# ChunLI-666/PointCloudProcessor

Measured on AMD Instinct MI355X. Metric: Mpoints×frames/sec colorized, higher is better.
Workload: dtype f32/f64

## Files before the change

### include/pcp_hip.h

```cpp
#ifndef PCP_HIP_H
#define PCP_HIP_H

#include <stdint.h>

#ifdef __cplusplus
extern "C" {
#endif

#define PCP_ABI_VERSION 6

#define PCP_OK 0
#define PCP_ERR_INVALID (-1)
#define PCP_ERR_STATE (-2)
#define PCP_ERR_DEVICE (-3)
#define PCP_ERR_NOMEM (-4)
#define PCP_ERR_RANGE (-5)

typedef struct pcp_context pcp_context;

typedef struct pcp_pose {
  double x, y, z, qw, qx, qy, qz;
} pcp_pose;

typedef struct pcp_camera {
// ... 70 lines not shown
int pcp_upload_cloud_aos(pcp_context *ctx, const void *points, int64_t n, int64_t stride_bytes);
int pcp_upload_cloud_from_result(pcp_context *dst, pcp_context *src, int64_t *out_n);
int64_t pcp_cloud_size(const pcp_context *ctx);

int pcp_pose_to_matrices(const pcp_pose *pose, const double *T_opt, float w2c[12], float c2w[12]);
int pcp_set_frames(pcp_context *ctx, const pcp_pose *poses, int32_t n_frames, const double *T_opt,
                   int32_t T_opt_stride);
int32_t pcp_frame_count(const pcp_context *ctx);
int pcp_upload_image(pcp_context *ctx, int32_t frame, const uint8_t *bgr, int64_t row_stride_bytes);
int pcp_upload_image_async(pcp_context *ctx, int32_t frame, const uint8_t *bgr, int64_t row_stride_bytes);
int pcp_upload_images_block(pcp_context *ctx, int32_t first_frame, int32_t count, const uint8_t *bgr, int64_t row_stride_bytes,
                            int64_t frame_stride_bytes);
int pcp_set_image_adjust(pcp_context *ctx, int32_t enable, float saturation_scale, float brightness_scale);
int pcp_download_image(pcp_context *ctx, int32_t frame, uint8_t *out_bgr, uint8_t *out_mask);
#define PCP_JPEG_MAGIC 0x4A504350u
#define PCP_JPEG_VERSION 1
typedef struct pcp_jpeg_component {
  int32_t h, v;
  int32_t blocks_w, blocks_h;
  int32_t down_w, down_h;
} pcp_jpeg_component;
typedef struct pcp_jpeg_header {
  uint32_t magic, version;
  int32_t width, height, ncomp, reserved;
  pcp_jpeg_component comp[3];
  int64_t n_blocks, n_values;
  int64_t quant_off, mask_off, offset_off, value_off;
} pcp_jpeg_header;
int pcp_upload_image_jpeg(pcp_context *ctx, int32_t frame, const uint8_t *blob, int64_t bytes);
int pcp_upload_image_jpeg_async(pcp_context *ctx, int32_t frame, const uint8_t *blob, int64_t bytes);
int pcp_upload_mask(pcp_context *ctx, int32_t frame, const uint8_t *gray, int64_t row_stride_bytes);

int pcp_project_frame(pcp_context *ctx, int32_t frame, int32_t *out_cell, int32_t *out_pixel, float *out_range,
                      float *out_xyz_cam);
int pcp_cull_frame(pcp_context *ctx, int32_t frame, uint8_t *out_keep, int64_t *out_kept, float *out_depth_map);
int pcp_frame_visible(pcp_context *ctx, int32_t frame, int64_t capacity, int32_t *out_index, uint8_t *out_rgb,
                      uint16_t *out_mask, float *out_xyz_cam, float *out_xyz_world, int64_t *out_count);

int pcp_hpr_stats(pcp_context *ctx, int64_t out[10]);

int pcp_depth_pass(pcp_context *ctx, int32_t frame_begin, int32_t frame_end);
int pcp_depth_maps_device(pcp_context *ctx, void **device_ptr, int64_t *n_floats);
int pcp_download_depth_map(pcp_context *ctx, int32_t frame, float *out_depth_map);
int pcp_depth_accum_reset(pcp_context *ctx);
int pcp_depth_accum_merge(pcp_context *ctx);
int pcp_depth_accum_apply(pcp_context *ctx);
int pcp_depth_accum_device(pcp_context *ctx, void **device_ptr, int64_t *n_floats);
#define PCP_DEPTH_OWN 0
#define PCP_DEPTH_BATCHED 1
int pcp_set_depth_source(pcp_context *ctx, int32_t source);
int pcp_hull_flags_import(pcp_context *ctx, int32_t frame, const uint8_t *keep);
int pcp_colour_reset(pcp_context *ctx);
int pcp_colour_pass(pcp_context *ctx, int32_t frame_begin, int32_t frame_end);
int pcp_colour_finalise(pcp_context *ctx, uint8_t *out_rgb, uint8_t *out_has, int32_t *out_count,
                        float *out_top_score, uint32_t *out_top_rgb, int32_t *out_top_frame);
int pcp_colorize(pcp_context *ctx, uint8_t *out_rgb, uint8_t *out_has);
int pcp_colorize_from_depth(pcp_context *ctx, uint8_t *out_rgb, uint8_t *out_has);
int pcp_download_result_packed(pcp_context *ctx, uint32_t *out_rgba);
int pcp_download_result_packed_async(pcp_context *ctx, uint32_t *out_rgba);
int pcp_download_wait_previous(pcp_context *ctx);
int pcp_colour_result_device(pcp_context *ctx, void **device_ptr, int64_t *n_words);
int pcp_colour_compact(pcp_context *ctx, int64_t capacity, int32_t *out_index, float *out_xyz, uint8_t *out_rgb, uint8_t *out_label,
                       int64_t *out_count);

int pcp_set_label_fusion(pcp_context *ctx, int32_t enable);
int pcp_colour_labels(pcp_context *ctx, uint8_t *out_label, uint8_t *out_hits, uint8_t *out_views);
int pcp_colour_labels_device(pcp_context *ctx, void **device_ptr, int64_t *n_words);

int pcp_colour_smooth_local(pcp_context *ctx, float radius, int64_t *out_has_count);
int pcp_colour_smooth_local_packed(pcp_context *ctx, float radius, const uint32_t *in_rgba, uint32_t *out_rgba,
                                   int64_t *out_has_count);

int pcp_mls_process(pcp_context *ctx, const pcp_mls_params *p, int64_t *out_count);
int pcp_set_mls_local_plane(pcp_context *ctx, double upsampling_radius, double upsampling_step);
int pcp_mls_local_plane_samples(double radius, double step, int64_t capacity, float *out_u, float *out_v, int64_t *out_count);
int pcp_mls_process_shard(pcp_context *ctx, const pcp_mls_params *p, int64_t index_begin, int64_t index_end,
                          int64_t *out_count);
int pcp_mls_process_slab(pcp_context *ctx, const pcp_mls_params *p, int32_t slab, int32_t n_slabs, int64_t *out_count);
int pcp_mls_stream_begin(pcp_context *ctx, const pcp_mls_params *p, int64_t chunk_capacity, int64_t *out_total,
                         int32_t *out_chunks);
int pcp_mls_stream_next(pcp_context *ctx, int64_t *out_count);
int pcp_mls_stream_seek(pcp_context *ctx, int32_t chunk);
int pcp_mls_fetch(pcp_context *ctx, int64_t capacity, float *out_xyz, float *out_normal, float *out_curvature,
                  int32_t *out_index);
int pcp_cloud_smooth(pcp_context *ctx, const pcp_mls_params *p, int64_t *out_count);

int pcp_cloud_smooth_stream_begin(pcp_context *ctx, const pcp_mls_params *p, int64_t chunk_capacity, int64_t *out_total_rows,
                                  int64_t *out_kept_rows, int32_t *out_chunks);
int pcp_cloud_smooth_stream_next(pcp_context *ctx, int64_t *out_count);
int pcp_cloud_smooth_stream_end(pcp_context *ctx);
int pcp_cloud_smooth_stream_seek(pcp_context *ctx, int32_t chunk);
int pcp_cloud_smooth_stream_stats(pcp_context *ctx, double out[13]);
int pcp_sor(pcp_context *ctx, int32_t mean_k, double std_mul, uint8_t *out_keep, int64_t *out_kept);
int64_t pcp_sor_chunk_points(void);
int pcp_sor_partial(pcp_context *ctx, int32_t mean_k, int32_t slab, int32_t n_slabs, int64_t capacity, double *out_chunk_sums,
                    int64_t *out_first_chunk, int64_t *out_chunks);
int pcp_sor_finish(pcp_context *ctx, double std_mul, const double *all_chunk_sums, int64_t n_chunks, int32_t slab, int32_t n_slabs,
                   uint8_t *out_keep, int64_t *out_kept);

int pcp_upload_intensity(pcp_context *ctx, const float *intensity, int64_t n);
int pcp_nid_prepare(pcp_context *ctx, int64_t *out_points);
int pcp_nid_evaluate(pcp_context *ctx, const double T[16], const double *T_init, int32_t bins, double *cost,
                     double grad6[6], int32_t *valid);
int pcp_nid_optimize(pcp_context *ctx, const double T_init[16], int32_t bins, int32_t max_outer_iterations,
                     double T_out[16], double *final_cost, int32_t *evaluations);

int pcp_nid_accumulate(pcp_context *ctx, const double T[16], int32_t bins);
int pcp_nid_histograms_device(pcp_context *ctx, void **device_ptr, int64_t *count);
int pcp_nid_finish(pcp_context *ctx, int32_t bins, double *cost, double grad6[6], int32_t *valid);
typedef int (*pcp_nid_eval_fn)(void *user, const double T[16], int32_t bins, double *cost, double grad6[6], int32_t *valid);
int pcp_nid_optimize_with(pcp_context *ctx, pcp_nid_eval_fn eval, void *user, const double T_init[16], int32_t bins,
                          int32_t max_outer_iterations, double T_out[16], double *final_cost, int32_t *evaluations);

#define PCP_ROWS_XYZI 0
#define PCP_ROWS_XYZRGB 1
#define PCP_ROWS_XYZRGBMASK 2
#define PCP_ROWS_POINTNORMAL 3
int64_t pcp_ascii_row_bound(int32_t kind);
int pcp_ascii_rows_host(int32_t kind, int64_t n, const float *f, const uint8_t *rgb, const uint16_t *mask, int64_t capacity,
                        char *out_text, int64_t *out_bytes);
int pcp_ascii_rows(pcp_context *ctx, int32_t kind, int64_t n, const float *f, const uint8_t *rgb, const uint16_t *mask,
                   int64_t capacity, char *out_text, int64_t *out_bytes);
int pcp_colour_compact_ascii(pcp_context *ctx, int32_t with_label, int64_t first_row, int64_t max_rows, int64_t capacity,
                             char *out_text, int64_t *out_rows, int64_t *out_bytes);
int pcp_mls_fetch_ascii(pcp_context *ctx, int64_t first_row, int64_t max_rows, int64_t capacity, char *out_text,
                        int64_t *out_rows, int64_t *out_bytes);

#define PCP_ASCII_PARSE_MAX_ROW 65536
#define PCP_PARSE_LIMIT_ROW 0
#define PCP_PARSE_LIMIT_TILE 1
#define PCP_PARSE_LIMIT_PIECE 2
#define PCP_PARSE_LIMIT_TILE_ROWS 3
#define PCP_PARSE_LIMIT_WINDOW 4
int64_t pcp_ascii_parse_limit(int32_t which);
int pcp_ascii_parse_host(const char *text, int64_t bytes, int32_t columns, const int32_t col[4], int32_t final_window,
                         int64_t max_rows, float *out_x, float *out_y, float *out_z, float *out_intensity,
                         int64_t *out_rows, int64_t *out_consumed, int64_t *out_bad_row);
int pcp_ascii_parse(pcp_context *ctx, const char *text, int64_t bytes, int32_t columns, const int32_t col[4], int32_t final_window,
                    int64_t max_rows, float *out_x, float *out_y, float *out_z, float *out_intensity,
                    int64_t *out_rows, int64_t *out_consumed, int64_t *out_bad_row);

int pcp_close_pairs(pcp_context *ctx, double radius, int64_t *points_with_close_neighbour);

int pcp_timing_enable(pcp_context *ctx, int32_t on);
int pcp_timing_reset(pcp_context *ctx);
int pcp_timing_get(pcp_context *ctx, int32_t kernel_id, double *total_ms, int64_t *launches);
const char *pcp_kernel_name(int32_t kernel_id);
int pcp_tile_mask_density(pcp_context *ctx, double *kept_fraction);
int pcp_tile_masks(pcp_context *ctx, int64_t *tiles, int32_t *mask_words, uint32_t *out_words);
int pcp_sor_redo_fraction(pcp_context *ctx, double *fraction);
int pcp_sor_distances(pcp_context *ctx, int64_t capacity, float *out_distance);
int pcp_selftest_arithmetic(pcp_context *ctx, int64_t samples, uint64_t seed, int64_t *mismatches_fp64,
                            int64_t *mismatches_fp32);

#ifdef __cplusplus
}
#endif
#endif
```

### pointcloudprocessor_amd/_build.py

```python
from __future__ import annotations

import os
import subprocess

_PKG = os.path.dirname(os.path.abspath(__file__))
_ROOT = os.path.dirname(_PKG)
CSRC = os.path.join(_PKG, "csrc")
LIB_DIR = os.path.join(_PKG, "lib")
LIB_PATH = os.path.join(LIB_DIR, "libpcp_hip.so")
INCLUDE = os.path.join(_ROOT, "include")

SOURCES = ["pcp_context.hip", "pcp_colour.hip", "pcp_mls.hip", "pcp_nid.hip", "pcp_hpr.hip", "pcp_colour_smooth.hip", "pcp_match.hip", "pcp_jpeg.hip",
           "pcp_stream_colour.hip", "pcp_ascii.hip", "pcp_ascii_parse.hip"]
HEADERS = ["pcp_internal.hpp", "pcp_device.hpp", "pcp_scan.hpp", "pcp_hsv.hpp", "pcp_exact.hpp", "pcp_ascii.hpp", "pcp_ascii_parse.hpp"]

HIPCC_FLAGS = [
    "--offload-arch=gfx950",
    "-O3",
    "-std=c++17",
    "-fPIC",
    "-ffp-contract=off",
    "-fhip-fp32-correctly-rounded-divide-sqrt",
    "-Wall",
    "-Wextra",
]


def _hipcc() -> str:
    for cand in (os.environ.get("HIPCC"), "/opt/rocm/bin/hipcc", "hipcc"):
        if cand and (os.path.isabs(cand) and os.path.exists(cand) or not os.path.isabs(cand)):
            return cand
    return "hipcc"


def source_sha256() -> str:
    import hashlib

    h = hashlib.sha256()
    h.update(" ".join(HIPCC_FLAGS).encode())
    for f in [os.path.join(CSRC, f) for f in SOURCES + HEADERS] + [os.path.join(INCLUDE, "pcp_hip.h")]:
        h.update(os.path.basename(f).encode())
        with open(f, "rb") as fh:
            h.update(fh.read())
    return h.hexdigest()


def is_stale() -> bool:
    if not os.path.exists(LIB_PATH):
        return True
    t = os.path.getmtime(LIB_PATH)
    deps = [os.path.join(CSRC, f) for f in SOURCES + HEADERS] + [os.path.join(INCLUDE, "pcp_hip.h")]
    return any(os.path.getmtime(d) > t for d in deps)


def build(force: bool = False, verbose: bool = False) -> str:
    if not force and not is_stale():
        return LIB_PATH
    os.makedirs(LIB_DIR, exist_ok=True)
    from concurrent.futures import ThreadPoolExecutor

    obj_dir = os.path.join(LIB_DIR, "obj")
    os.makedirs(obj_dir, exist_ok=True)
    inc = ["-I", os.path.relpath(INCLUDE, CSRC), "-I", "."]

    def compile_one(src):
        stem = os.path.splitext(src)[0]
        obj = os.path.join(os.path.relpath(obj_dir, CSRC), stem + ".o")
        cmd = [_hipcc()] + HIPCC_FLAGS + inc + [f"-cuid={stem}", "-c", src, "-o", obj]
        return cmd, subprocess.run(cmd, capture_output=True, text=True, cwd=CSRC)

    with ThreadPoolExecutor(max_workers=len(SOURCES)) as pool:
        results = list(pool.map(compile_one, SOURCES))
    log = ""
    for cmd, proc in results:
        if verbose or proc.returncode != 0:
            log += " ".join(cmd) + "\n" + proc.stdout + proc.stderr
    if any(proc.returncode != 0 for _, proc in results):
        print(log)
        raise RuntimeError("hipcc failed building libpcp_hip.so:\n" + log[-4000:])
    objs = [os.path.join(os.path.relpath(obj_dir, CSRC), os.path.splitext(src)[0] + ".o") for src in SOURCES]
    link = [_hipcc(), "--offload-arch=gfx950", "--hip-link", "-shared", "-fPIC", "-o", LIB_PATH] + objs
    proc = subprocess.run(link, capture_output=True, text=True, cwd=CSRC)
    if verbose or proc.returncode != 0:
        print(log + " ".join(link))
        print(proc.stdout)
        print(proc.stderr)
    if proc.returncode != 0:
        raise RuntimeError("hipcc failed linking libpcp_hip.so:\n" + proc.stderr[-4000:])
    return LIB_PATH


if __name__ == "__main__":
    print(build(force=True, verbose=True))
```

### pointcloudprocessor_amd/capi.py

```python
from __future__ import annotations

import ctypes as C
import os
import re

import numpy as np

from . import _build

PCP_OK = 0
PCP_ERR_INVALID = -1
PCP_ERR_STATE = -2
PCP_ERR_DEVICE = -3
PCP_ERR_NOMEM = -4
PCP_ERR_RANGE = -5

NID_EVAL_FN = C.CFUNCTYPE(C.c_int, C.c_void_p, C.POINTER(C.c_double), C.c_int32, C.POINTER(C.c_double), C.POINTER(C.c_double),
                          C.POINTER(C.c_int32))
K_PROJECT, K_DEPTH, K_COLOUR, K_VISIBILITY, K_MLS_GRID, K_MLS_FIT, K_MISC, K_SOR, K_MLS_VOXEL, K_TILE_MASK, K_NID, K_HPR = range(12)
K_COLOUR_SMOOTH = 12
K_COUNT = 13


class PcpError(RuntimeError):
# ... 635 lines not shown
    def cloud_smooth(self, params: MLSParams) -> int:
        cnt = C.c_int64()
        self._check(self.lib.pcp_cloud_smooth(self.h, C.byref(params), C.byref(cnt)))
        return cnt.value

    def mls_fetch(self, count: int):
        xyz = np.empty((count, 3), np.float32)
        nrm = np.empty((count, 3), np.float32)
        curv = np.empty(count, np.float32)
        idx = np.empty(count, np.int32)
        self._check(self.lib.pcp_mls_fetch(self.h, C.c_int64(count), _ptr(xyz), _ptr(nrm), _ptr(curv), _ptr(idx)))
        return dict(xyz=xyz, normal=nrm, curvature=curv, index=idx)

    def mls_fetch_index(self, count: int) -> np.ndarray:
        idx = np.empty(count, np.int32)
        self._check(self.lib.pcp_mls_fetch(self.h, C.c_int64(count), None, None, None, _ptr(idx)))
        return idx

    def sor(self, mean_k: int = 60, std_mul: float = 0.7):
        keep = np.empty(self.n, np.uint8)
        kept = C.c_int64()
        self._check(self.lib.pcp_sor(self.h, C.c_int32(mean_k), C.c_double(std_mul), _ptr(keep), C.byref(kept)))
        return keep, kept.value

    def sor_chunk_points(self) -> int:
        return int(self.lib.pcp_sor_chunk_points())

    def sor_partial(self, mean_k: int, slab: int, n_slabs: int):
        c = self.sor_chunk_points()
        chunks = (self.n + c - 1) // c
        out = np.zeros((max(chunks, 1), 2), np.float64)
        first, cnt = C.c_int64(), C.c_int64()
        self._check(self.lib.pcp_sor_partial(self.h, C.c_int32(mean_k), C.c_int32(slab), C.c_int32(n_slabs), C.c_int64(len(out)),
                                             _ptr(out), C.byref(first), C.byref(cnt)))
        return first.value, out[:cnt.value].copy()

    def sor_finish(self, std_mul: float, all_chunk_sums: np.ndarray, slab: int, n_slabs: int):
        sums = np.ascontiguousarray(all_chunk_sums, np.float64)
        keep = np.empty(self.n, np.uint8)
        kept = C.c_int64()
        self._check(self.lib.pcp_sor_finish(self.h, C.c_double(std_mul), _ptr(sums), C.c_int64(len(sums)), C.c_int32(slab),
                                            C.c_int32(n_slabs), _ptr(keep), C.byref(kept)))
        return keep, kept.value

    def close_pairs(self, radius: float = 2.5e-5) -> int:
        cnt = C.c_int64()
        self._check(self.lib.pcp_close_pairs(self.h, C.c_double(radius), C.byref(cnt)))
        return cnt.value

    def sor_distances(self) -> np.ndarray:
        out = np.empty(self.n, np.float32)
        self._check(self.lib.pcp_sor_distances(self.h, C.c_int64(len(out)), _ptr(out)))
        return out

    def sor_redo_fraction(self) -> float:
        v = C.c_double()
        self._check(self.lib.pcp_sor_redo_fraction(self.h, C.byref(v)))
        return v.value

    def upload_intensity(self, intensity):
        a = np.ascontiguousarray(intensity, np.float32)
        self._check(self.lib.pcp_upload_intensity(self.h, _ptr(a), C.c_int64(len(a))))

    def nid_prepare(self) -> int:
        cnt = C.c_int64()
        self._check(self.lib.pcp_nid_prepare(self.h, C.byref(cnt)))
        return cnt.value

    def nid_evaluate(self, T, T_init=None, bins: int = 16):
        T = np.ascontiguousarray(T, np.float64).reshape(16)
        Ti = None if T_init is None else np.ascontiguousarray(T_init, np.float64).reshape(16)
        cost = C.c_double()
        grad = np.zeros(6, np.float64)
        valid = C.c_int32()
        self._check(self.lib.pcp_nid_evaluate(self.h, _ptr(T), _ptr(Ti), C.c_int32(bins), C.byref(cost), _ptr(grad),
                                              C.byref(valid)))
        return cost.value, grad, bool(valid.value)

    def nid_optimize(self, T_init, bins: int = 16, max_outer_iterations: int = 10):
        Ti = np.ascontiguousarray(T_init, np.float64).reshape(16)
        out = np.zeros(16, np.float64)
        cost = C.c_double()
        evals = C.c_int32()
        self._check(self.lib.pcp_nid_optimize(self.h, _ptr(Ti), C.c_int32(bins), C.c_int32(max_outer_iterations), _ptr(out),
                                              C.byref(cost), C.byref(evals)))
        return out.reshape(4, 4), cost.value, evals.value

    def nid_accumulate(self, T, bins: int = 16):
        T = np.ascontiguousarray(T, np.float64).reshape(16)
        self._check(self.lib.pcp_nid_accumulate(self.h, _ptr(T), C.c_int32(bins)))

    def nid_histograms_device(self):
        p = C.c_void_p()
        n = C.c_int64()
        self._check(self.lib.pcp_nid_histograms_device(self.h, C.byref(p), C.byref(n)))
        return p.value, n.value

    def nid_finish(self, bins: int = 16):
        cost = C.c_double()
        grad = np.zeros(6, np.float64)
        valid = C.c_int32()
        self._check(self.lib.pcp_nid_finish(self.h, C.c_int32(bins), C.byref(cost), _ptr(grad), C.byref(valid)))
        return cost.value, grad, bool(valid.value)

    def nid_optimize_with(self, evaluate, T_init, bins: int = 16, max_outer_iterations: int = 10):
        errors = []

        @NID_EVAL_FN
        def trampoline(_user, T, b, cost, grad, valid):
            try:
                c, g, ok = evaluate(np.ctypeslib.as_array(T, (16,)).copy().reshape(4, 4), int(b))
                cost[0] = float(c)
                for k in range(6):
                    grad[k] = float(g[k])
                valid[0] = 1 if ok else 0
                return 0
            except Exception as e:
                errors.append(e)
                return -3

        Ti = np.ascontiguousarray(T_init, np.float64).reshape(16)
        out = np.zeros(16, np.float64)
        cost = C.c_double()
        evals = C.c_int32()
        rc = self.lib.pcp_nid_optimize_with(self.h, trampoline, None, _ptr(Ti), C.c_int32(bins), C.c_int32(max_outer_iterations),
                                            _ptr(out), C.byref(cost), C.byref(evals))
        if errors:
            raise errors[0]
        self._check(rc)
        return out.reshape(4, 4), cost.value, evals.value

    def timing_enable(self, on: bool = True):
        self._check(self.lib.pcp_timing_enable(self.h, C.c_int32(1 if on else 0)))

    def timing_reset(self):
        self._check(self.lib.pcp_timing_reset(self.h))

    def timing_get(self, kernel_id: int):
        ms = C.c_double()
        cnt = C.c_int64()
        self._check(self.lib.pcp_timing_get(self.h, C.c_int32(kernel_id), C.byref(ms), C.byref(cnt)))
        return ms.value, cnt.value

    def tile_mask_density(self) -> float:
        v = C.c_double()
        self._check(self.lib.pcp_tile_mask_density(self.h, C.byref(v)))
        return v.value

    def selftest_arithmetic(self, samples: int = 1 << 26, seed: int = 1):
        a, b = C.c_int64(), C.c_int64()
        self._check(self.lib.pcp_selftest_arithmetic(self.h, C.c_int64(samples), C.c_uint64(seed), C.byref(a), C.byref(b)))
        return a.value, b.value

    def tile_masks(self) -> np.ndarray:
        t, w = C.c_int64(), C.c_int32()
        self._check(self.lib.pcp_tile_masks(self.h, C.byref(t), C.byref(w), None))
        out = np.empty((t.value, w.value), np.uint32)
        self._check(self.lib.pcp_tile_masks(self.h, None, None, _ptr(out)))
        return out

    def kernel_name(self, kernel_id: int) -> str:
        return self.lib.pcp_kernel_name(C.c_int32(kernel_id)).decode()
```

### pointcloudprocessor_amd/csrc/pcp_colour.hip

```cpp
#include <algorithm>
#include <cfloat>
#include <cstdlib>

#include "pcp_device.hpp"
#include "pcp_hsv.hpp"
#include "pcp_scan.hpp"

namespace pcp {

constexpr int kBlock = 256;
constexpr uint32_t kFltMaxBits = 0x7f7fffffu;

template <bool kCommon>
__device__ __forceinline__ DevCamera common_camera(const DevCamera &in) {
  DevCamera c = in;
  if constexpr (kCommon) {
    c.cull_mode = PCP_CULL_ZBUFFER;
    c.enable_zbuf = 1;
    c.pretest = 1;
    c.ds_fast = 1;
  }
  return c;
}
inline bool is_common_camera(const DevCamera &c) {
  return c.cull_mode == PCP_CULL_ZBUFFER && c.enable_zbuf == 1 && c.pretest == 1 && c.ds_fast == 1;
}

struct ProjectOut {
  int32_t *cell;
  int32_t *pixel;
  float *range;
  float *xc, *yc, *zc;
};

__device__ __forceinline__ void project_store_one(const DevCamera &cam, const DevFrame &fr, float x, float y, float z,
                                                  int32_t &cell, int32_t &pixel, float &range, float &xc, float &yc,
                                                  float &zc) {
  const Projected p = project_point<true, false>(cam, fr.w2c, x, y, z);
  cell = p.cell;
  pixel = p.pixel;
  range = p.cell != -1 ? static_cast<float>(range64(p.xc, p.yc, p.zc)) : FLT_MAX;
  xc = p.xc;
  yc = p.yc;
  zc = p.zc;
}

template <bool kCommon>
__global__ __launch_bounds__(kBlock) void k_project_frame(const float *__restrict__ x, const float *__restrict__ y,
                                                          const float *__restrict__ z, int64_t n, DevCamera cam_in,
                                                          DevFrame fr, ProjectOut out) {
  const DevCamera cam = common_camera<kCommon>(cam_in);
  const int64_t q = static_cast<int64_t>(blockIdx.x) * kBlock + threadIdx.x;
  const int64_t i0 = q * 4;
  if (i0 >= n) return;
  if (i0 + 3 < n) {
    typedef float nt_f4 __attribute__((ext_vector_type(4)));
    typedef int nt_i4 __attribute__((ext_vector_type(4)));
    const nt_f4 ax = __builtin_nontemporal_load(reinterpret_cast<const nt_f4 *>(x + i0));
    const nt_f4 ay = __builtin_nontemporal_load(reinterpret_cast<const nt_f4 *>(y + i0));
    const nt_f4 az = __builtin_nontemporal_load(reinterpret_cast<const nt_f4 *>(z + i0));
    const float4 vx = make_float4(ax.x, ax.y, ax.z, ax.w), vy = make_float4(ay.x, ay.y, ay.z, ay.w),
                 vz = make_float4(az.x, az.y, az.z, az.w);
    int4 cell, pixel;
    float4 range, xc, yc, zc;
    project_store_one(cam, fr, vx.x, vy.x, vz.x, cell.x, pixel.x, range.x, xc.x, yc.x, zc.x);
    project_store_one(cam, fr, vx.y, vy.y, vz.y, cell.y, pixel.y, range.y, xc.y, yc.y, zc.y);
    project_store_one(cam, fr, vx.z, vy.z, vz.z, cell.z, pixel.z, range.z, xc.z, yc.z, zc.z);
    project_store_one(cam, fr, vx.w, vy.w, vz.w, cell.w, pixel.w, range.w, xc.w, yc.w, zc.w);
    if (out.cell) {
      const nt_i4 c4 = {cell.x, cell.y, cell.z, cell.w};
      __builtin_nontemporal_store(c4, reinterpret_cast<nt_i4 *>(out.cell + i0));
    }
    if (out.range) {
      const nt_f4 r4 = {range.x, range.y, range.z, range.w};
      __builtin_nontemporal_store(r4, reinterpret_cast<nt_f4 *>(out.range + i0));
    }
    if (out.pixel) *reinterpret_cast<int4 *>(out.pixel + i0) = pixel;
    if (out.xc) {
      *reinterpret_cast<float4 *>(out.xc + i0) = xc;
      *reinterpret_cast<float4 *>(out.yc + i0) = yc;
      *reinterpret_cast<float4 *>(out.zc + i0) = zc;
    }
  } else {
    for (int64_t i = i0; i < n; ++i) {
      int32_t cell, pixel;
      float range, xc, yc, zc;
      project_store_one(cam, fr, x[i], y[i], z[i], cell, pixel, range, xc, yc, zc);
      if (out.cell) out.cell[i] = cell;
      if (out.range) out.range[i] = range;
      if (out.pixel) out.pixel[i] = pixel;
      if (out.xc) {
        out.xc[i] = xc;
        out.yc[i] = yc;
        out.zc[i] = zc;
      }
    }
  }
}

struct Interval {
  double lo, hi;
};
__device__ __forceinline__ Interval iv_add(Interval a, Interval b) { return {a.lo + b.lo, a.hi + b.hi}; }
__device__ __forceinline__ Interval iv_scale(double k, Interval a) {
  return k >= 0.0 ? Interval{k * a.lo, k * a.hi} : Interval{k * a.hi, k * a.lo};
}
__device__ __forceinline__ Interval iv_mul(Interval a, Interval b) {
  const double p0 = a.lo * b.lo, p1 = a.lo * b.hi, p2 = a.hi * b.lo, p3 = a.hi * b.hi;
  return {fmin(fmin(p0, p1), fmin(p2, p3)), fmax(fmax(p0, p1), fmax(p2, p3))};
}
__device__ __forceinline__ Interval iv_sqr(Interval a) {
  const double l = fabs(a.lo), h = fabs(a.hi);
  const double mx = fmax(l, h), mn = (a.lo <= 0.0 && a.hi >= 0.0) ? 0.0 : fmin(l, h);
  return {mn * mn, mx * mx};
}
__device__ __forceinline__ Interval iv_mul_pos(Interval a, Interval b) { return {a.lo * b.lo, a.hi * b.hi}; }
__device__ __forceinline__ Interval iv_mul_by_pos(Interval a, Interval b) {
  return {a.lo * (a.lo >= 0.0 ? b.lo : b.hi), a.hi * (a.hi >= 0.0 ? b.hi : b.lo)};
}
__device__ __forceinline__ double iv_rcp_pos(double b) {
  double r = __builtin_amdgcn_rcp(b);
  r = fma(fma(-b, r, 1.0), r, r);
  r = fma(fma(-b, r, 1.0), r, r);
  return r;
}
__device__ __forceinline__ Interval iv_pad(Interval a) {
  const double e = 1e-12 * (fabs(a.lo) + fabs(a.hi)) + 1e-300;
  return {a.lo - e, a.hi + e};
}

__device__ __forceinline__ int tile_classify(const DevCamera &c, const DevFrame &fr, float4 sph) {
  const double cx = sph.x, cy = sph.y, cz = sph.z;
  const float *m = fr.w2c;
  const double X = (m[0] * cx + m[1] * cy) + (m[2] * cz + m[3]);
  const double Y = (m[4] * cx + m[5] * cy) + (m[6] * cz + m[7]);
  const double Z = (m[8] * cx + m[9] * cy) + (m[10] * cz + m[11]);
  const double mag = fr.norm_bound * (fabs(cx) + fabs(cy) + fabs(cz) + 3.0 * sph.w) + fabs(static_cast<double>(m[3])) +
                     fabs(static_cast<double>(m[7])) + fabs(static_cast<double>(m[11])) + 1e-3;
  const double rho = fr.norm_bound * static_cast<double>(sph.w) * (1.0 + 1e-6) + 1e-6 * mag;
  if (!(rho >= 0.0) || !isfinite(X + Y + Z + rho)) return 0;
  if (Z + rho <= 0.0) return 1;
  if (Z - rho <= 0.0) return 0;
  const Interval zi{Z - rho, Z + rho};
  if (!(zi.lo >= 1e-290)) return 0;
  const Interval iz{iv_rcp_pos(zi.hi) * (1.0 - 1e-13), iv_rcp_pos(zi.lo) * (1.0 + 1e-13)};
  const Interval xn = iv_pad(iv_mul_by_pos(Interval{X - rho, X + rho}, iz));
  const Interval yn = iv_pad(iv_mul_by_pos(Interval{Y - rho, Y + rho}, iz));
  const Interval x2 = iv_sqr(xn), y2 = iv_sqr(yn);
  const Interval r2 = iv_add(x2, y2);
  const Interval r4 = iv_mul_pos(r2, r2);
  const Interval r6 = iv_mul_pos(r2, r4);
  Interval rc = iv_add(iv_add(iv_scale(c.k1, r2), iv_scale(c.k2, r4)), iv_scale(c.k3, r6));
  rc.lo += 1.0;
  rc.hi += 1.0;
  const Interval t1 = iv_scale(2.0, iv_mul(xn, yn));
  const Interval t2 = iv_add(r2, iv_scale(2.0, x2));
  const Interval t3 = iv_add(r2, iv_scale(2.0, y2));
  const Interval xd = iv_pad(iv_add(iv_add(iv_mul(rc, xn), iv_scale(c.p1, t1)), iv_scale(c.p2, t2)));
  const Interval yd = iv_pad(iv_add(iv_add(iv_mul(rc, yn), iv_scale(c.p1, t3)), iv_scale(c.p2, t1)));
  Interval u = iv_pad(iv_scale(c.fx, xd)), v = iv_pad(iv_scale(c.fy, yd));
  u.lo += c.cx; u.hi += c.cx;
  v.lo += c.cy; v.hi += c.cy;
  if (!isfinite(u.lo + u.hi + v.lo + v.hi)) return 0;
  if (u.hi < static_cast<double>(c.u_lo) || u.lo > static_cast<double>(c.u_hi) ||
      v.hi < static_cast<double>(c.v_lo) || v.lo > static_cast<double>(c.v_hi))
    return 1;
  return (u.lo > static_cast<double>(c.u_lo) + 1.0 && u.hi < static_cast<double>(c.u_hi) - 1.0 &&
          v.lo > static_cast<double>(c.v_lo) + 1.0 && v.hi < static_cast<double>(c.v_hi) - 1.0)
             ? 2
             : 0;
}

constexpr int kTileGroup = 16;

__global__ __launch_bounds__(kBlock) void k_group_mask_flat(const float4 *__restrict__ spheres, int64_t groups, DevCamera cam,
                                                            const DevFrame *__restrict__ frames, int32_t n_frames,
                                                            int32_t w0, int32_t w1, int32_t words,
                                                            uint32_t *__restrict__ group_mask,
// ... 54 lines not shown
      if (b >= 0 && have) cls = cull_enabled ? tile_classify(cam, frames[(w << 5) + b], sph) : 0;
      const unsigned long long keep = __ballot(cls != 1), ins = __ballot(cls == 2);
#pragma unroll
      for (int k = 0; k < 4; ++k) {
        if (bit[k] >= 0) {
          word |= static_cast<uint32_t>((keep >> (k * 16 + t)) & 1ull) << bit[k];
          inside |= static_cast<uint32_t>((ins >> (k * 16 + t)) & 1ull) << bit[k];
        }
      }
    }
  }
  if (slot == 0 && have) {
    tile_mask[tile * words + w] = word;
    if (inside_mask) inside_mask[tile * words + w] = inside;
  }
}

constexpr int kWorkBins = 1024;
constexpr int kWorkPerBlock = 1024;
__global__ __launch_bounds__(kBlock) void k_tile_work_hist(const uint32_t *__restrict__ tile_mask, int64_t tiles, int32_t w0,
                                                          int32_t w1, int32_t words, int32_t *__restrict__ tile_work,
                                                          int32_t *__restrict__ hist) {
  __shared__ int32_t cnt[kWorkBins];
  for (int b = threadIdx.x; b < kWorkBins; b += kBlock) cnt[b] = 0;
  __syncthreads();
  const int64_t base = static_cast<int64_t>(blockIdx.x) * kWorkPerBlock;
  for (int q = 0; q < kWorkPerBlock / kBlock; ++q) {
    const int64_t t = base + q * kBlock + threadIdx.x;
    if (t < tiles) {
      int32_t visits = 0;
      for (int32_t w = w0; w < w1; ++w) visits += __builtin_popcount(tile_mask[t * words + w]);
      tile_work[t] = visits;
      atomicAdd(&cnt[min(visits, kWorkBins - 1)], 1);
    }
  }
  __syncthreads();
  for (int b = threadIdx.x; b < kWorkBins; b += kBlock)
    if (cnt[b]) atomicAdd(&hist[b], cnt[b]);
}
__device__ __forceinline__ int32_t block_exclusive_scan(int32_t v, int32_t *total);
__global__ __launch_bounds__(kBlock) void k_work_scatter(const int32_t *__restrict__ work, int64_t tiles,
                                                        const int32_t *__restrict__ hist, int32_t *__restrict__ cursor,
                                                        int32_t *__restrict__ order) {
  __shared__ int32_t cnt[kWorkBins];
  __shared__ int32_t first[kWorkBins];
  for (int b = threadIdx.x; b < kWorkBins; b += kBlock) cnt[b] = 0;
  {
    constexpr int kPer = kWorkBins / kBlock;
    int32_t h[kPer], mine = 0;
#pragma unroll
    for (int k = 0; k < kPer; ++k) {
      h[k] = hist[kWorkBins - 1 - (static_cast<int>(threadIdx.x) * kPer + k)];
      mine += h[k];
    }
    int32_t total = 0;
    int32_t run = block_exclusive_scan(mine, &total);
#pragma unroll
    for (int k = 0; k < kPer; ++k) {
      first[kWorkBins - 1 - (static_cast<int>(threadIdx.x) * kPer + k)] = run;
      run += h[k];
    }
  }
  __syncthreads();
  const int64_t base = static_cast<int64_t>(blockIdx.x) * kWorkPerBlock;
  int32_t bin[kWorkPerBlock / kBlock], rank[kWorkPerBlock / kBlock];
#pragma unroll
  for (int q = 0; q < kWorkPerBlock / kBlock; ++q) {
    const int64_t t = base + q * kBlock + threadIdx.x;
    bin[q] = t < tiles ? min(work[t], kWorkBins - 1) : -1;
    rank[q] = bin[q] >= 0 ? atomicAdd(&cnt[bin[q]], 1) : 0;
  }
  __syncthreads();
  for (int b = threadIdx.x; b < kWorkBins; b += kBlock)
    if (cnt[b]) cnt[b] = first[b] + atomicAdd(&cursor[b], cnt[b]);
  __syncthreads();
#pragma unroll
  for (int q = 0; q < kWorkPerBlock / kBlock; ++q)
    if (bin[q] >= 0) order[cnt[bin[q]] + rank[q]] = static_cast<int32_t>(base + q * kBlock + threadIdx.x);
}

constexpr uint32_t kXcdChunk = 16;
__device__ __forceinline__ uint32_t xcd_chunked_block() {
  constexpr uint32_t kXcd = 8, kSuper = kXcd * kXcdChunk;
  const uint32_t b = blockIdx.x;
  if (b >= (gridDim.x / kSuper) * kSuper) return b;
  const uint32_t x = b % kXcd, slot = b / kXcd;
  return ((slot / kXcdChunk) * kXcd + x) * kXcdChunk + slot % kXcdChunk;
}

constexpr unsigned long long kDepthEmpty = 0x7f7f7f7f7f7f7f7full;
__device__ __forceinline__ void depth_min(unsigned long long *__restrict__ map, int32_t cell, unsigned long long bits) {
  if (bits < map[cell]) atomicMin(map + cell, bits);
}
__device__ __forceinline__ double sumsq64(float xc, float yc, float zc) {
  const double X = xc, Y = yc, Z = zc;
  return (X * X + Y * Y) + Z * Z;
}
__global__ __launch_bounds__(kBlock) void k_depth_finish(const unsigned long long *__restrict__ sq, int64_t count,
                                                         uint32_t *__restrict__ range) {
  int64_t i = static_cast<int64_t>(blockIdx.x) * kBlock + threadIdx.x;
  const int64_t stride = static_cast<int64_t>(gridDim.x) * kBlock;
  for (; i < count; i += stride) {
    const unsigned long long b = sq[i];
    float r = FLT_MAX;
    if (b != kDepthEmpty) r = fminf(static_cast<float>(sqrt(__longlong_as_double(static_cast<long long>(b)))), FLT_MAX);
    range[i] = __float_as_uint(r);
  }
}

__device__ __forceinline__ uint32_t range_bits(int32_t w, int32_t f0, int32_t f1) {
  const int32_t fb = max(f0, w << 5), fe = min(f1, (w << 5) + 32);
  const int32_t nb = fe - fb;
  return nb <= 0 ? 0u : (((nb >= 32) ? 0xffffffffu : ((1u << nb) - 1u)) << (fb & 31));
}

template <bool kCommon>
__global__ __launch_bounds__(kBlock) void k_depth_pass(const float *__restrict__ x, const float *__restrict__ y,
                                                       const float *__restrict__ z, int64_t n, DevCamera cam_in,
                                                       const DevFrame *__restrict__ frames, int32_t f0, int32_t f1,
                                                       unsigned long long *__restrict__ depth, int64_t cells,
                                                       int32_t depth_first_frame, uint32_t *__restrict__ tile_mask,
                                                       const uint32_t *__restrict__ tile_inside, int32_t words,
                                                       const int32_t *__restrict__ tile_order) {
  DevCamera cam = common_camera<kCommon>(cam_in);
  if constexpr (kCommon) cam.pretest = 0;
  __shared__ unsigned long long combine[kBlock];
  const int lane = threadIdx.x & 63;
  unsigned long long *tbl = combine + (threadIdx.x & ~63);
  const int64_t j = tile_order ? static_cast<int64_t>(tile_order[blockIdx.x]) * 64 + threadIdx.x
                               : static_cast<int64_t>(xcd_chunked_block()) * kBlock + threadIdx.x;
  const bool live = j < n;
  if (!__ballot(live)) return;
  const float px = live ? x[j] : 0.0f, py = live ? y[j] : 0.0f, pz = live ? z[j] : 0.0f;
  const int64_t tile = __builtin_amdgcn_readfirstlane(static_cast<int32_t>(j >> 6));
  const bool finite_sure = cam.frames_bounded != 0 && __all(fabsf(px) <= 0x1p40f && fabsf(py) <= 0x1p40f && fabsf(pz) <= 0x1p40f);
  unsigned long long *held_at = nullptr;
  unsigned long long held_bits = 0ull, held_seen = 0ull;
  auto settle_held = [&]() {
    if (held_at && held_bits < held_seen) atomicMin(held_at, held_bits);
    held_at = nullptr;
  };
  for (int32_t w = f0 >> 5; w <= (f1 - 1) >> 5; ++w) {
    const uint32_t in_range = range_bits(w, f0, f1);
    uint32_t todo = in_range;
    if (tile_mask) todo &= tile_mask[tile * words + w];
    todo = __builtin_amdgcn_readfirstlane(todo);
    const uint32_t inside = tile_inside ? __builtin_amdgcn_readfirstlane(tile_inside[tile * words + w]) : 0u;
    uint32_t seen = 0u;
    while (todo) {
      const int32_t b = __builtin_ctz(todo);
      const int32_t f = (w << 5) + b;
      todo &= todo - 1u;
      const DevFrame &fr = frames[f];
      const Projected p = project_point(cam, fr.w2c, px, py, pz, ((inside >> b) & 1u) == 0u, finite_sure);
      const bool in_map = live && p.cell >= 0;
      const bool cand = live && p.pixel >= 0 && (cam.enable_zbuf ? p.cell >= 0 : p.cell != -1);
      if (__ballot(cand)) seen |= 1u << b;
      settle_held();
      if (cam.enable_zbuf && __ballot(in_map)) {
        unsigned long long *map = depth + static_cast<uint64_t>(static_cast<uint32_t>(f - depth_first_frame)) * static_cast<uint32_t>(cells);
        unsigned long long key = ~0ull, sbits = 0ull;
        if (in_map) {
          sbits = static_cast<unsigned long long>(__double_as_longlong(sumsq64(p.xc, p.yc, p.zc)));
          key = (static_cast<unsigned long long>(static_cast<uint32_t>(p.cell)) << 32) | (sbits >> 32);
        }
        tbl[lane] = ~0ull;
        __builtin_amdgcn_wave_barrier();
        if (in_map) atomicMin(&tbl[p.cell & 63], key);
        __builtin_amdgcn_wave_barrier();
        if (in_map) {
          const unsigned long long got = tbl[p.cell & 63];
          if (got == key || static_cast<uint32_t>(got >> 32) != static_cast<uint32_t>(p.cell)) {
            held_at = map + p.cell;
            held_bits = sbits;
            held_seen = *held_at;
          }
        }
        __builtin_amdgcn_wave_barrier();
      }
    }
    if (tile_mask && lane == 0 && live) {
      uint32_t *dst = tile_mask + tile * words + w;
      *dst = (*dst & ~in_range) | seen;
    }
  }
  settle_held();
}

__global__ __launch_bounds__(kBlock) void k_visibility(const float *__restrict__ x, const float *__restrict__ y,
                                                       const float *__restrict__ z, int64_t n, DevCamera cam,
                                                       DevFrame fr, const uint32_t *__restrict__ depth,
                                                       const int32_t *__restrict__ perm,
                                                       uint8_t *__restrict__ keep, int32_t require_pixel) {
  const int64_t i = static_cast<int64_t>(blockIdx.x) * kBlock + threadIdx.x;
  if (i >= n) return;
  const Projected p = project_point(cam, fr.w2c, x[i], y[i], z[i]);
  bool k = keep_rule(cam, p, depth);
  if (require_pixel) k = k && p.pixel >= 0;
  if (k) keep[perm ? perm[i] : i] = 1;
}

__device__ __forceinline__ bool keep_by_depth(float xc, float yc, float zc, double lim) {
  const double s = sumsq64(xc, yc, zc);
  const double L = lim * lim;
  bool keep = s < L * (1.0 - 0x1p-40);
  const bool sure = lim > 0.0 && (keep || s > L * (1.0 + 0x1p-40));
  if (!sure) keep = !(sqrt(s) > lim);
  return keep;
}

struct TopState {
  float *score;
  uint32_t *rgb;
  int32_t *frame;
  int32_t *count;
};

struct MatchArgs {
  const uint8_t *in_a;
  unsigned long long *moved;
  float e2;
};

struct LabelOut {
  uint32_t *word;
};

template <bool kCommon, int kMatch, bool kOneShot, bool kLabel = false>
__global__ __launch_bounds__(kBlock) void k_colour_pass(const float *__restrict__ x, const float *__restrict__ y,
                                                        const float *__restrict__ z, int64_t n, DevCamera cam_in,
                                                        const DevFrame *__restrict__ frames, int32_t f0, int32_t f1,
                                                        const uint32_t *__restrict__ depth, int64_t cells,
                                                        const uint32_t *__restrict__ tile_mask, int32_t words,
                                                        const uint32_t *__restrict__ images, int64_t image_px,
                                                        TopState st, const int32_t *__restrict__ perm,
                                                        uint32_t *__restrict__ rgba, int32_t flags_in,
                                                        const uint32_t *__restrict__ hull_bits_in, MatchArgs mb,
                                                        [[maybe_unused]] LabelOut lab) {
  DevCamera cam = common_camera<kCommon>(cam_in);
  if constexpr (kMatch == 1) cam.match_mode = PCP_MATCH_IDENTITY;
  if constexpr (kMatch == 2 || kMatch == 3) cam.match_mode = PCP_MATCH_ROUNDTRIP;
  const uint32_t *__restrict__ hull_bits = kCommon ? nullptr : hull_bits_in;
  const int32_t flags = kOneShot ? 4 : flags_in;
  const int64_t j = static_cast<int64_t>(xcd_chunked_block()) * kBlock + threadIdx.x;
  const bool live = j < n;
  if (!__ballot(live)) return;
  const float px = live ? x[j] : 0.0f, py = live ? y[j] : 0.0f, pz = live ? z[j] : 0.0f;
  const int64_t tile = __builtin_amdgcn_readfirstlane(static_cast<int32_t>(j >> 6));
  const bool finite_sure = cam.frames_bounded != 0 && __all(fabsf(px) <= 0x1p40f && fabsf(py) <= 0x1p40f && fabsf(pz) <= 0x1p40f);
  Top5 t;
  t.init();
  if ((flags & 1) && live) {
    t.s0 = st.score[0 * n + j]; t.s1 = st.score[1 * n + j]; t.s2 = st.score[2 * n + j];
    t.s3 = st.score[3 * n + j]; t.s4 = st.score[4 * n + j];
    t.c0 = st.rgb[0 * n + j]; t.c1 = st.rgb[1 * n + j]; t.c2 = st.rgb[2 * n + j];
    t.c3 = st.rgb[3 * n + j]; t.c4 = st.rgb[4 * n + j];
    t.f0 = st.frame[0 * n + j]; t.f1 = st.frame[1 * n + j]; t.f2 = st.frame[2 * n + j];
    t.f3 = st.frame[3 * n + j]; t.f4 = st.frame[4 * n + j];
    t.count = st.count[j];
  }
  [[maybe_unused]] bool in_a = false;
  [[maybe_unused]] uint32_t moved = 0u;
  if constexpr (kMatch == 3) in_a = live && mb.in_a[j] != 0;
  for (int32_t w = f0 >> 5; w <= (f1 - 1) >> 5; ++w) {
    uint32_t todo = range_bits(w, f0, f1);
    if (tile_mask) todo &= tile_mask[tile * words + w];
    todo = __builtin_amdgcn_readfirstlane(todo);
    const uint32_t hull_word = (hull_bits && live) ? hull_bits[static_cast<int64_t>(w) * n + j] : 0xffffffffu;
    while (todo) {
      const int32_t f = (w << 5) + __builtin_ctz(todo);
      todo &= todo - 1u;
      const DevFrame &fr = frames[f];
      const Projected p = project_point<false>(cam, fr.w2c, px, py, pz, true, finite_sure);
      const bool cand = live && p.pixel >= 0 && (cam.enable_zbuf ? p.cell >= 0 : p.cell != -1) &&
                        ((hull_word >> (f & 31)) & 1u);
      if (cand) {
        const uint32_t dbits = cam.enable_zbuf ? depth[static_cast<uint64_t>(static_cast<uint32_t>(f)) * static_cast<uint32_t>(cells) + static_cast<uint32_t>(p.cell)] : 0u;
        bool keep = true;
        if (cam.enable_zbuf) keep = keep_by_depth(p.xc, p.yc, p.zc, static_cast<double>(__uint_as_float(dbits)) + cam.slack);
        float sx = p.xc, sy = p.yc, sz = p.zc;
        if constexpr (kMatch == 3) {
          if (keep) keep = roundtrip_sample_moved(cam, fr, px, py, pz, sx, sy, sz, mb.e2, moved) && !in_a;
        } else {
          if (cam.match_mode == PCP_MATCH_ROUNDTRIP && keep) keep = roundtrip_sample(cam, fr, px, py, pz, sx, sy, sz);
        }
        if (keep) {
          const uint32_t texel = images[static_cast<uint64_t>(static_cast<uint32_t>(f)) * static_cast<uint32_t>(image_px) + static_cast<uint32_t>(p.pixel)];
          t.insert(final_score(sx, sy, sz, fr.px, fr.py, fr.pz), kLabel ? texel : texel & 0xffffffu, f);
        }
      }
    }
  }
  if constexpr (kMatch == 3) {
    if (moved) atomicAdd(mb.moved, static_cast<unsigned long long>(moved));
  }
  if (!live) return;
  if (flags & 2) {
    st.score[0 * n + j] = t.s0; st.score[1 * n + j] = t.s1; st.score[2 * n + j] = t.s2;
    st.score[3 * n + j] = t.s3; st.score[4 * n + j] = t.s4;
    st.rgb[0 * n + j] = t.c0; st.rgb[1 * n + j] = t.c1; st.rgb[2 * n + j] = t.c2;
    st.rgb[3 * n + j] = t.c3; st.rgb[4 * n + j] = t.c4;
    st.frame[0 * n + j] = t.f0; st.frame[1 * n + j] = t.f1; st.frame[2 * n + j] = t.f2;
    st.frame[3 * n + j] = t.f3; st.frame[4 * n + j] = t.f4;
    st.count[j] = t.count;
  }
  if (flags & 4) {
    const int64_t o = perm[j];
    rgba[o] = t.finalise();
    if constexpr (kLabel) {
      uint32_t bad = 0u;
      lab.word[o] = t.labels(bad);
      if (bad) lab.word[n] = 1u;
    }
  }
}

__device__ __forceinline__ Top5 load_top5(const TopState &st, int64_t n, int64_t j) {
  Top5 t;
  t.s0 = st.score[0 * n + j]; t.s1 = st.score[1 * n + j]; t.s2 = st.score[2 * n + j];
  t.s3 = st.score[3 * n + j]; t.s4 = st.score[4 * n + j];
  t.c0 = st.rgb[0 * n + j]; t.c1 = st.rgb[1 * n + j]; t.c2 = st.rgb[2 * n + j];
  t.c3 = st.rgb[3 * n + j]; t.c4 = st.rgb[4 * n + j];
  t.f0 = st.frame[0 * n + j]; t.f1 = st.frame[1 * n + j]; t.f2 = st.frame[2 * n + j];
  t.f3 = st.frame[3 * n + j]; t.f4 = st.frame[4 * n + j];
  t.count = st.count[j];
  return t;
}
__global__ __launch_bounds__(kBlock) void k_finalise(int64_t n, TopState st, const int32_t *__restrict__ perm,
                                                     uint32_t *__restrict__ rgba) {
  const int64_t j = static_cast<int64_t>(blockIdx.x) * kBlock + threadIdx.x;
  if (j >= n) return;
  const Top5 t = load_top5(st, n, j);
  rgba[static_cast<int64_t>(perm[j])] = t.finalise();
}
__global__ __launch_bounds__(kBlock) void k_finalise_labels(int64_t n, TopState st, const int32_t *__restrict__ perm,
                                                            uint32_t *__restrict__ rgba, LabelOut lab) {
  const int64_t j = static_cast<int64_t>(blockIdx.x) * kBlock + threadIdx.x;
  if (j >= n) return;
  const Top5 t = load_top5(st, n, j);
  const int64_t o = perm[j];
  rgba[o] = t.finalise();
  uint32_t bad = 0u;
  lab.word[o] = t.labels(bad);
  if (bad) lab.word[n] = 1u;
}

template <bool kLabel>
__global__ __launch_bounds__(kBlock) void k_match_fixup(const float *__restrict__ x, const float *__restrict__ y,
                                                        const float *__restrict__ z, int64_t n, DevCamera cam,
                                                        const DevFrame *__restrict__ frames, int32_t f0, int32_t f1,
                                                        const uint32_t *__restrict__ depth, int64_t cells,
                                                        const uint32_t *__restrict__ tile_mask, int32_t words,
                                                        const uint32_t *__restrict__ images, int64_t image_px, TopState st,
                                                        const int32_t *__restrict__ perm, uint32_t *__restrict__ rgba,
                                                        int32_t flags, const uint32_t *__restrict__ hull_bits,
                                                        const int32_t *__restrict__ list, int64_t na,
                                                        const int64_t *__restrict__ off, const int32_t *__restrict__ cols,
                                                        [[maybe_unused]] LabelOut lab) {
  const int64_t a = static_cast<int64_t>(blockIdx.x) * kBlock + threadIdx.x;
  if (a >= na) return;
  const int64_t j = list[a];
  Top5 t;
  t.init();
  if (flags & 1) {
    t.s0 = st.score[0 * n + j]; t.s1 = st.score[1 * n + j]; t.s2 = st.score[2 * n + j];
    t.s3 = st.score[3 * n + j]; t.s4 = st.score[4 * n + j];
    t.c0 = st.rgb[0 * n + j]; t.c1 = st.rgb[1 * n + j]; t.c2 = st.rgb[2 * n + j];
    t.c3 = st.rgb[3 * n + j]; t.c4 = st.rgb[4 * n + j];
    t.f0 = st.frame[0 * n + j]; t.f1 = st.frame[1 * n + j]; t.f2 = st.frame[2 * n + j];
    t.f3 = st.frame[3 * n + j]; t.f4 = st.frame[4 * n + j];
    t.count = st.count[j];
  }
  const float qx = x[j], qy = y[j], qz = z[j];
  const int64_t r0 = off[a], r1 = off[a + 1];
  for (int32_t f = f0; f < f1; ++f) {
    const DevFrame &fr = frames[f];
    const int32_t w = f >> 5;
    const uint32_t bit = 1u << (f & 31);
    for (int64_t r = r0; r < r1; ++r) {
      const int64_t i = cols[r];
      if (tile_mask && !(tile_mask[(i >> 6) * words + w] & bit)) continue;
      if (hull_bits && !(hull_bits[static_cast<int64_t>(w) * n + i] & bit)) continue;
      const float px = x[i], py = y[i], pz = z[i];
      const Projected p = project_point<false>(cam, fr.w2c, px, py, pz);
      const bool cand = p.pixel >= 0 && (cam.enable_zbuf ? p.cell >= 0 : p.cell != -1);
      if (!cand) continue;
      if (cam.enable_zbuf) {
        const uint32_t dbits = depth[static_cast<uint64_t>(static_cast<uint32_t>(f)) * static_cast<uint32_t>(cells) + static_cast<uint32_t>(p.cell)];
        if (!keep_by_depth(p.xc, p.yc, p.zc, static_cast<double>(__uint_as_float(dbits)) + cam.slack)) continue;
      }
      float sx = p.xc, sy = p.yc, sz = p.zc;
      if (!roundtrip_sample(cam, fr, qx, qy, qz, sx, sy, sz)) continue;
      const uint32_t texel = images[static_cast<uint64_t>(static_cast<uint32_t>(f)) * static_cast<uint32_t>(image_px) + static_cast<uint32_t>(p.pixel)];
      t.insert(final_score(sx, sy, sz, fr.px, fr.py, fr.pz), kLabel ? texel : texel & 0xffffffu, f);
    }
  }
  if (flags & 2) {
    st.score[0 * n + j] = t.s0; st.score[1 * n + j] = t.s1; st.score[2 * n + j] = t.s2;
    st.score[3 * n + j] = t.s3; st.score[4 * n + j] = t.s4;
    st.rgb[0 * n + j] = t.c0; st.rgb[1 * n + j] = t.c1; st.rgb[2 * n + j] = t.c2;
    st.rgb[3 * n + j] = t.c3; st.rgb[4 * n + j] = t.c4;
    st.frame[0 * n + j] = t.f0; st.frame[1 * n + j] = t.f1; st.frame[2 * n + j] = t.f2;
    st.frame[3 * n + j] = t.f3; st.frame[4 * n + j] = t.f4;
    st.count[j] = t.count;
  }
  if (flags & 4) {
    const int64_t o = perm[j];
    rgba[o] = t.finalise();
    if constexpr (kLabel) {
      uint32_t bad = 0u;
      lab.word[o] = t.labels(bad);
      if (bad) lab.word[n] = 1u;
    }
  }
}

template <bool kLabel>
inline auto colour_pass_kernel(bool common, int32_t match_mode, int32_t flags) {
  auto kernel = k_colour_pass<false, 0, false, kLabel>;
  if (common && match_mode == PCP_MATCH_IDENTITY)
    kernel = flags == 4 ? k_colour_pass<true, 1, true, kLabel> : k_colour_pass<true, 1, false, kLabel>;
  if (common && match_mode == PCP_MATCH_ROUNDTRIP)
    kernel = flags == 4 ? k_colour_pass<true, 2, true, kLabel> : k_colour_pass<true, 2, false, kLabel>;
  if (match_mode == PCP_MATCH_RADIUS)
    kernel = !common ? k_colour_pass<false, 3, false, kLabel>
                     : flags == 4 ? k_colour_pass<true, 3, true, kLabel> : k_colour_pass<true, 3, false, kLabel>;
  return kernel;
}

__device__ __forceinline__ uint64_t mix64(uint64_t v) {
  v += 0x9e3779b97f4a7c15ull;
  v = (v ^ (v >> 30)) * 0xbf58476d1ce4e5b9ull;
  v = (v ^ (v >> 27)) * 0x94d049bb133111ebull;
  return v ^ (v >> 31);
}
__device__ __forceinline__ bool same_f64(double a, double b) {
  if (a != a && b != b) return true;
  if (a == 0.0 && b == 0.0) return true;
  return __double_as_longlong(a) == __double_as_longlong(b);
}

__global__ __launch_bounds__(kBlock) void k_selftest_div64(int64_t samples, uint64_t seed,
                                                           unsigned long long *__restrict__ bad) {
  const int64_t i = static_cast<int64_t>(blockIdx.x) * kBlock + threadIdx.x;
  if (i >= samples) return;
  const uint64_t a = mix64(seed ^ static_cast<uint64_t>(i) * 3u), b = mix64(a);
  uint32_t bx = static_cast<uint32_t>(a), by = static_cast<uint32_t>(a >> 32), bz = static_cast<uint32_t>(b);
  const uint32_t mode = static_cast<uint32_t>(b >> 32) & 3u;
  if (mode != 0u) {
    const uint32_t span = mode == 1u ? 12u : 40u;
    bx = (bx & 0x807fffffu) | ((127u - span / 2u + (bx >> 23) % span) << 23);
    by = (by & 0x807fffffu) | ((127u - span / 2u + (by >> 23) % span) << 23);
    bz = (bz & 0x807fffffu) | ((127u - span / 2u + (bz >> 23) % span) << 23);
  }
  const float xc = __uint_as_float(bx), yc = __uint_as_float(by), zc = fabsf(__uint_as_float(bz));
  if (!(zc > 0.0f)) return;
  double xn, yn;
  divide_xy_by_z(xc, yc, zc, xn, yn);
  const double xr = static_cast<double>(xc) / static_cast<double>(zc);
  const double yr = static_cast<double>(yc) / static_cast<double>(zc);
  if (!same_f64(xn, xr) || !same_f64(yn, yr)) atomicAdd(bad, 1ull);
}

__global__ __launch_bounds__(kBlock) void k_selftest_div32(DevCamera cam, unsigned long long *__restrict__ bad) {
  const uint32_t lane = blockIdx.x * kBlock + threadIdx.x;
  uint32_t wrong = 0u;
  for (uint32_t k = 0; k < 256u; ++k) {
    const float x = __uint_as_float((k << 24) | lane);
    const float a = div_by_ds(cam, x), b = x / cam.ds_f;
    const float ax = fabsf(x);
    if (ax >= 0x1p-40f && ax <= 0x1p60f) {
      if (!((a != a && b != b) || __float_as_uint(a) == __float_as_uint(b))) ++wrong;
    } else {
      if (cell_of_quotient(a, cam.cull_wf) != cell_of_quotient(b, cam.cull_wf)) ++wrong;
      if (cell_of_quotient(a, cam.cull_hf) != cell_of_quotient(b, cam.cull_hf)) ++wrong;
    }
  }
  if (wrong) atomicAdd(bad, static_cast<unsigned long long>(wrong));
}

__global__ __launch_bounds__(kBlock) void k_unpack_result(const uint32_t *__restrict__ packed, int64_t n,
                                                         uint8_t *__restrict__ rgb, uint8_t *__restrict__ has) {
  const int64_t i = static_cast<int64_t>(blockIdx.x) * kBlock + threadIdx.x;
  if (i >= n) return;
  const uint32_t v = packed[i];
  rgb[3 * i + 0] = static_cast<uint8_t>(v & 0xffu);
  rgb[3 * i + 1] = static_cast<uint8_t>((v >> 8) & 0xffu);
  rgb[3 * i + 2] = static_cast<uint8_t>((v >> 16) & 0xffu);
  has[i] = static_cast<uint8_t>(v >> 24);
}

__global__ __launch_bounds__(kBlock) void k_unpack_labels(const uint32_t *__restrict__ packed, int64_t n,
                                                         uint8_t *__restrict__ label, uint8_t *__restrict__ hits,
                                                         uint8_t *__restrict__ views) {
  const int64_t i = static_cast<int64_t>(blockIdx.x) * kBlock + threadIdx.x;
  if (i >= n) return;
  const uint32_t v = packed[i];
  if (label) label[i] = static_cast<uint8_t>(v & 0xffu);
  if (hits) hits[i] = static_cast<uint8_t>((v >> 8) & 0xffu);
  if (views) views[i] = static_cast<uint8_t>((v >> 16) & 0xffu);
}

__global__ __launch_bounds__(kBlock) void k_fill_u32(uint32_t *__restrict__ p, int64_t n, uint32_t v) {
  int64_t i = static_cast<int64_t>(blockIdx.x) * kBlock + threadIdx.x;
  const int64_t stride = static_cast<int64_t>(gridDim.x) * kBlock;
  for (; i < n; i += stride) p[i] = v;
}

__global__ __launch_bounds__(kBlock) void k_scatter_u32(const uint32_t *__restrict__ in,
                                                        const int32_t *__restrict__ perm, int64_t n,
                                                        uint32_t *__restrict__ out) {
  const int64_t j = static_cast<int64_t>(blockIdx.x) * kBlock + threadIdx.x;
  if (j < n) out[perm[j]] = in[j];
}

__global__ __launch_bounds__(kBlock) void k_pack_bgr(const uint8_t *__restrict__ bgr, int64_t row_stride, int32_t w,
                                                     int32_t h, uint32_t *__restrict__ texels, int32_t clear_mask,
                                                     const int32_t *__restrict__ hsv_tables, float sat_scale,
                                                     float val_scale) {
  const int64_t i = static_cast<int64_t>(blockIdx.x) * kBlock + threadIdx.x;
  if (i >= static_cast<int64_t>(w) * h) return;
  const int32_t v = static_cast<int32_t>(i / w), u = static_cast<int32_t>(i - static_cast<int64_t>(v) * w);
  const uint8_t *p = bgr + static_cast<int64_t>(v) * row_stride + 3 * u;
  const uint32_t keep = clear_mask ? 0u : (texels[i] & 0xff000000u);
  uint32_t b = p[0], g = p[1], r = p[2];
  if (hsv_tables) hsv_round_trip(hsv_tables, hsv_tables + 256, sat_scale, val_scale, b, g, r);
  texels[i] = keep | b | (g << 8) | (r << 16);
}

__global__ __launch_bounds__(kBlock) void k_pack_bgr16(const uint8_t *__restrict__ bgr, int64_t row_stride, int32_t w,
                                                       int32_t h, uint32_t *__restrict__ texels, int32_t clear_mask,
                                                       const int32_t *__restrict__ hsv_tables, float sat_scale,
                                                       float val_scale) {
  const int32_t groups = w >> 4;
  const int64_t n_groups = static_cast<int64_t>(groups) * h;
  const int64_t g = static_cast<int64_t>(blockIdx.x) * kBlock + threadIdx.x;
  uint4 a, b, c;
  if (row_stride == 3 * static_cast<int64_t>(w)) {
    __shared__ uint4 piece[3 * kBlock];
    const int64_t base = static_cast<int64_t>(blockIdx.x) * (3 * kBlock);
    const int64_t pieces = 3 * n_groups;
    const uint4 *src = reinterpret_cast<const uint4 *>(bgr);
#pragma unroll
    for (int q = 0; q < 3; ++q) {
      const int64_t i = base + q * kBlock + threadIdx.x;
      if (i < pieces) piece[q * kBlock + threadIdx.x] = src[i];
    }
    __syncthreads();
    if (g >= n_groups) return;
    a = piece[3 * threadIdx.x];
    b = piece[3 * threadIdx.x + 1];
    c = piece[3 * threadIdx.x + 2];
  } else {
    if (g >= n_groups) return;
    const int32_t vr = static_cast<int32_t>(g / groups), gr = static_cast<int32_t>(g - static_cast<int64_t>(vr) * groups);
    const uint4 *src = reinterpret_cast<const uint4 *>(bgr + static_cast<int64_t>(vr) * row_stride + static_cast<int64_t>(gr) * 48);
    a = src[0];
    b = src[1];
    c = src[2];
  }
  const int32_t v = static_cast<int32_t>(g / groups), gu = static_cast<int32_t>(g - static_cast<int64_t>(v) * groups);
  const uint32_t in[12] = {a.x, a.y, a.z, a.w, b.x, b.y, b.z, b.w, c.x, c.y, c.z, c.w};
  uint4 *dst = reinterpret_cast<uint4 *>(texels + static_cast<int64_t>(v) * w + static_cast<int64_t>(gu) * 16);
  uint32_t out[16];
#pragma unroll
  for (int q = 0; q < 4; ++q) {
    const uint32_t d0 = in[3 * q], d1 = in[3 * q + 1], d2 = in[3 * q + 2];
    out[4 * q + 0] = d0 & 0xffffffu;
    out[4 * q + 1] = (d0 >> 24) | ((d1 & 0xffffu) << 8);
    out[4 * q + 2] = (d1 >> 16) | ((d2 & 0xffu) << 16);
    out[4 * q + 3] = d2 >> 8;
  }
  if (hsv_tables) {
#pragma unroll
    for (int k = 0; k < 16; ++k) {
      uint32_t bb = out[k] & 0xffu, gg = (out[k] >> 8) & 0xffu, rr = out[k] >> 16;
      hsv_round_trip(hsv_tables, hsv_tables + 256, sat_scale, val_scale, bb, gg, rr);
      out[k] = bb | (gg << 8) | (rr << 16);
    }
  }
  if (!clear_mask) {
#pragma unroll
    for (int q = 0; q < 4; ++q) {
      const uint4 old = dst[q];
      out[4 * q + 0] |= old.x & 0xff000000u;
      out[4 * q + 1] |= old.y & 0xff000000u;
      out[4 * q + 2] |= old.z & 0xff000000u;
      out[4 * q + 3] |= old.w & 0xff000000u;
    }
  }
#pragma unroll
  for (int q = 0; q < 4; ++q) dst[q] = make_uint4(out[4 * q], out[4 * q + 1], out[4 * q + 2], out[4 * q + 3]);
}

__global__ __launch_bounds__(kBlock) void k_pack_mask(const uint8_t *__restrict__ gray, int64_t row_stride, int32_t w,
                                                      int32_t h, uint32_t *__restrict__ texels) {
  const int64_t i = static_cast<int64_t>(blockIdx.x) * kBlock + threadIdx.x;
  if (i >= static_cast<int64_t>(w) * h) return;
  const int32_t v = static_cast<int32_t>(i / w), u = static_cast<int32_t>(i - static_cast<int64_t>(v) * w);
  texels[i] = (texels[i] & 0x00ffffffu) | (static_cast<uint32_t>(gray[static_cast<int64_t>(v) * row_stride + u]) << 24);
}

constexpr int kTile = 1024;

__device__ __forceinline__ int32_t block_exclusive_scan(int32_t v, int32_t *total) {
  __shared__ int32_t wave_sum[kBlock / 64];
  const int lane = threadIdx.x & 63, wid = threadIdx.x >> 6;
  int32_t incl = v;
#pragma unroll
  for (int o = 1; o < 64; o <<= 1) {
    const int32_t t = __shfl_up(incl, o, 64);
    if (lane >= o) incl += t;
  }
  if (lane == 63) wave_sum[wid] = incl;
  __syncthreads();
  int32_t base = 0, tot = 0;
#pragma unroll
  for (int k = 0; k < kBlock / 64; ++k) {
    if (k < wid) base += wave_sum[k];
    tot += wave_sum[k];
  }
  __syncthreads();
  *total = tot;
  return base + incl - v;
}

__global__ __launch_bounds__(kBlock) void k_tile_count(const uint8_t *__restrict__ flags, int64_t n,
                                                       int32_t *__restrict__ tile_count) {
  const int64_t base = static_cast<int64_t>(blockIdx.x) * kTile + threadIdx.x * 4;
  int32_t c = 0;
#pragma unroll
  for (int k = 0; k < 4; ++k)
    if (base + k < n) c += flags[base + k] ? 1 : 0;
// ... 455 lines not shown
  }
  int pack(pcp_context *ctx, int, hipStream_t us, int32_t k, uint32_t *dst, int32_t clear_mask, const int32_t *tables) override {
    const int32_t w = ctx->dcam.img_w, h = ctx->dcam.img_h;
    const int64_t px = static_cast<int64_t>(w) * h;
    const uint8_t *sk = src + static_cast<int64_t>(k) * block_stride;
    if ((w & 15) == 0 && (row_stride_bytes & 15) == 0 && (reinterpret_cast<uintptr_t>(sk) & 15u) == 0)
      hipLaunchKernelGGL(k_pack_bgr16, dim3(blocks_for(px / 16)), dim3(kBlock), 0, us, sk, row_stride_bytes, w, h, dst,
                         clear_mask, tables, ctx->saturation_scale, ctx->brightness_scale);
    else
      hipLaunchKernelGGL(k_pack_bgr, dim3(blocks_for(px)), dim3(kBlock), 0, us, sk, row_stride_bytes, w, h, dst, clear_mask,
                         tables, ctx->saturation_scale, ctx->brightness_scale);
    return PCP_OK;
  }
};

static int upload_image_impl(pcp_context *ctx, const char *who, int32_t frame, const uint8_t *bgr, int64_t row_stride_bytes,
                             bool wait, size_t block_bytes = 0, int64_t block_stride = 0, int32_t block_frames = 1) {
  BgrSource source(bgr, row_stride_bytes, block_bytes, block_stride);
  return upload_texels(ctx, who, frame, block_frames, block_bytes > 0, wait, source);
}

extern "C" {

int pcp_upload_image(pcp_context *ctx, int32_t frame, const uint8_t *bgr, int64_t row_stride_bytes) {
  return upload_image_impl(ctx, "pcp_upload_image", frame, bgr, row_stride_bytes, true);
}

int pcp_upload_image_async(pcp_context *ctx, int32_t frame, const uint8_t *bgr, int64_t row_stride_bytes) {
  return upload_image_impl(ctx, "pcp_upload_image_async", frame, bgr, row_stride_bytes, false);
}

constexpr size_t kBlockUploadBytes = size_t(128) << 20;

int pcp_upload_images_block(pcp_context *ctx, int32_t first_frame, int32_t count, const uint8_t *bgr, int64_t row_stride_bytes,
                            int64_t frame_stride_bytes) {
  int rc = check_ready(ctx, "pcp_upload_images_block", true);
  if (rc != PCP_OK) return rc;
  if (count < 0 || first_frame < 0 || first_frame + count > ctx->n_frames)
    return set_error(ctx, PCP_ERR_RANGE, "pcp_upload_images_block: keyframes [%d, %d) outside 0..%d", first_frame, first_frame + count,
                     ctx->n_frames);
  if (count == 0) return PCP_OK;
  const int32_t w = ctx->dcam.img_w, h = ctx->dcam.img_h;
  if (!bgr || row_stride_bytes < 3 * static_cast<int64_t>(w) || frame_stride_bytes < row_stride_bytes * h)
    return set_error(ctx, PCP_ERR_INVALID, "pcp_upload_images_block: NULL block, row stride < 3*width or frame stride < rows");
  hipPointerAttribute_t attr{};
  const bool host_pinned = hipPointerGetAttributes(&attr, bgr) == hipSuccess && attr.type == hipMemoryTypeHost;
  if (!host_pinned) {
    (void)hipGetLastError();
    for (int32_t k = 0; k < count; ++k)
      if ((rc = upload_image_impl(ctx, "pcp_upload_images_block", first_frame + k, bgr + static_cast<int64_t>(k) * frame_stride_bytes,
                                  row_stride_bytes, false)) != PCP_OK)
        return rc;
    return PCP_OK;
  }
  const int32_t per_block = static_cast<int32_t>(std::max<int64_t>(1, static_cast<int64_t>(kBlockUploadBytes) / frame_stride_bytes));
  for (int32_t b0 = 0; b0 < count; b0 += per_block) {
    const int32_t b1 = std::min(count, b0 + per_block);
    const size_t bytes = static_cast<size_t>(b1 - b0 - 1) * static_cast<size_t>(frame_stride_bytes) + static_cast<size_t>(row_stride_bytes) * h;
    if ((rc = upload_image_impl(ctx, "pcp_upload_images_block", first_frame + b0, bgr + static_cast<int64_t>(b0) * frame_stride_bytes,
                                row_stride_bytes, false, bytes, frame_stride_bytes, b1 - b0)) != PCP_OK)
      return rc;
  }
  return PCP_OK;
}

int pcp_set_image_adjust(pcp_context *ctx, int32_t enable, float saturation_scale, float brightness_scale) {
  if (!ctx) return PCP_ERR_INVALID;
  if (!(saturation_scale >= 0.0f) || !(brightness_scale >= 0.0f))
    return set_error(ctx, PCP_ERR_INVALID, "pcp_set_image_adjust: scales must be >= 0");
  PCP_HIP_TRY(ctx, hipSetDevice(ctx->device));
  if (enable && !ctx->hsv_tables.p) {
    int32_t tab[512];
    hsv_build_tables(tab, tab + 256);
    PCP_HIP_TRY(ctx, ctx->hsv_tables.ensure(512));
    PCP_HIP_TRY(ctx, hipMemcpyAsync(ctx->hsv_tables.p, tab, sizeof(tab), hipMemcpyHostToDevice, ctx->stream));
    PCP_HIP_TRY(ctx, hipStreamSynchronize(ctx->stream));
  }
  ctx->adjust_images = enable != 0;
  ctx->saturation_scale = saturation_scale;
  ctx->brightness_scale = brightness_scale;
  return PCP_OK;
}

int pcp_download_image(pcp_context *ctx, int32_t frame, uint8_t *out_bgr, uint8_t *out_mask) {
  int rc = check_ready(ctx, "pcp_download_image", true);
  if (rc != PCP_OK) return rc;
  if ((rc = check_frame(ctx, "pcp_download_image", frame)) != PCP_OK) return rc;
  if (!ctx->images.p || !(ctx->image_set[static_cast<size_t>(frame)] || ctx->mask_set[static_cast<size_t>(frame)]))
    return set_error(ctx, PCP_ERR_STATE, "pcp_download_image: nothing uploaded for keyframe %d", frame);
  if ((rc = wait_images(ctx, frame, frame + 1)) != PCP_OK) return rc;
  const int32_t w = ctx->dcam.img_w, h = ctx->dcam.img_h;
  const size_t px = static_cast<size_t>(w) * h;
  std::vector<uint32_t> texels(px);
  PCP_HIP_TRY(ctx, hipMemcpyAsync(texels.data(), ctx->images.p + static_cast<int64_t>(frame) * static_cast<int64_t>(px),
                                  px * 4, hipMemcpyDeviceToHost, ctx->stream));
  PCP_HIP_TRY(ctx, hipStreamSynchronize(ctx->stream));
  for (size_t i = 0; i < px; ++i) {
    const uint32_t t = texels[i];
    if (out_bgr) {
      out_bgr[3 * i + 0] = static_cast<uint8_t>(t & 0xffu);
      out_bgr[3 * i + 1] = static_cast<uint8_t>((t >> 8) & 0xffu);
      out_bgr[3 * i + 2] = static_cast<uint8_t>((t >> 16) & 0xffu);
    }
    if (out_mask) out_mask[i] = static_cast<uint8_t>(t >> 24);
  }
  return PCP_OK;
}

int pcp_upload_mask(pcp_context *ctx, int32_t frame, const uint8_t *gray, int64_t row_stride_bytes) {
  int rc = check_ready(ctx, "pcp_upload_mask", true);
  if (rc != PCP_OK) return rc;
  if ((rc = check_frame(ctx, "pcp_upload_mask", frame)) != PCP_OK) return rc;
  const int32_t w = ctx->dcam.img_w, h = ctx->dcam.img_h;
  if (!gray || row_stride_bytes < static_cast<int64_t>(w))
    return set_error(ctx, PCP_ERR_INVALID, "pcp_upload_mask: NULL mask or row stride < width");
  if ((rc = ensure_images(ctx)) != PCP_OK) return rc;
  if ((rc = wait_images(ctx, frame, frame + 1)) != PCP_OK) return rc;
  const size_t bytes = static_cast<size_t>(row_stride_bytes) * h;
  PCP_HIP_TRY(ctx, ctx->s_keep.ensure(bytes + 16));
  PCP_HIP_TRY(ctx, hipMemcpyAsync(ctx->s_keep.p, gray, bytes, hipMemcpyDefault, ctx->stream));
  const int64_t px = static_cast<int64_t>(w) * h;
  {
    LaunchTimer t(ctx, PCP_K_MISC);
    hipLaunchKernelGGL(k_pack_mask, dim3(blocks_for(px)), dim3(kBlock), 0, ctx->stream, ctx->s_keep.p,
                       row_stride_bytes, w, h, ctx->images.p + static_cast<int64_t>(frame) * px);
    PCP_HIP_TRY(ctx, hipGetLastError());
  }
  PCP_HIP_TRY(ctx, hipStreamSynchronize(ctx->stream));
  ctx->mask_set[static_cast<size_t>(frame)] = 1;
  return PCP_OK;
}

int pcp_project_frame(pcp_context *ctx, int32_t frame, int32_t *out_cell, int32_t *out_pixel, float *out_range,
                      float *out_xyz_cam) {
  int rc = check_ready(ctx, "pcp_project_frame", true);
  if (rc != PCP_OK) return rc;
  if ((rc = check_frame(ctx, "pcp_project_frame", frame)) != PCP_OK) return rc;
  const int64_t n = ctx->n;
  const size_t plane = plane_of(ctx);
  PCP_HIP_TRY(ctx, ctx->s_cell.ensure(plane + 4));
  PCP_HIP_TRY(ctx, ctx->s_range.ensure(plane + 4));
  if (out_pixel) PCP_HIP_TRY(ctx, ctx->s_pixel.ensure(plane + 4));
  if (out_xyz_cam) PCP_HIP_TRY(ctx, ctx->s_cam.ensure(3 * plane + 4));
  if (n == 0) return PCP_OK;
  ProjectOut o{};
  o.cell = ctx->s_cell.p;
  o.range = ctx->s_range.p;
  o.pixel = out_pixel ? ctx->s_pixel.p : nullptr;
  o.xc = out_xyz_cam ? ctx->s_cam.p : nullptr;
  o.yc = out_xyz_cam ? ctx->s_cam.p + plane : nullptr;
  o.zc = out_xyz_cam ? ctx->s_cam.p + 2 * plane : nullptr;
  {
    LaunchTimer t(ctx, PCP_K_PROJECT);
    hipLaunchKernelGGL(is_common_camera(ctx->dcam) ? k_project_frame<true> : k_project_frame<false>, dim3(blocks_for(div_up(n, 4))), dim3(kBlock), 0, ctx->stream, ctx->sxyz.p,
                       ctx->sxyz.p + plane, ctx->sxyz.p + 2 * plane, n, ctx->dcam,
                       ctx->hframes[static_cast<size_t>(frame)], o);
    PCP_HIP_TRY(ctx, hipGetLastError());
  }
  if (!(out_cell || out_range || out_pixel || out_xyz_cam)) return PCP_OK;
  const size_t sn = static_cast<size_t>(n);
  PCP_HIP_TRY(ctx, ctx->s_u32.ensure(plane + 4));
  auto fetch = [&](const void *sorted, void *host) -> int {
    {
      LaunchTimer t(ctx, PCP_K_MISC);
      hipLaunchKernelGGL(k_scatter_u32, dim3(blocks_for(n)), dim3(kBlock), 0, ctx->stream,
                         static_cast<const uint32_t *>(sorted), ctx->perm.p, n, ctx->s_u32.p);
      PCP_HIP_TRY(ctx, hipGetLastError());
    }
    PCP_HIP_TRY(ctx, hipMemcpyAsync(host, ctx->s_u32.p, sn * 4, hipMemcpyDeviceToHost, ctx->stream));
    PCP_HIP_TRY(ctx, hipStreamSynchronize(ctx->stream));
    return PCP_OK;
  };
  if (out_cell && (rc = fetch(o.cell, out_cell)) != PCP_OK) return rc;
  if (out_range && (rc = fetch(o.range, out_range)) != PCP_OK) return rc;
  if (out_pixel && (rc = fetch(o.pixel, out_pixel)) != PCP_OK) return rc;
  if (out_xyz_cam) {
    if ((rc = fetch(o.xc, out_xyz_cam)) != PCP_OK) return rc;
    if ((rc = fetch(o.yc, out_xyz_cam + sn)) != PCP_OK) return rc;
    if ((rc = fetch(o.zc, out_xyz_cam + 2 * sn)) != PCP_OK) return rc;
  }
  return PCP_OK;
}

int pcp_cull_frame(pcp_context *ctx, int32_t frame, uint8_t *out_keep, int64_t *out_kept, float *out_depth_map) {
  int rc = check_ready(ctx, "pcp_cull_frame", true);
  if (rc != PCP_OK) return rc;
  if ((rc = check_frame(ctx, "pcp_cull_frame", frame)) != PCP_OK) return rc;
  const int64_t n = ctx->n;
  if ((rc = single_frame_depth(ctx, frame)) != PCP_OK) return rc;
  if ((rc = frame_keep_flags(ctx, frame, false)) != PCP_OK) return rc;
  if (out_kept) {
    int64_t cnt = 0;
    if (n > 0 && (rc = compact_flags(ctx, ctx->s_keep.p, n, nullptr, 0, &cnt)) != PCP_OK) return rc;
    *out_kept = cnt;
  }
  if (out_keep && n > 0)
    PCP_HIP_TRY(ctx, hipMemcpyAsync(out_keep, ctx->s_keep.p, static_cast<size_t>(n), hipMemcpyDefault, ctx->stream));
  if (out_depth_map)
    PCP_HIP_TRY(ctx, hipMemcpyAsync(out_depth_map, ctx->s_u32.p, static_cast<size_t>(cells_of(ctx)) * 4,
                                    hipMemcpyDeviceToHost, ctx->stream));
  PCP_HIP_TRY(ctx, hipStreamSynchronize(ctx->stream));
  return PCP_OK;
}

int pcp_frame_visible(pcp_context *ctx, int32_t frame, int64_t capacity, int32_t *out_index, uint8_t *out_rgb,
                      uint16_t *out_mask, float *out_xyz_cam, float *out_xyz_world, int64_t *out_count) {
  int rc = check_ready(ctx, "pcp_frame_visible", true);
  if (rc != PCP_OK) return rc;
  if ((rc = check_frame(ctx, "pcp_frame_visible", frame)) != PCP_OK) return rc;
  if (capacity < 0) return set_error(ctx, PCP_ERR_INVALID, "pcp_frame_visible: negative capacity");
  const int64_t n = ctx->n;
  if (out_count) *out_count = 0;
  if (n == 0) return PCP_OK;
  if ((rc = ensure_images(ctx)) != PCP_OK) return rc;
  if ((rc = wait_images(ctx, frame, frame + 1)) != PCP_OK) return rc;
  if ((rc = single_frame_depth(ctx, frame)) != PCP_OK) return rc;
  const size_t plane = plane_of(ctx);
  PCP_HIP_TRY(ctx, ctx->s_cell.ensure(plane + 4));
  if ((rc = frame_keep_flags(ctx, frame, true)) != PCP_OK) return rc;
  int64_t m = 0;
  if ((rc = compact_flags(ctx, ctx->s_keep.p, n, ctx->s_cell.p, static_cast<int64_t>(plane), &m)) != PCP_OK) return rc;
  if (out_count) *out_count = m;
  const int64_t take = std::min(m, capacity);
  if (take == 0) return PCP_OK;
  const size_t st = static_cast<size_t>(take);
  PCP_HIP_TRY(ctx, ctx->s_range.ensure(st + 4));
  const bool want_cam = out_xyz_cam != nullptr, want_world = out_xyz_world != nullptr;
  PCP_HIP_TRY(ctx, ctx->s_cam.ensure((want_cam ? 3 * st : 0) + (want_world ? 3 * st : 0) + 4));
  float *d_cam = want_cam ? ctx->s_cam.p : nullptr;
  float *d_world = want_world ? ctx->s_cam.p + (want_cam ? 3 * st : 0) : nullptr;
  const int64_t px = static_cast<int64_t>(ctx->dcam.img_w) * ctx->dcam.img_h;
  {
    LaunchTimer t(ctx, PCP_K_MISC);
    hipLaunchKernelGGL(k_gather_visible, dim3(blocks_for(take)), dim3(kBlock), 0, ctx->stream, ctx->xyz.p,
                       ctx->xyz.p + plane, ctx->xyz.p + 2 * plane, ctx->dcam, ctx->hframes[static_cast<size_t>(frame)],
                       ctx->s_cell.p, take, ctx->images.p + static_cast<int64_t>(frame) * px,
                       static_cast<int32_t>(ctx->image_set[static_cast<size_t>(frame)]),
                       static_cast<int32_t>(ctx->mask_set[static_cast<size_t>(frame)]),
                       reinterpret_cast<uint32_t *>(ctx->s_range.p), d_cam, d_world);
    PCP_HIP_TRY(ctx, hipGetLastError());
  }
  std::vector<uint32_t> rgbm;
  if (out_rgb || out_mask) {
    rgbm.resize(st);
    PCP_HIP_TRY(ctx, hipMemcpyAsync(rgbm.data(), ctx->s_range.p, st * 4, hipMemcpyDeviceToHost, ctx->stream));
  }
  if (out_index) PCP_HIP_TRY(ctx, hipMemcpyAsync(out_index, ctx->s_cell.p, st * 4, hipMemcpyDeviceToHost, ctx->stream));
  if (want_cam) PCP_HIP_TRY(ctx, hipMemcpyAsync(out_xyz_cam, d_cam, 3 * st * 4, hipMemcpyDeviceToHost, ctx->stream));
  if (want_world) PCP_HIP_TRY(ctx, hipMemcpyAsync(out_xyz_world, d_world, 3 * st * 4, hipMemcpyDeviceToHost, ctx->stream));
  PCP_HIP_TRY(ctx, hipStreamSynchronize(ctx->stream));
  for (size_t k = 0; k < rgbm.size(); ++k) {
    if (out_rgb) {
      out_rgb[3 * k + 0] = static_cast<uint8_t>(rgbm[k] & 0xffu);
      out_rgb[3 * k + 1] = static_cast<uint8_t>((rgbm[k] >> 8) & 0xffu);
      out_rgb[3 * k + 2] = static_cast<uint8_t>((rgbm[k] >> 16) & 0xffu);
    }
    if (out_mask) out_mask[k] = static_cast<uint16_t>(rgbm[k] >> 24);
  }
  return PCP_OK;
}

int pcp_depth_pass(pcp_context *ctx, int32_t frame_begin, int32_t frame_end) {
  int rc = check_ready(ctx, "pcp_depth_pass", true);
  if (rc != PCP_OK) return rc;
  if (frame_begin < 0 || frame_end > ctx->n_frames || frame_begin > frame_end)
    return set_error(ctx, PCP_ERR_RANGE, "pcp_depth_pass: keyframe range [%d,%d) outside 0..%d", frame_begin, frame_end,
                     ctx->n_frames);
  if (frame_begin == frame_end) return PCP_OK;
  if ((rc = ensure_depth(ctx)) != PCP_OK) return rc;
  const int64_t cells = cells_of(ctx);
  const int64_t map_cells = static_cast<int64_t>(frame_end - frame_begin) * cells;
  const bool z_maps = ctx->n > 0 && ctx->dcam.enable_zbuf;
  if (z_maps) {
    PCP_HIP_TRY(ctx, ctx->depth_sq.ensure(static_cast<size_t>(map_cells) + 4));
  } else if ((rc = fill_u32(ctx, ctx->depth.p + static_cast<int64_t>(frame_begin) * cells, map_cells, kFltMaxBits)) != PCP_OK) {
    return rc;
  }
  if (ctx->n > 0) {
    const size_t plane = plane_of(ctx);
    const int32_t w0 = frame_begin >> 5, w1 = ((frame_end - 1) >> 5) + 1;
    static const bool cull_tiles = [] {
      const char *e = std::getenv("PCP_DISABLE_TILE_CULL");
      return !(e && e[0] == '1');
    }();
    {
      LaunchTimer t(ctx, PCP_K_TILE_MASK);
      const int64_t groups = div_up(ctx->n_tiles, kTileGroup);
      const float4 *tile_sph = reinterpret_cast<const float4 *>(ctx->tile_sphere.p);
      const size_t gwords = static_cast<size_t>(groups) * ctx->mask_words;
      PCP_HIP_TRY(ctx, ctx->group_mask.ensure(2 * gwords + 8));
      uint32_t *group_inside = ctx->group_mask.p + gwords + 4;
      hipLaunchKernelGGL(k_group_mask_flat, dim3(std::max(blocks_for(groups * (w1 - w0) * 32), blocks_for(2 * kWorkBins))),
                         dim3(kBlock), 0, ctx->stream, tile_sph + ctx->n_tiles, groups, ctx->dcam, ctx->frames.p, ctx->n_frames,
                         w0, w1, ctx->mask_words, ctx->group_mask.p, group_inside, cull_tiles ? 1 : 0, ctx->work_hist.p,
                         2 * kWorkBins, z_maps ? reinterpret_cast<unsigned long long *>(ctx->depth_sq.p) : nullptr,
                         z_maps ? map_cells : int64_t(0));
      hipLaunchKernelGGL(k_tile_mask_dense, dim3(static_cast<uint32_t>(div_up(groups * (w1 - w0), kBlock / 64))), dim3(kBlock),
                         0, ctx->stream, tile_sph, ctx->n_tiles, ctx->dcam, ctx->frames.p, ctx->n_frames, w0, w1,
                         ctx->mask_words, ctx->group_mask.p, group_inside, ctx->tile_mask.p, ctx->tile_inside.p, cull_tiles ? 1 : 0);
      if ((rc = sort_tiles_by_work(ctx, w0, w1, ctx->tile_order.p)) != PCP_OK) return rc;
      ctx->tile_order_live = true;
    }
    if (ctx->cull.cull_mode == PCP_CULL_HPR) {
      int rch = ensure_hull_bits(ctx);
      if (rch != PCP_OK) return rch;
      if (!ctx->depth_from_batch) {
        int32_t clear_until = frame_begin;
        for (int32_t f = frame_begin; f < frame_end; ++f) {
          uint32_t *hull_plane = ctx->hull_bits.p + static_cast<size_t>(f >> 5) * static_cast<size_t>(ctx->n);
          if ((f & 31) == 0 && std::min(f + 32, ctx->n_frames) <= frame_end) {
            PCP_HIP_TRY(ctx, hipMemsetAsync(hull_plane, 0, static_cast<size_t>(ctx->n) * 4, ctx->stream));
            clear_until = std::min(f + 32, ctx->n_frames);
          }
          if (f >= clear_until) {
            LaunchTimer t(ctx, PCP_K_HPR);
            hipLaunchKernelGGL(k_hull_clear, dim3(blocks_for(ctx->n)), dim3(kBlock), 0, ctx->stream, hull_plane, ctx->n, 1u << (f & 31));
          }
        }
        PCP_HIP_TRY(ctx, hipGetLastError());
        const char *le = std::getenv("PCP_HPR_LANES");
        const int32_t lanes = le && le[0] >= '1' && le[0] <= '8' ? le[0] - '0' : 4;
        if ((rc = hpr_run_range(ctx, frame_begin, frame_end, lanes, ctx->tile_mask.p)) != PCP_OK) return rc;
        for (int32_t f = frame_begin; f < frame_end; ++f) ctx->hull_valid[static_cast<size_t>(f)] = 1;
      }
    }
    {
      LaunchTimer t(ctx, PCP_K_DEPTH);
      hipLaunchKernelGGL(is_common_camera(ctx->dcam) ? k_depth_pass<true> : k_depth_pass<false>,
                         dim3(static_cast<uint32_t>(ctx->n_tiles)), dim3(64), 0, ctx->stream, ctx->sxyz.p,
                         ctx->sxyz.p + plane, ctx->sxyz.p + 2 * plane, ctx->n, ctx->dcam, ctx->frames.p, frame_begin,
                         frame_end, ctx->depth_sq.p, cells, frame_begin, ctx->tile_mask.p, ctx->tile_inside.p,
                         ctx->mask_words, ctx->tile_order.p);
      if (z_maps)
        hipLaunchKernelGGL(k_depth_finish, dim3(static_cast<uint32_t>(std::min<int64_t>(div_up(map_cells, kBlock), 4096))),
                           dim3(kBlock), 0, ctx->stream, ctx->depth_sq.p, map_cells,
                           ctx->depth.p + static_cast<int64_t>(frame_begin) * cells);
      PCP_HIP_TRY(ctx, hipGetLastError());
    }
  }
  for (int32_t f = frame_begin; f < frame_end; ++f) ctx->depth_valid[static_cast<size_t>(f)] = 1;
  return PCP_OK;
}

int pcp_depth_maps_device(pcp_context *ctx, void **device_ptr, int64_t *n_floats) {
  int rc = check_ready(ctx, "pcp_depth_maps_device", true);
  if (rc != PCP_OK) return rc;
  if (ctx->cull.cull_mode == PCP_CULL_HPR)
    return set_error(ctx, PCP_ERR_STATE, "pcp_depth_maps_device: PCP_CULL_HPR has no depth maps to merge across point shards "
                     "(the hull needs the whole map on one GPU)");
  if ((rc = ensure_depth(ctx)) != PCP_OK) return rc;
  if (device_ptr) *device_ptr = ctx->depth.p;
  if (n_floats) *n_floats = cells_of(ctx) * ctx->n_frames;
  return PCP_OK;
}

int pcp_set_depth_source(pcp_context *ctx, int32_t source) {
  if (!ctx) return PCP_ERR_INVALID;
  if (source != PCP_DEPTH_OWN && source != PCP_DEPTH_BATCHED)
    return set_error(ctx, PCP_ERR_INVALID, "pcp_set_depth_source: unknown source %d", source);
  ctx->depth_from_batch = source == PCP_DEPTH_BATCHED;
  return PCP_OK;
}

int pcp_hull_flags_import(pcp_context *ctx, int32_t frame, const uint8_t *keep) {
  int rc = check_ready(ctx, "pcp_hull_flags_import", true);
  if (rc != PCP_OK) return rc;
  if ((rc = check_frame(ctx, "pcp_hull_flags_import", frame)) != PCP_OK) return rc;
  if (ctx->cull.cull_mode != PCP_CULL_HPR || !ctx->depth_from_batch)
    return set_error(ctx, PCP_ERR_STATE, "pcp_hull_flags_import: needs cull_mode PCP_CULL_HPR and pcp_set_depth_source(PCP_DEPTH_BATCHED)");
  if (!keep && ctx->n > 0) return set_error(ctx, PCP_ERR_INVALID, "pcp_hull_flags_import: NULL flags");
  if ((rc = ensure_hull_bits(ctx)) != PCP_OK) return rc;
  if (ctx->n > 0) {
    PCP_HIP_TRY(ctx, ctx->s_keep.ensure(static_cast<size_t>(ctx->n) + 16));
    PCP_HIP_TRY(ctx, hipMemcpyAsync(ctx->s_keep.p, keep, static_cast<size_t>(ctx->n), hipMemcpyDefault, ctx->stream));
    if ((rc = store_hull_bits(ctx, frame, false)) != PCP_OK) return rc;
    PCP_HIP_TRY(ctx, hipStreamSynchronize(ctx->stream));
  }
  ctx->hull_valid[static_cast<size_t>(frame)] = 1;
  return PCP_OK;
}

int pcp_download_depth_map(pcp_context *ctx, int32_t frame, float *out_depth_map) {
  int rc = check_ready(ctx, "pcp_download_depth_map", true);
  if (rc != PCP_OK) return rc;
  if ((rc = check_frame(ctx, "pcp_download_depth_map", frame)) != PCP_OK) return rc;
  if (!out_depth_map) return set_error(ctx, PCP_ERR_INVALID, "pcp_download_depth_map: NULL output");
  if (!ctx->depth.p || !ctx->depth_valid[static_cast<size_t>(frame)])
    return set_error(ctx, PCP_ERR_STATE, "pcp_download_depth_map: pcp_depth_pass has not covered keyframe %d", frame);
  const int64_t cells = cells_of(ctx);
  PCP_HIP_TRY(ctx, hipMemcpyAsync(out_depth_map, ctx->depth.p + static_cast<int64_t>(frame) * cells,
                                  static_cast<size_t>(cells) * 4, hipMemcpyDeviceToHost, ctx->stream));
  PCP_HIP_TRY(ctx, hipStreamSynchronize(ctx->stream));
  return PCP_OK;
}

int pcp_colour_reset(pcp_context *ctx) {
  if (!ctx) return PCP_ERR_INVALID;
  ctx->colour_state_live = false;
  ctx->colour_result_live = false;
  ctx->labels_live = false;
  return PCP_OK;
}

static int begin_result(pcp_context *ctx, uint32_t **dst) {
  const int32_t cur = ctx->rgba_cur ^ 1;
  PCP_HIP_TRY(ctx, ctx->rgba2[cur].ensure(static_cast<size_t>(ctx->n) + 4));
  if (ctx->copy_pending[cur]) {
    PCP_HIP_TRY(ctx, hipStreamWaitEvent(ctx->stream, ctx->copy_done[cur], 0));
    ctx->copy_pending[cur] = false;
  }
  *dst = ctx->rgba2[cur].p;
  return PCP_OK;
}

static int labels_begin(pcp_context *ctx) {
  ctx->labels_live = false;
  if (!ctx->label_fusion) return PCP_OK;
  PCP_HIP_TRY(ctx, ctx->labels.ensure(static_cast<size_t>(ctx->n) + 4));
  PCP_HIP_TRY(ctx, hipMemsetAsync(ctx->labels.p + ctx->n, 0, 4, ctx->stream));
  return PCP_OK;
}

static int labels_end(pcp_context *ctx) {
  if (!ctx->label_fusion) return PCP_OK;
  uint32_t bad = 0;
  uint32_t *dst = ctx->readback ? static_cast<uint32_t *>(ctx->readback) : &bad;
  PCP_HIP_TRY(ctx, hipMemcpyAsync(dst, ctx->labels.p + ctx->n, 4, hipMemcpyDeviceToHost, ctx->stream));
  PCP_HIP_TRY(ctx, hipStreamSynchronize(ctx->stream));
  if (*dst != 0)
    return set_error(ctx, PCP_ERR_RANGE, "label fusion: a view score outside [2^-3, 2) reached the label arithmetic "
                     "(final_score cannot produce one): no labels for this result");
  ctx->labels_live = true;
  return PCP_OK;
}

static int check_masks(pcp_context *ctx, int32_t frame_begin, int32_t frame_end) {
  if (!ctx->label_fusion) return PCP_OK;
  for (int32_t f = frame_begin; f < frame_end; ++f)
    if (static_cast<size_t>(f) >= ctx->mask_set.size() || !ctx->mask_set[static_cast<size_t>(f)])
      return set_error(ctx, PCP_ERR_STATE, "pcp_colour_pass: label fusion is on and no mask was uploaded for keyframe %d", f);
  return PCP_OK;
}

static int colour_pass_impl(pcp_context *ctx, int32_t frame_begin, int32_t frame_end, bool one_shot,
                            uint32_t *result = nullptr) {
  int rc = check_ready(ctx, "pcp_colour_pass", true);
  if (rc != PCP_OK) return rc;
  if (frame_begin < 0 || frame_end > ctx->n_frames || frame_begin > frame_end)
    return set_error(ctx, PCP_ERR_RANGE, "pcp_colour_pass: keyframe range [%d,%d) outside 0..%d", frame_begin, frame_end,
                     ctx->n_frames);
  if ((rc = check_masks(ctx, frame_begin, frame_end)) != PCP_OK) return rc;
  for (int32_t f = frame_begin; f < frame_end; ++f) {
    if (!ctx->depth.p || !ctx->depth_valid[static_cast<size_t>(f)])
      return set_error(ctx, PCP_ERR_STATE, "pcp_colour_pass: pcp_depth_pass has not covered keyframe %d", f);
    if (!ctx->images.p || !ctx->image_set[static_cast<size_t>(f)])
      return set_error(ctx, PCP_ERR_STATE, "pcp_colour_pass: no image uploaded for keyframe %d", f);
    if (ctx->cull.cull_mode == PCP_CULL_HPR && ctx->depth_from_batch &&
        (static_cast<size_t>(f) >= ctx->hull_valid.size() || !ctx->hull_valid[static_cast<size_t>(f)]))
      return set_error(ctx, PCP_ERR_STATE, "pcp_colour_pass: PCP_CULL_HPR on an index shard, pcp_hull_flags_import has not covered keyframe %d", f);
  }
  const bool radius = ctx->dcam.match_mode == PCP_MATCH_RADIUS;
  if (radius && ctx->depth_from_batch)
    return set_error(ctx, PCP_ERR_STATE, "pcp_colour_pass: PCP_MATCH_RADIUS needs the whole map on one context: an index shard "
                     "(PCP_DEPTH_BATCHED) cannot see the neighbours that other shards hold");
  if ((rc = ensure_state(ctx)) != PCP_OK) return rc;
  if ((rc = wait_images(ctx, frame_begin, frame_end)) != PCP_OK) return rc;
  if (ctx->n == 0) return PCP_OK;
  if (radius && (rc = match_table_prepare(ctx)) != PCP_OK) return rc;
  if (frame_begin == frame_end) {
    if (one_shot && result) PCP_HIP_TRY(ctx, hipMemsetAsync(result, 0, static_cast<size_t>(ctx->n) * 4, ctx->stream));
    if (one_shot && ctx->label_fusion)
      PCP_HIP_TRY(ctx, hipMemsetAsync(ctx->labels.p, 0, static_cast<size_t>(ctx->n) * 4, ctx->stream));
    return PCP_OK;
  }
  const size_t plane = plane_of(ctx);
  TopState st{ctx->top_score.p, ctx->top_rgb.p, ctx->top_frame.p, ctx->view_count.p};
  int32_t flags = 0;
  if (ctx->colour_state_live) flags |= 1;
  if (one_shot)
    flags |= 4;
  else
    flags |= 2;
  MatchArgs mb{nullptr, nullptr, 0.0f};
  if (radius) {
    mb = MatchArgs{ctx->match_in_a.p, ctx->match_moved.p, ctx->match_e2};
    PCP_HIP_TRY(ctx, hipMemsetAsync(ctx->match_moved.p, 0, 8, ctx->stream));
  }
  const uint32_t *hull = ctx->cull.cull_mode == PCP_CULL_HPR ? ctx->hull_bits.p : static_cast<const uint32_t *>(nullptr);
  {
    LaunchTimer t(ctx, PCP_K_COLOUR);
    const bool common = is_common_camera(ctx->dcam) && ctx->cull.cull_mode != PCP_CULL_HPR;
    const bool label = ctx->label_fusion;
    const LabelOut lab{label ? ctx->labels.p : nullptr};
    auto kernel = label ? colour_pass_kernel<true>(common, ctx->dcam.match_mode, flags)
                        : colour_pass_kernel<false>(common, ctx->dcam.match_mode, flags);
    hipLaunchKernelGGL(kernel, dim3(blocks_for(ctx->n)), dim3(kBlock), 0, ctx->stream, ctx->sxyz.p, ctx->sxyz.p + plane,
                       ctx->sxyz.p + 2 * plane, ctx->n, ctx->dcam, ctx->frames.p, frame_begin, frame_end, ctx->depth.p,
                       cells_of(ctx), ctx->tile_mask.p, ctx->mask_words, ctx->images.p,
                       static_cast<int64_t>(ctx->dcam.img_w) * ctx->dcam.img_h, st, ctx->perm.p, result, flags, hull, mb, lab);
    PCP_HIP_TRY(ctx, hipGetLastError());
    if (radius && ctx->match_a > 0) {
      hipLaunchKernelGGL(label ? k_match_fixup<true> : k_match_fixup<false>, dim3(blocks_for(ctx->match_a)), dim3(kBlock), 0, ctx->stream, ctx->sxyz.p,
                         ctx->sxyz.p + plane, ctx->sxyz.p + 2 * plane, ctx->n, ctx->dcam, ctx->frames.p, frame_begin, frame_end,
                         ctx->depth.p, cells_of(ctx), ctx->tile_mask.p, ctx->mask_words, ctx->images.p,
                         static_cast<int64_t>(ctx->dcam.img_w) * ctx->dcam.img_h, st, ctx->perm.p, result, flags, hull,
                         ctx->match_list.p, ctx->match_a, ctx->match_off.p, ctx->match_cols.p, lab);
      PCP_HIP_TRY(ctx, hipGetLastError());
    }
  }
  if (!one_shot) ctx->colour_state_live = true;
  if (radius) {
    unsigned long long moved = 0;
    unsigned long long *dst = ctx->readback ? static_cast<unsigned long long *>(ctx->readback) : &moved;
    PCP_HIP_TRY(ctx, hipMemcpyAsync(dst, ctx->match_moved.p, 8, hipMemcpyDeviceToHost, ctx->stream));
    PCP_HIP_TRY(ctx, hipStreamSynchronize(ctx->stream));
    if (*dst != 0)
      return set_error(ctx, PCP_ERR_RANGE, "pcp_colour_pass: PCP_MATCH_RADIUS: %llu samples moved further than the bound E = %g m "
                       "in their fp32 round trip; the neighbour table may miss their matches", *dst, ctx->match_e);
  }
  return PCP_OK;
}

int pcp_colour_pass(pcp_context *ctx, int32_t frame_begin, int32_t frame_end) {
  return colour_pass_impl(ctx, frame_begin, frame_end, false);
}

static int end_result(pcp_context *ctx, uint8_t *out_rgb, uint8_t *out_has) {
  const int64_t n = ctx->n;
  const int32_t cur = ctx->rgba_cur ^ 1;
  uint32_t *dst = ctx->rgba2[cur].p;
  PCP_HIP_TRY(ctx, hipEventRecord(ctx->result_ready[cur], ctx->stream));
  ctx->rgba_cur = cur;
  ctx->colour_result_live = true;
  if ((out_rgb || out_has) && n > 0) {
    const size_t sn = static_cast<size_t>(n);
    PCP_HIP_TRY(ctx, ctx->s_keep.ensure(4 * sn + 16));
    uint8_t *d_rgb = ctx->s_keep.p, *d_has = ctx->s_keep.p + 3 * sn;
    hipLaunchKernelGGL(k_unpack_result, dim3(blocks_for(n)), dim3(kBlock), 0, ctx->stream, dst, n, d_rgb, d_has);
    PCP_HIP_TRY(ctx, hipGetLastError());
    if (out_rgb) PCP_HIP_TRY(ctx, hipMemcpyAsync(out_rgb, d_rgb, 3 * sn, hipMemcpyDeviceToHost, ctx->stream));
    if (out_has) PCP_HIP_TRY(ctx, hipMemcpyAsync(out_has, d_has, sn, hipMemcpyDeviceToHost, ctx->stream));
    PCP_HIP_TRY(ctx, hipStreamSynchronize(ctx->stream));
  }
  return PCP_OK;
}

int pcp_colour_finalise(pcp_context *ctx, uint8_t *out_rgb, uint8_t *out_has, int32_t *out_count, float *out_top_score,
                        uint32_t *out_top_rgb, int32_t *out_top_frame) {
  int rc = check_ready(ctx, "pcp_colour_finalise", false);
  if (rc != PCP_OK) return rc;
  const int64_t n = ctx->n;
  if ((rc = ensure_state(ctx)) != PCP_OK) return rc;
  const size_t sn = static_cast<size_t>(n);
  uint32_t *result = nullptr;
  if ((rc = begin_result(ctx, &result)) != PCP_OK) return rc;
  if ((rc = labels_begin(ctx)) != PCP_OK) return rc;
  if (!ctx->colour_state_live && n > 0) {
    PCP_HIP_TRY(ctx, hipMemsetAsync(result, 0, sn * 4, ctx->stream));
    if (ctx->label_fusion) PCP_HIP_TRY(ctx, hipMemsetAsync(ctx->labels.p, 0, sn * 4, ctx->stream));
    if ((rc = fill_u32(ctx, reinterpret_cast<uint32_t *>(ctx->top_score.p), kTopM * n, 0xbf800000u)) != PCP_OK) return rc;
    PCP_HIP_TRY(ctx, hipMemsetAsync(ctx->top_rgb.p, 0, kTopM * sn * 4, ctx->stream));
    PCP_HIP_TRY(ctx, hipMemsetAsync(ctx->top_frame.p, 0xff, kTopM * sn * 4, ctx->stream));
    PCP_HIP_TRY(ctx, hipMemsetAsync(ctx->view_count.p, 0, sn * 4, ctx->stream));
  } else if (n > 0) {
    TopState st{ctx->top_score.p, ctx->top_rgb.p, ctx->top_frame.p, ctx->view_count.p};
    LaunchTimer t(ctx, PCP_K_COLOUR);
    const bool label = ctx->label_fusion;
    const LabelOut lab{label ? ctx->labels.p : nullptr};
    if (label)
      hipLaunchKernelGGL(k_finalise_labels, dim3(blocks_for(n)), dim3(kBlock), 0, ctx->stream, n, st, ctx->perm.p, result, lab);
    else
      hipLaunchKernelGGL(k_finalise, dim3(blocks_for(n)), dim3(kBlock), 0, ctx->stream, n, st, ctx->perm.p, result);
    PCP_HIP_TRY(ctx, hipGetLastError());
  }
  if ((rc = labels_end(ctx)) != PCP_OK) return rc;
  if ((rc = end_result(ctx, out_rgb, out_has)) != PCP_OK) return rc;
  if ((out_count || out_top_score || out_top_rgb || out_top_frame) && n > 0) {
    std::vector<int32_t> perm(sn), cnt;
    std::vector<uint32_t> tmp(kTopM * sn);
    PCP_HIP_TRY(ctx, hipMemcpyAsync(perm.data(), ctx->perm.p, sn * 4, hipMemcpyDeviceToHost, ctx->stream));
    auto fetch5 = [&](const void *src, void *dst_v) -> int {
      PCP_HIP_TRY(ctx, hipMemcpyAsync(tmp.data(), src, kTopM * sn * 4, hipMemcpyDeviceToHost, ctx->stream));
      PCP_HIP_TRY(ctx, hipStreamSynchronize(ctx->stream));
      uint32_t *dst = static_cast<uint32_t *>(dst_v);
      for (size_t j = 0; j < sn; ++j)
        for (int k = 0; k < kTopM; ++k) dst[static_cast<size_t>(perm[j]) * kTopM + k] = tmp[static_cast<size_t>(k) * sn + j];
      return PCP_OK;
    };
    if (out_top_score && (rc = fetch5(ctx->top_score.p, out_top_score)) != PCP_OK) return rc;
    if (out_top_rgb && (rc = fetch5(ctx->top_rgb.p, out_top_rgb)) != PCP_OK) return rc;
    if (out_top_rgb && ctx->label_fusion)
      for (size_t k = 0; k < kTopM * sn; ++k) out_top_rgb[k] &= 0xffffffu;
    if (out_top_frame && (rc = fetch5(ctx->top_frame.p, out_top_frame)) != PCP_OK) return rc;
    if (out_count) {
      cnt.resize(sn);
      PCP_HIP_TRY(ctx, hipMemcpyAsync(cnt.data(), ctx->view_count.p, sn * 4, hipMemcpyDeviceToHost, ctx->stream));
      PCP_HIP_TRY(ctx, hipStreamSynchronize(ctx->stream));
      for (size_t j = 0; j < sn; ++j) out_count[perm[j]] = cnt[j];
    }
  }
  return PCP_OK;
}

int pcp_colorize(pcp_context *ctx, uint8_t *out_rgb, uint8_t *out_has) {
  int rc = check_ready(ctx, "pcp_colorize", true);
  if (rc != PCP_OK) return rc;
  if ((rc = check_masks(ctx, 0, ctx->n_frames)) != PCP_OK) return rc;
  pcp_colour_reset(ctx);
  if ((rc = pcp_depth_pass(ctx, 0, ctx->n_frames)) != PCP_OK) return rc;
  uint32_t *result = nullptr;
  if ((rc = begin_result(ctx, &result)) != PCP_OK) return rc;
  if ((rc = labels_begin(ctx)) != PCP_OK) return rc;
  if ((rc = colour_pass_impl(ctx, 0, ctx->n_frames, true, result)) != PCP_OK) return rc;
  if ((rc = labels_end(ctx)) != PCP_OK) return rc;
  return end_result(ctx, out_rgb, out_has);
}

int pcp_colorize_from_depth(pcp_context *ctx, uint8_t *out_rgb, uint8_t *out_has) {
  int rc = check_ready(ctx, "pcp_colorize_from_depth", true);
  if (rc != PCP_OK) return rc;
  pcp_colour_reset(ctx);
  uint32_t *result = nullptr;
  if ((rc = begin_result(ctx, &result)) != PCP_OK) return rc;
  if ((rc = labels_begin(ctx)) != PCP_OK) return rc;
  if ((rc = colour_pass_impl(ctx, 0, ctx->n_frames, true, result)) != PCP_OK) return rc;
  if ((rc = labels_end(ctx)) != PCP_OK) return rc;
  return end_result(ctx, out_rgb, out_has);
}

int pcp_colour_smooth_local(pcp_context *ctx, float radius, int64_t *out_has_count) {
  if (!ctx) return PCP_ERR_INVALID;
  if (!smooth_radius_ok(radius))
    return set_error(ctx, PCP_ERR_INVALID, "pcp_colour_smooth_local: radius %g outside (0, 1]", static_cast<double>(radius));
  if (!ctx->colour_result_live)
    return set_error(ctx, PCP_ERR_STATE, "pcp_colour_smooth_local: no result (call pcp_colorize / pcp_colour_finalise)");
  if (out_has_count) *out_has_count = 0;
  if (ctx->n == 0) return PCP_OK;
  PCP_HIP_TRY(ctx, hipSetDevice(ctx->device));
  const uint32_t *src = ctx->rgba2[ctx->rgba_cur].p;
  uint32_t *dst = nullptr;
  int rc = begin_result(ctx, &dst);
  if (rc != PCP_OK) return rc;
  if ((rc = colour_smooth_words(ctx, radius, src, dst, out_has_count)) != PCP_OK) return rc;
  return end_result(ctx, nullptr, nullptr);
}

int pcp_download_result_packed(pcp_context *ctx, uint32_t *out_rgba) {
  if (!ctx) return PCP_ERR_INVALID;
  if (!ctx->colour_result_live)
    return set_error(ctx, PCP_ERR_STATE, "pcp_download_result_packed: no result (call pcp_colorize / pcp_colour_finalise)");
  if (!out_rgba && ctx->n > 0) return set_error(ctx, PCP_ERR_INVALID, "pcp_download_result_packed: NULL output");
  if (ctx->n > 0)
    PCP_HIP_TRY(ctx, hipMemcpyAsync(out_rgba, ctx->rgba2[ctx->rgba_cur].p, static_cast<size_t>(ctx->n) * 4,
                                    hipMemcpyDeviceToHost, ctx->stream));
  PCP_HIP_TRY(ctx, hipStreamSynchronize(ctx->stream));
  return PCP_OK;
}

int pcp_download_result_packed_async(pcp_context *ctx, uint32_t *out_rgba) {
  if (!ctx) return PCP_ERR_INVALID;
  if (!ctx->colour_result_live)
    return set_error(ctx, PCP_ERR_STATE, "pcp_download_result_packed_async: no result (call pcp_colorize / pcp_colour_finalise)");
  if (!out_rgba && ctx->n > 0) return set_error(ctx, PCP_ERR_INVALID, "pcp_download_result_packed_async: NULL output");
  const int32_t cur = ctx->rgba_cur;
  PCP_HIP_TRY(ctx, hipStreamWaitEvent(ctx->copy_stream, ctx->result_ready[cur], 0));
  if (ctx->n > 0)
    PCP_HIP_TRY(ctx, hipMemcpyAsync(out_rgba, ctx->rgba2[cur].p, static_cast<size_t>(ctx->n) * 4, hipMemcpyDeviceToHost,
                                    ctx->copy_stream));
  PCP_HIP_TRY(ctx, hipEventRecord(ctx->copy_done[cur], ctx->copy_stream));
  ctx->copy_pending[cur] = true;
  return PCP_OK;
}

int pcp_download_wait_previous(pcp_context *ctx) {
  if (!ctx) return PCP_ERR_INVALID;
  const int32_t prev = ctx->rgba_cur ^ 1;
  if (ctx->copy_pending[prev]) PCP_HIP_TRY(ctx, hipEventSynchronize(ctx->copy_done[prev]));
  return PCP_OK;
}

int pcp_tile_mask_density(pcp_context *ctx, double *kept_fraction) {
  if (!ctx || !kept_fraction) return PCP_ERR_INVALID;
  if (!ctx->tile_mask.p || ctx->n_tiles == 0 || ctx->n_frames == 0)
    return set_error(ctx, PCP_ERR_STATE, "pcp_tile_mask_density: no masks (call pcp_depth_pass)");
  std::vector<uint32_t> h(static_cast<size_t>(ctx->n_tiles) * ctx->mask_words);
  PCP_HIP_TRY(ctx, hipMemcpyAsync(h.data(), ctx->tile_mask.p, h.size() * 4, hipMemcpyDeviceToHost, ctx->stream));
  PCP_HIP_TRY(ctx, hipStreamSynchronize(ctx->stream));
  uint64_t bits = 0;
  for (uint32_t w : h) bits += static_cast<uint64_t>(__builtin_popcount(w));
  *kept_fraction = static_cast<double>(bits) / (static_cast<double>(ctx->n_tiles) * ctx->n_frames);
  return PCP_OK;
}

int pcp_tile_masks(pcp_context *ctx, int64_t *tiles, int32_t *mask_words, uint32_t *out_words) {
  if (!ctx) return PCP_ERR_INVALID;
  if (!ctx->tile_mask.p || ctx->n_tiles == 0 || ctx->n_frames == 0)
    return set_error(ctx, PCP_ERR_STATE, "pcp_tile_masks: no masks (call pcp_depth_pass)");
  if (tiles) *tiles = ctx->n_tiles;
  if (mask_words) *mask_words = ctx->mask_words;
  if (out_words) {
    PCP_HIP_TRY(ctx, hipMemcpyAsync(out_words, ctx->tile_mask.p, static_cast<size_t>(ctx->n_tiles) * ctx->mask_words * 4,
                                    hipMemcpyDeviceToHost, ctx->stream));
    PCP_HIP_TRY(ctx, hipStreamSynchronize(ctx->stream));
  }
  return PCP_OK;
}

int pcp_colour_result_device(pcp_context *ctx, void **device_ptr, int64_t *n_words) {
  if (!ctx) return PCP_ERR_INVALID;
  if (!ctx->colour_result_live)
    return set_error(ctx, PCP_ERR_STATE, "pcp_colour_result_device: no result (call pcp_colorize / pcp_colour_finalise)");
  if (device_ptr) *device_ptr = ctx->rgba2[ctx->rgba_cur].p;
  if (n_words) *n_words = ctx->n;
  return PCP_OK;
}

int pcp_set_label_fusion(pcp_context *ctx, int32_t enable) {
  if (!ctx) return PCP_ERR_INVALID;
  const bool on = enable != 0;
  if (on != ctx->label_fusion && ctx->colour_state_live)
    return set_error(ctx, PCP_ERR_STATE, "pcp_set_label_fusion: a top-5 accumulation is live (its lists %s the masks): "
                     "call pcp_colour_reset first", ctx->label_fusion ? "hold" : "do not hold");
  ctx->label_fusion = on;
  return PCP_OK;
}

int pcp_colour_labels(pcp_context *ctx, uint8_t *out_label, uint8_t *out_hits, uint8_t *out_views) {
  if (!ctx) return PCP_ERR_INVALID;
  if (!ctx->labels_live)
    return set_error(ctx, PCP_ERR_STATE, "pcp_colour_labels: no labels (pcp_set_label_fusion(1), then pcp_colorize / "
                     "pcp_colorize_from_depth / pcp_colour_finalise)");
  const int64_t n = ctx->n;
  if (n == 0 || !(out_label || out_hits || out_views)) return PCP_OK;
  PCP_HIP_TRY(ctx, hipSetDevice(ctx->device));
  const size_t sn = static_cast<size_t>(n);
  PCP_HIP_TRY(ctx, ctx->s_keep.ensure(4 * sn + 16));
  uint8_t *d_label = ctx->s_keep.p, *d_hits = d_label + sn, *d_views = d_hits + sn;
  hipLaunchKernelGGL(k_unpack_labels, dim3(blocks_for(n)), dim3(kBlock), 0, ctx->stream, ctx->labels.p, n,
                     out_label ? d_label : nullptr, out_hits ? d_hits : nullptr, out_views ? d_views : nullptr);
  PCP_HIP_TRY(ctx, hipGetLastError());
  if (out_label) PCP_HIP_TRY(ctx, hipMemcpyAsync(out_label, d_label, sn, hipMemcpyDeviceToHost, ctx->stream));
  if (out_hits) PCP_HIP_TRY(ctx, hipMemcpyAsync(out_hits, d_hits, sn, hipMemcpyDeviceToHost, ctx->stream));
  if (out_views) PCP_HIP_TRY(ctx, hipMemcpyAsync(out_views, d_views, sn, hipMemcpyDeviceToHost, ctx->stream));
  PCP_HIP_TRY(ctx, hipStreamSynchronize(ctx->stream));
  return PCP_OK;
}

int pcp_colour_labels_device(pcp_context *ctx, void **device_ptr, int64_t *n_words) {
  if (!ctx) return PCP_ERR_INVALID;
  if (!ctx->labels_live)
    return set_error(ctx, PCP_ERR_STATE, "pcp_colour_labels_device: no labels (pcp_set_label_fusion(1), then pcp_colorize / "
                     "pcp_colorize_from_depth / pcp_colour_finalise)");
  if (device_ptr) *device_ptr = ctx->labels.p;
  if (n_words) *n_words = ctx->n;
  return PCP_OK;
}

int pcp_selftest_arithmetic(pcp_context *ctx, int64_t samples, uint64_t seed, int64_t *mismatches_fp64,
                            int64_t *mismatches_fp32) {
  if (!ctx) return PCP_ERR_INVALID;
  if (!ctx->have_camera) return set_error(ctx, PCP_ERR_STATE, "pcp_selftest_arithmetic: pcp_set_camera has not been called");
  PCP_HIP_TRY(ctx, hipSetDevice(ctx->device));
  if (samples < 0) return set_error(ctx, PCP_ERR_INVALID, "pcp_selftest_arithmetic: negative sample count");
  PCP_HIP_TRY(ctx, ctx->s_counter.ensure(4));
  unsigned long long *bad = ctx->s_counter.p;
  PCP_HIP_TRY(ctx, hipMemsetAsync(bad, 0, 16, ctx->stream));
  if (samples > 0)
    hipLaunchKernelGGL(k_selftest_div64, dim3(blocks_for(samples)), dim3(kBlock), 0, ctx->stream, samples, seed, bad);
  hipLaunchKernelGGL(k_selftest_div32, dim3((1u << 24) / kBlock), dim3(kBlock), 0, ctx->stream, ctx->dcam, bad + 1);
  PCP_HIP_TRY(ctx, hipGetLastError());
  unsigned long long h[2] = {0, 0};
  PCP_HIP_TRY(ctx, hipMemcpyAsync(h, bad, 16, hipMemcpyDeviceToHost, ctx->stream));
  PCP_HIP_TRY(ctx, hipStreamSynchronize(ctx->stream));
  if (mismatches_fp64) *mismatches_fp64 = static_cast<int64_t>(h[0]);
  if (mismatches_fp32) *mismatches_fp32 = static_cast<int64_t>(h[1]);
  return PCP_OK;
}

}
```

### pointcloudprocessor_amd/csrc/pcp_context.hip

```cpp
#include <algorithm>
#include <cfloat>
#include <cmath>
#include <cstdlib>
#include <new>
#include <vector>

#include "pcp_internal.hpp"
#include "pcp_scan.hpp"

namespace pcp {

static thread_local std::string g_error;

int set_error(const pcp_context *ctx, int code, const char *fmt, ...) {
  char buf[1024];
  va_list ap;
  va_start(ap, fmt);
  vsnprintf(buf, sizeof(buf), fmt, ap);
  va_end(ap);
  if (ctx)
    ctx->error = buf;
  else
    g_error = buf;
  return code;
}

void set_global_error(const char *fmt, ...) {
  char buf[1024];
  va_list ap;
  va_start(ap, fmt);
  vsnprintf(buf, sizeof(buf), fmt, ap);
  va_end(ap);
  g_error = buf;
}

LaunchTimer::LaunchTimer(pcp_context *c, int32_t kernel) : ctx(c) {
  if (!ctx || !ctx->timing) return;
  auto grab = [&](hipEvent_t &e) {
    if (!ctx->event_pool.empty()) {
      e = ctx->event_pool.back();
      ctx->event_pool.pop_back();
      return true;
    }
    return hipEventCreate(&e) == hipSuccess;
  };
  if (!grab(ev.start)) return;
  if (!grab(ev.stop)) {
    ctx->event_pool.push_back(ev.start);
    return;
  }
  ev.kernel = kernel;
  active = hipEventRecord(ev.start, ctx->stream) == hipSuccess;
}

LaunchTimer::~LaunchTimer() {
  if (!active) return;
  (void)hipEventRecord(ev.stop, ctx->stream);
  ctx->pending.push_back(ev);
}

int drain_timing(pcp_context *ctx) {
  for (auto &p : ctx->pending) {
    float ms = 0.0f;
    hipError_t e = hipEventSynchronize(p.stop);
    if (e == hipSuccess) e = hipEventElapsedTime(&ms, p.start, p.stop);
    if (e == hipSuccess && p.kernel >= 0 && p.kernel < PCP_K_COUNT) {
      ctx->slots[p.kernel].total_ms += ms;
      ctx->slots[p.kernel].launches += 1;
    }
    ctx->event_pool.push_back(p.start);
    ctx->event_pool.push_back(p.stop);
  }
  ctx->pending.clear();
  return PCP_OK;
}

static void rotation_from_quaternion(const pcp_pose &p, double R[3][3]) {
  const double tx = 2.0 * p.qx, ty = 2.0 * p.qy, tz = 2.0 * p.qz;
  const double twx = tx * p.qw, twy = ty * p.qw, twz = tz * p.qw;
  const double txx = tx * p.qx, txy = ty * p.qx, txz = tz * p.qx;
  const double tyy = ty * p.qy, tyz = tz * p.qy, tzz = tz * p.qz;
  R[0][0] = 1.0 - (tyy + tzz);
  R[0][1] = txy - twz;
  R[0][2] = txz + twy;
  R[1][0] = txy + twz;
  R[1][1] = 1.0 - (txx + tzz);
  R[1][2] = tyz - twx;
  R[2][0] = txz - twy;
  R[2][1] = tyz + twx;
  R[2][2] = 1.0 - (txx + tyy);
}

static void invert_affine_f32(const float in[12], float out[12]) {
  const float a = in[0], b = in[1], c = in[2];
  const float d = in[4], e = in[5], f = in[6];
  const float g = in[8], h = in[9], i = in[10];
  const float k00 = e * i - f * h, k10 = h * c - i * b, k20 = b * f - c * e;
  const float det = k00 * a + (k10 * d + k20 * g);
  const float inv = 1.0f / det;
  const float L[3][3] = {{k00 * inv, k10 * inv, k20 * inv},
                         {(f * g - d * i) * inv, (i * a - g * c) * inv, (c * d - a * f) * inv},
                         {(d * h - e * g) * inv, (g * b - h * a) * inv, (a * e - b * d) * inv}};
  for (int r = 0; r < 3; ++r) {
    out[4 * r + 0] = L[r][0];
    out[4 * r + 1] = L[r][1];
    out[4 * r + 2] = L[r][2];
    out[4 * r + 3] = (-L[r][0]) * in[3] + ((-L[r][1]) * in[7] + (-L[r][2]) * in[11]);
  }
}

static void matrices_from_pose(const pcp_pose &pose, const double *T, float w2c[12], float c2w[12]) {
  double R[3][3];
  rotation_from_quaternion(pose, R);
  const double t[3] = {pose.x, pose.y, pose.z};
  if (!T) {
    for (int r = 0; r < 3; ++r) {
      const double a0 = R[0][r], a1 = R[1][r], a2 = R[2][r];
      w2c[4 * r + 0] = static_cast<float>(a0);
      w2c[4 * r + 1] = static_cast<float>(a1);
      w2c[4 * r + 2] = static_cast<float>(a2);
      w2c[4 * r + 3] = static_cast<float>(-((a0 * t[0] + a1 * t[1]) + a2 * t[2]));
      c2w[4 * r + 0] = static_cast<float>(R[r][0]);
      c2w[4 * r + 1] = static_cast<float>(R[r][1]);
      c2w[4 * r + 2] = static_cast<float>(R[r][2]);
      c2w[4 * r + 3] = static_cast<float>(t[r]);
    }
    return;
  }
  for (int r = 0; r < 3; ++r)
    for (int c = 0; c < 4; ++c) {
      double s = (R[r][0] * T[0 * 4 + c] + R[r][1] * T[1 * 4 + c]) + R[r][2] * T[2 * 4 + c];
      if (c == 3) s = s + t[r] * T[15];
      c2w[4 * r + c] = static_cast<float>(s);
    }
  invert_affine_f32(c2w, w2c);
}

constexpr int kUpBlock = 256;

__device__ __forceinline__ uint32_t spread10(uint32_t v) {
  v &= 0x3ffu;
  v = (v | (v << 16)) & 0x030000ffu;
  v = (v | (v << 8)) & 0x0300f00fu;
  v = (v | (v << 4)) & 0x030c30c3u;
  v = (v | (v << 2)) & 0x09249249u;
  return v;
}

__global__ __launch_bounds__(kUpBlock) void k_up_bbox(const float *__restrict__ x, const float *__restrict__ y,
                                                     const float *__restrict__ z, int64_t n,
                                                     float *__restrict__ partial ,
                                                     unsigned long long *__restrict__ nonfinite) {
  __shared__ float sh[6][kUpBlock / 64];
  float lo[3] = {FLT_MAX, FLT_MAX, FLT_MAX}, hi[3] = {-FLT_MAX, -FLT_MAX, -FLT_MAX};
  uint32_t bad = 0;
  for (int64_t i = static_cast<int64_t>(blockIdx.x) * kUpBlock + threadIdx.x; i < n; i += static_cast<int64_t>(gridDim.x) * kUpBlock) {
    const float v[3] = {x[i], y[i], z[i]};
    bool fin = true;
#pragma unroll
    for (int a = 0; a < 3; ++a) {
// ... 511 lines not shown
  ctx->g_start.release();
  ctx->g_occ.release();
  ctx->g_occ_rank.release();
  ctx->g_order.release();
  ctx->g_xyz.release();
  ctx->m_tmp.release();
  ctx->s_dist.release();
  ctx->css_dist.release();
  ctx->s_kth.release();
  ctx->css_words.release();
  ctx->m_state.release();
  ctx->slp_table.release();
  ctx->c_perm.release();
  ctx->m_flag.release();
  ctx->intensity.release();
  for (auto &lane : ctx->hpr_lane) lane.release();
  if (ctx->hpr_fork) (void)hipEventDestroy(ctx->hpr_fork);
  for (auto &e : ctx->hpr_join)
    if (e) (void)hipEventDestroy(e);
  ctx->hull_bits.release();
  ctx->nid_pts.release();
  ctx->nid_chunk_kf.release();
  ctx->nid_hist.release();
  ctx->m_sums.release();
  ctx->c_index.release();
  ctx->c_xyz.release();
  ctx->c_mark.release();
  ctx->c_where.release();
  ctx->c_xyz2.release();
  ctx->v_bitmap.release();
  ctx->v_occ.release();
  ctx->v_rank.release();
  ctx->v_plane.release();
  ctx->v_vox.release();
  ctx->v_offsets.release();
  ctx->mls_xyz.release();
  ctx->mls_normal.release();
  ctx->mls_curv.release();
  ctx->mls_index.release();
  ctx->mls_alt_xyz.release();
  ctx->mls_alt_normal.release();
  ctx->mls_alt_curv.release();
  ctx->mls_alt_index.release();
  if (ctx->readback) (void)hipHostFree(ctx->readback);
  if (ctx->own_stream) (void)hipStreamDestroy(ctx->own_stream);
  delete ctx;
}

const char *pcp_last_error(const pcp_context *ctx) { return ctx ? ctx->error.c_str() : g_error.c_str(); }

int pcp_set_stream(pcp_context *ctx, void *hip_stream) {
  if (!ctx) return PCP_ERR_INVALID;
  PCP_HIP_TRY(ctx, hipStreamSynchronize(ctx->stream));
  ctx->stream = hip_stream ? static_cast<hipStream_t>(hip_stream) : ctx->own_stream;
  return PCP_OK;
}

int pcp_synchronize(pcp_context *ctx) {
  if (!ctx) return PCP_ERR_INVALID;
  for (hipStream_t us : ctx->upload_stream)
    if (us) PCP_HIP_TRY(ctx, hipStreamSynchronize(us));
  std::fill(ctx->image_pending.begin(), ctx->image_pending.end(), uint8_t(0));
  PCP_HIP_TRY(ctx, hipStreamSynchronize(ctx->stream));
  PCP_HIP_TRY(ctx, hipStreamSynchronize(ctx->copy_stream));
  ctx->copy_pending[0] = ctx->copy_pending[1] = false;
  return PCP_OK;
}

void pcp_default_camera(pcp_camera *cam) {
  cam->fx = 4818.200388954926;
  cam->fy = 4819.10345841615;
  cam->cx = 2032.4178620390019;
  cam->cy = 1535.1895959282901;
  cam->k1 = 0.003043514741045163;
  cam->k2 = 0.06634739187544138;
  cam->p1 = -0.000217681797407554;
  cam->p2 = -0.0006654964142658197;
  cam->k3 = 0.0;
  cam->image_width = 4096;
  cam->image_height = 3000;
  cam->cull_width = 4096;
  cam->cull_height = 3000;
}

void pcp_default_cull_params(pcp_cull_params *p) {
  p->enable_depth_buffer_culling = 1;
  p->downsample_factor = 14;
  p->depth_slack = 0.05;
  p->cull_mode = PCP_CULL_ZBUFFER;
  p->match_mode = PCP_MATCH_ROUNDTRIP;
  p->hpr_flip_radius = 90000.0;
}

void pcp_default_mls_params(pcp_mls_params *p) {
  p->search_radius = 0.03;
  p->sqr_gauss_param = 0.0009;
  p->polynomial_order = 2;
  p->compute_normals = 1;
  p->upsampling = 3;
  p->vgd_iterations = 4;
  p->vgd_voxel_size = 0.001f;
  p->sor_mean_k = 60;
  p->sor_std_mul = 0.7;
}

int pcp_set_camera(pcp_context *ctx, const pcp_camera *cam, const pcp_cull_params *cull) {
  if (!ctx || !cam) return set_error(ctx, PCP_ERR_INVALID, "pcp_set_camera: NULL argument");
  pcp_cull_params cp;
  if (cull)
    cp = *cull;
  else
    pcp_default_cull_params(&cp);
  if (cam->image_width <= 0 || cam->image_height <= 0 || cam->cull_width <= 0 || cam->cull_height <= 0)
    return set_error(ctx, PCP_ERR_INVALID, "pcp_set_camera: image / cull size must be positive");
  if (cp.downsample_factor <= 0) return set_error(ctx, PCP_ERR_INVALID, "pcp_set_camera: downsample_factor must be > 0");
  if (cp.cull_mode != PCP_CULL_ZBUFFER && cp.cull_mode != PCP_CULL_HPR_CANDIDATES && cp.cull_mode != PCP_CULL_HPR)
    return set_error(ctx, PCP_ERR_INVALID, "pcp_set_camera: unknown cull_mode %d", cp.cull_mode);
  if (cp.cull_mode == PCP_CULL_HPR && !(cp.hpr_flip_radius > 0.0 && cp.hpr_flip_radius < 1e300))
    return set_error(ctx, PCP_ERR_INVALID, "pcp_set_camera: hpr_flip_radius must be positive and finite");
  if (cp.match_mode != PCP_MATCH_IDENTITY && cp.match_mode != PCP_MATCH_ROUNDTRIP && cp.match_mode != PCP_MATCH_RADIUS)
    return set_error(ctx, PCP_ERR_INVALID, "pcp_set_camera: unknown match_mode %d", cp.match_mode);
  if (cam->cull_width > (1 << 24) || cam->cull_height > (1 << 24))
    return set_error(ctx, PCP_ERR_INVALID, "pcp_set_camera: cull size above 2^24 is not supported");
  if (static_cast<int64_t>(cam->image_width) * cam->image_height >= (int64_t(1) << 31))
    return set_error(ctx, PCP_ERR_INVALID, "pcp_set_camera: image too large for int32 pixel indices");
  ctx->camera = *cam;
  ctx->cull = cp;
  DevCamera &d = ctx->dcam;
  d.fx = cam->fx;
  d.fy = cam->fy;
  d.cx = cam->cx;
  d.cy = cam->cy;
  d.k1 = cam->k1;
  d.k2 = cam->k2;
  d.p1 = cam->p1;
  d.p2 = cam->p2;
  d.k3 = cam->k3;
  d.slack = cp.depth_slack;
  d.ds = cp.downsample_factor;
  d.ds_f = static_cast<float>(cp.downsample_factor);
  d.ds_rcp = 1.0f / d.ds_f;
  d.ds_fast = (d.ds_f >= 0x1p-20f && d.ds_f <= 0x1p20f) ? 1 : 0;
  if (const char *e = std::getenv("PCP_DISABLE_FAST_EXACT")) d.ds_fast = (e[0] == '1') ? 0 : d.ds_fast;
  d.img_w = cam->image_width;
  d.img_h = cam->image_height;
  d.cull_w = cam->cull_width;
  d.cull_h = cam->cull_height;
  d.img_wd = static_cast<double>(cam->image_width);
  d.img_hd = static_cast<double>(cam->image_height);
  d.cull_wf = static_cast<float>(cam->cull_width);
  d.cull_hf = static_cast<float>(cam->cull_height);
  d.mw = cam->cull_width / cp.downsample_factor;
  d.mh = cam->cull_height / cp.downsample_factor;
  d.cull_mode = cp.cull_mode == PCP_CULL_HPR ? PCP_CULL_HPR_CANDIDATES : cp.cull_mode;
  d.match_mode = cp.match_mode;
  d.cull_wd = static_cast<double>(cam->cull_width);
  d.cull_hd = static_cast<double>(cam->cull_height);
  {
    const double eps = static_cast<double>(1e-5f);
    d.match_r2 = static_cast<float>(eps * eps);
  }
  d.enable_zbuf = (cp.enable_depth_buffer_culling && cp.cull_mode == PCP_CULL_ZBUFFER) ? 1 : 0;
  d.pretest = 1;
  d.qfx = static_cast<float>(cam->fx);
  d.qfy = static_cast<float>(cam->fy);
  d.qcx = static_cast<float>(cam->cx);
  d.qcy = static_cast<float>(cam->cy);
  d.qk1 = static_cast<float>(cam->k1);
  d.qk2 = static_cast<float>(cam->k2);
  d.qk3 = static_cast<float>(cam->k3);
  d.qp1 = static_cast<float>(cam->p1);
  d.qp2 = static_cast<float>(cam->p2);
  {
    const float ds = static_cast<float>(cp.downsample_factor);
    const bool hpr = cp.cull_mode != PCP_CULL_ZBUFFER;
    const float cw = hpr ? static_cast<float>(d.cull_w) : ds * static_cast<float>(d.enable_zbuf ? d.mw : d.cull_w);
    const float ch = hpr ? static_cast<float>(d.cull_h) : ds * static_cast<float>(d.enable_zbuf ? d.mh : d.cull_h);
    d.u_lo = -(ds + 0.5f);
    d.v_lo = -(ds + 0.5f);
    d.u_hi = std::max(cw, static_cast<float>(d.img_w)) + 0.5f;
    d.v_hi = std::max(ch, static_cast<float>(d.img_h)) + 0.5f;
  }
  if (const char *e = std::getenv("PCP_DISABLE_PRETEST")) d.pretest = (e[0] == '1') ? 0 : 1;

  ctx->have_camera = true;
  for (hipStream_t us : ctx->upload_stream)
    if (us) (void)hipStreamSynchronize(us);
  std::fill(ctx->image_pending.begin(), ctx->image_pending.end(), uint8_t(0));
  ctx->image_set.assign(ctx->image_set.size(), 0);
  ctx->mask_set.assign(ctx->mask_set.size(), 0);
  std::fill(ctx->depth_valid.begin(), ctx->depth_valid.end(), uint8_t(0));
  ctx->hull_valid.clear();
  ctx->depth_accum.release();
  ctx->depth_accum_live = false;
  ctx->colour_state_live = false;
  ctx->colour_result_live = false;
  ctx->labels_live = false;
  return PCP_OK;
}

int pcp_upload_cloud(pcp_context *ctx, const float *x, const float *y, const float *z, int64_t n) {
  if (!ctx) return PCP_ERR_INVALID;
  if (n < 0 || n >= (int64_t(1) << 31)) return set_error(ctx, PCP_ERR_INVALID, "pcp_upload_cloud: n=%lld out of range", (long long)n);
  if (n > 0 && (!x || !y || !z)) return set_error(ctx, PCP_ERR_INVALID, "pcp_upload_cloud: NULL coordinate array");
  return store_cloud(ctx, x, y, z, n);
}

int pcp_upload_cloud_aos(pcp_context *ctx, const void *points, int64_t n, int64_t stride_bytes) {
  if (!ctx) return PCP_ERR_INVALID;
  if (n < 0 || n >= (int64_t(1) << 31)) return set_error(ctx, PCP_ERR_INVALID, "pcp_upload_cloud_aos: n out of range");
  if (stride_bytes < 12) return set_error(ctx, PCP_ERR_INVALID, "pcp_upload_cloud_aos: stride must be >= 12 bytes");
  if (n > 0 && !points) return set_error(ctx, PCP_ERR_INVALID, "pcp_upload_cloud_aos: NULL points");
  if (stride_bytes % 4 == 0 && (reinterpret_cast<uintptr_t>(points) & 3u) == 0)
    return store_cloud(ctx, nullptr, nullptr, nullptr, n, points, stride_bytes);
  std::vector<float> x(static_cast<size_t>(n)), y(static_cast<size_t>(n)), z(static_cast<size_t>(n));
  const uint8_t *base = static_cast<const uint8_t *>(points);
  for (int64_t i = 0; i < n; ++i) {
    float v[3];
    std::memcpy(v, base + i * stride_bytes, 12);
    x[static_cast<size_t>(i)] = v[0];
    y[static_cast<size_t>(i)] = v[1];
    z[static_cast<size_t>(i)] = v[2];
  }
  return store_cloud(ctx, x.data(), y.data(), z.data(), n);
}

int pcp_upload_cloud_from_result(pcp_context *dst, pcp_context *src, int64_t *out_n) {
  if (!dst || !src) return dst ? set_error(dst, PCP_ERR_INVALID, "pcp_upload_cloud_from_result: NULL source context") : PCP_ERR_INVALID;
  if (out_n) *out_n = 0;
  if (dst->device != src->device)
    return set_error(dst, PCP_ERR_INVALID, "pcp_upload_cloud_from_result: the contexts are on GPUs %d and %d (one GPU only)", dst->device,
                     src->device);
  if (!src->mls_result_live)
    return set_error(dst, PCP_ERR_STATE, "pcp_upload_cloud_from_result: the source context holds no smoothing result (pcp_mls_process*, "
                     "pcp_cloud_smooth, pcp_mls_stream_next, pcp_cloud_smooth_stream_next since its latest upload)");
  const int64_t m = src->mls_count;
  const float *rows = src->mls_xyz.p;
  if (m > 0 && !rows) return set_error(dst, PCP_ERR_STATE, "pcp_upload_cloud_from_result: the source result has no rows on the device");
  PCP_HIP_TRY(dst, hipSetDevice(dst->device));
  if (dst != src && m > 0) {
    if (!src->handoff) PCP_HIP_TRY(dst, hipEventCreateWithFlags(&src->handoff, hipEventDisableTiming));
    PCP_HIP_TRY(dst, hipEventRecord(src->handoff, src->stream));
    PCP_HIP_TRY(dst, hipStreamWaitEvent(dst->stream, src->handoff, 0));
  }
  const int rc = store_cloud(dst, nullptr, nullptr, nullptr, m, rows, 12, true, dst == src);
  if (rc == PCP_OK && out_n) *out_n = m;
  return rc;
}

int64_t pcp_cloud_size(const pcp_context *ctx) { return ctx ? ctx->n : -1; }

int pcp_pose_to_matrices(const pcp_pose *pose, const double *T_opt, float w2c[12], float c2w[12]) {
  if (!pose || !w2c || !c2w) {
    set_global_error("pcp_pose_to_matrices: NULL argument");
    return PCP_ERR_INVALID;
  }
  matrices_from_pose(*pose, T_opt, w2c, c2w);
  return PCP_OK;
}

int pcp_set_frames(pcp_context *ctx, const pcp_pose *poses, int32_t n_frames, const double *T_opt,
                   int32_t T_opt_stride) {
  if (!ctx) return PCP_ERR_INVALID;
  if (n_frames < 0 || (n_frames > 0 && !poses)) return set_error(ctx, PCP_ERR_INVALID, "pcp_set_frames: bad poses");
  if (T_opt && T_opt_stride != 0 && T_opt_stride != 16)
    return set_error(ctx, PCP_ERR_INVALID, "pcp_set_frames: T_opt_stride must be 0 (global) or 16 (per keyframe)");
  PCP_HIP_TRY(ctx, hipSetDevice(ctx->device));
  for (hipStream_t us : ctx->upload_stream)
    if (us) PCP_HIP_TRY(ctx, hipStreamSynchronize(us));
  std::fill(ctx->image_pending.begin(), ctx->image_pending.end(), uint8_t(0));
  ctx->poses.assign(poses, poses + n_frames);
  ctx->hframes.resize(static_cast<size_t>(n_frames));
  for (int32_t f = 0; f < n_frames; ++f) {
    DevFrame &d = ctx->hframes[static_cast<size_t>(f)];
    const double *T = T_opt ? T_opt + static_cast<int64_t>(T_opt_stride) * f : nullptr;
    matrices_from_pose(poses[f], T, d.w2c, d.c2w);
    invert_affine_f32(d.c2w, d.c2w_inv);
    d.pad_[0] = d.pad_[1] = d.pad_[2] = d.pad_[3] = 0.0f;
    d.px = poses[f].x;
    d.py = poses[f].y;
    d.pz = poses[f].z;
    {
      double g[3][3];
      for (int a = 0; a < 3; ++a)
        for (int b = 0; b < 3; ++b) {
          g[a][b] = 0.0;
          for (int k = 0; k < 3; ++k) g[a][b] += static_cast<double>(d.w2c[4 * k + a]) * static_cast<double>(d.w2c[4 * k + b]);
        }
      double rowmax = 0.0;
      for (int a = 0; a < 3; ++a) rowmax = std::max(rowmax, std::fabs(g[a][0]) + std::fabs(g[a][1]) + std::fabs(g[a][2]));
      d.norm_bound = std::sqrt(rowmax) * (1.0 + 1e-9);
    }
  }
  {
    bool bounded = true;
    for (int32_t f = 0; f < n_frames; ++f)
      for (int k = 0; k < 12; ++k) bounded = bounded && std::fabs(ctx->hframes[static_cast<size_t>(f)].w2c[k]) <= 0x1p40f;
    ctx->dcam.frames_bounded = bounded ? 1 : 0;
  }
  PCP_HIP_TRY(ctx, ctx->frames.ensure(static_cast<size_t>(n_frames) + 1));
  if (n_frames > 0)
    PCP_HIP_TRY(ctx, hipMemcpyAsync(ctx->frames.p, ctx->hframes.data(), sizeof(DevFrame) * n_frames,
                                    hipMemcpyHostToDevice, ctx->stream));
  PCP_HIP_TRY(ctx, hipStreamSynchronize(ctx->stream));
  ctx->n_frames = n_frames;
  ctx->image_set.assign(static_cast<size_t>(n_frames), 0);
// ... 49 lines not shown
```

### pointcloudprocessor_amd/csrc/pcp_device.hpp

```cpp
#pragma once

#include <hip/hip_runtime.h>

#include <cfloat>
#include <cstdint>

#include "pcp_internal.hpp"

namespace pcp {

__device__ __forceinline__ void xform(const float *__restrict__ m, float x, float y, float z, float &xc, float &yc,
                                      float &zc) {
  xc = x * m[0] + (y * m[1] + (z * m[2] + m[3]));
  yc = x * m[4] + (y * m[5] + (z * m[6] + m[7]));
  zc = x * m[8] + (y * m[9] + (z * m[10] + m[11]));
}

__device__ __forceinline__ void divide_xy_by_z(float xc, float yc, float zc, double &xn, double &yn, bool finite_sure = false) {
  const double X = xc, Y = yc, Z = zc;
  if (finite_sure || (xc - xc) + (yc - yc) + (zc - zc) == 0.0f) {
    double r = __builtin_amdgcn_rcp(Z);
    double e = __builtin_fma(-Z, r, 1.0);
    r = __builtin_fma(r, e, r);
    e = __builtin_fma(-Z, r, 1.0);
    r = __builtin_fma(r, e, r);
    const double qx = X * r, qy = Y * r;
    const double rx = __builtin_fma(-Z, qx, X), ry = __builtin_fma(-Z, qy, Y);
    xn = __builtin_fma(rx, r, qx);
    yn = __builtin_fma(ry, r, qy);
  } else {
    xn = X / Z;
    yn = Y / Z;
  }
}

template <bool kShortDiv = true>
__device__ __forceinline__ void project_uv(const DevCamera &c, float xc, float yc, float zc, double &u, double &v,
                                           bool finite_sure = false) {
  double xn, yn;
  if (kShortDiv && c.ds_fast) {
    if (finite_sure)
      divide_xy_by_z(xc, yc, zc, xn, yn, true);
    else
      divide_xy_by_z(xc, yc, zc, xn, yn);
  } else {
    xn = static_cast<double>(xc) / static_cast<double>(zc);
    yn = static_cast<double>(yc) / static_cast<double>(zc);
  }
  const double x2 = xn * xn;
  const double y2 = yn * yn;
  const double r2 = x2 + y2;
  const double r4 = r2 * r2;
  const double r6 = r2 * r4;
  const double rc = ((1.0 + c.k1 * r2) + c.k2 * r4) + c.k3 * r6;
  const double t1 = (2.0 * xn) * yn;
  const double t2 = r2 + 2.0 * x2;
  const double t3 = r2 + 2.0 * y2;
  const double xd = (rc * xn + c.p1 * t1) + c.p2 * t2;
  const double yd = (rc * yn + c.p1 * t3) + c.p2 * t1;
  u = c.fx * xd + c.cx;
  v = c.fy * yd + c.cy;
}

__device__ __forceinline__ float div_by_ds(const DevCamera &c, float x) {
  if (c.ds_fast) {
    float q = x * c.ds_rcp;
    float e = __builtin_fmaf(-c.ds_f, q, x);
    q = __builtin_fmaf(e, c.ds_rcp, q);
    e = __builtin_fmaf(-c.ds_f, q, x);
    return __builtin_fmaf(e, c.ds_rcp, q);
  }
  return x / c.ds_f;
}
__device__ __forceinline__ int32_t cell_of_quotient(float q, float size) {
  return ((q > -1.0f) & (q < size)) ? static_cast<int32_t>(q) : -1;
}

template <bool kShortDiv = true>
__device__ __forceinline__ int32_t cull_cell(const DevCamera &c, double u, double v) {
  if (c.cull_mode == PCP_CULL_HPR_CANDIDATES) {
    return (u > -1.0 && u < c.cull_wd && v > -1.0 && v < c.cull_hd) ? -2 : -1;
  }
  const float cxf = kShortDiv ? div_by_ds(c, static_cast<float>(u)) : static_cast<float>(u) / c.ds_f;
  const float cyf = kShortDiv ? div_by_ds(c, static_cast<float>(v)) : static_cast<float>(v) / c.ds_f;
  const int32_t cx = cell_of_quotient(cxf, c.cull_wf), cy = cell_of_quotient(cyf, c.cull_hf);
  if ((cx < 0) | (cy < 0)) return -1;
  return ((cx < c.mw) & (cy < c.mh)) ? cy * c.mw + cx : (c.enable_zbuf ? -1 : -2);
}

__device__ __forceinline__ int32_t colour_pixel(const DevCamera &c, double u, double v) {
  if (!(u > -1.0 && u < c.img_wd && v > -1.0 && v < c.img_hd)) return -1;
  return static_cast<int32_t>(v) * c.img_w + static_cast<int32_t>(u);
}

__device__ __forceinline__ double range64(float xc, float yc, float zc) {
  const double X = xc, Y = yc, Z = zc;
  return sqrt((X * X + Y * Y) + Z * Z);
}

__device__ __forceinline__ bool surely_rejected(const DevCamera &c, float xc, float yc, float zc) {
  const float rz = __builtin_amdgcn_rcpf(zc);
  const float xn = xc * rz, yn = yc * rz;
  const float x2 = xn * xn, y2 = yn * yn;
  const float r2 = x2 + y2, r4 = r2 * r2, r6 = r2 * r4;
  const float rc = __builtin_fmaf(c.qk3, r6, __builtin_fmaf(c.qk2, r4, __builtin_fmaf(c.qk1, r2, 1.0f)));
  const float ra = __builtin_fmaf(fabsf(c.qk3), r6, __builtin_fmaf(fabsf(c.qk2), r4, __builtin_fmaf(fabsf(c.qk1), r2, 1.0f)));
  const float t1 = 2.0f * xn * yn;
  const float t2 = __builtin_fmaf(2.0f, x2, r2), t3 = __builtin_fmaf(2.0f, y2, r2);
  const float at1 = fabsf(t1);
  const float xd = __builtin_fmaf(c.qp2, t2, __builtin_fmaf(c.qp1, t1, rc * xn));
  const float yd = __builtin_fmaf(c.qp2, t1, __builtin_fmaf(c.qp1, t3, rc * yn));
  const float sx = __builtin_fmaf(fabsf(c.qp2), t2, __builtin_fmaf(fabsf(c.qp1), at1, ra * fabsf(xn)));
  const float sy = __builtin_fmaf(fabsf(c.qp2), at1, __builtin_fmaf(fabsf(c.qp1), t3, ra * fabsf(yn)));
  const float u = __builtin_fmaf(c.qfx, xd, c.qcx), v = __builtin_fmaf(c.qfy, yd, c.qcy);
  constexpr float kErr = 1.52587890625e-05f;
  const float eu = kErr * __builtin_fmaf(fabsf(c.qfx), sx, fabsf(c.qcx));
  const float ev = kErr * __builtin_fmaf(fabsf(c.qfy), sy, fabsf(c.qcy));
  const float over = fmaxf(fmaxf(c.u_lo - (u + eu), (u - eu) - c.u_hi), fmaxf(c.v_lo - (v + ev), (v - ev) - c.v_hi));
  return over > 0.0f;
}

struct Projected {
  float xc, yc, zc;
  int32_t cell;
  int32_t pixel;
};

template <bool kPretest = true, bool kShortDiv = true>
__device__ __forceinline__ Projected project_point(const DevCamera &c, const float *__restrict__ m, float x, float y,
                                                   float z, bool pretest_here = true, bool finite_sure = false) {
  Projected p;
  xform(m, x, y, z, p.xc, p.yc, p.zc);
  p.cell = -1;
  p.pixel = -1;
  if (p.zc > 0.0f && !(kPretest && pretest_here && c.pretest && surely_rejected(c, p.xc, p.yc, p.zc))) {
    double u, v;
    project_uv<kShortDiv>(c, p.xc, p.yc, p.zc, u, v, finite_sure);
    p.cell = cull_cell<kShortDiv>(c, u, v);
    p.pixel = colour_pixel(c, u, v);
  }
  return p;
}

__device__ __forceinline__ bool keep_rule(const DevCamera &c, const Projected &p, const uint32_t *__restrict__ depth) {
  if (!c.enable_zbuf) return p.cell != -1;
  if (p.cell < 0) return false;
  const double r = range64(p.xc, p.yc, p.zc);
  const double lim = static_cast<double>(__uint_as_float(depth[p.cell])) + c.slack;
  return !(r > lim);
}

__device__ __forceinline__ bool roundtrip_sample(const DevCamera &c, const DevFrame &fr, float wx0, float wy0, float wz0,
                                                 float &xc, float &yc, float &zc) {
  float wx, wy, wz;
  xform(fr.c2w, xc, yc, zc, wx, wy, wz);
  const float dx = wx - wx0, dy = wy - wy0, dz = wz - wz0;
  float d2 = dx * dx;
  d2 += dy * dy;
  d2 += dz * dz;
  if (!(d2 < c.match_r2)) return false;
  const float *m = fr.c2w_inv;
  xc = (m[0] * wx + m[1] * wy) + (m[2] * wz + m[3]);
  yc = (m[4] * wx + m[5] * wy) + (m[6] * wz + m[7]);
  zc = (m[8] * wx + m[9] * wy) + (m[10] * wz + m[11]);
  return true;
}

__device__ __forceinline__ bool roundtrip_sample_moved(const DevCamera &c, const DevFrame &fr, float wx0, float wy0, float wz0,
                                                       float &xc, float &yc, float &zc, float e2, uint32_t &moved) {
  float wx, wy, wz;
  xform(fr.c2w, xc, yc, zc, wx, wy, wz);
  const float dx = wx - wx0, dy = wy - wy0, dz = wz - wz0;
  float d2 = dx * dx;
  d2 += dy * dy;
  d2 += dz * dz;
  moved += (d2 <= e2) ? 0u : 1u;
  if (!(d2 < c.match_r2)) return false;
  const float *m = fr.c2w_inv;
  xc = (m[0] * wx + m[1] * wy) + (m[2] * wz + m[3]);
  yc = (m[4] * wx + m[5] * wy) + (m[6] * wz + m[7]);
  zc = (m[8] * wx + m[9] * wy) + (m[10] * wz + m[11]);
  return true;
}

__device__ __forceinline__ float final_score(float xc, float yc, float zc, double px, double py, double pz) {
  const double dx = static_cast<double>(xc) - px;
  const double dy = static_cast<double>(yc) - py;
  const double dz = static_cast<double>(zc) - pz;
  const double sq = (dx * dx + dy * dy) + dz * dz;
  const double y0 = __builtin_amdgcn_rsq(sq);
  const double e = __builtin_fma(-(sq * y0), y0, 1.0);
  const double y = __builtin_fma(y0 * e, __builtin_fma(0.375, e, 0.5), y0);
  const double t = (dz * y + 1.0) * 0.5;
  const float lo = static_cast<float>(t - 4e-15), hi = static_cast<float>(t + 4e-15);
  float o = lo;
  const bool settled = (sq > 0x1p-100) & (sq < 0x1p100) & (lo == hi);
  if (!settled) {
    const double cosA = sq > 0.0 ? dz / sqrt(sq) : dz;
    o = static_cast<float>((cosA + 1.0) / 2.0);
  }
  o = 0.2f + 0.8f * o;
  const float dist = sqrtf((xc * xc + yc * yc) + zc * zc);
  const float diff = fabsf(dist - 2.0f);
  float nd = diff / 2.0f;
  nd = nd < 1.0f ? nd : 1.0f;
  float d = 1.0f - nd;
  d = 0.2f + 0.8f * d;
  return static_cast<float>(static_cast<double>(o + d) / 2.0);
}

struct Top5 {
  float s0, s1, s2, s3, s4;
  uint32_t c0, c1, c2, c3, c4;
  int32_t f0, f1, f2, f3, f4;
  int32_t count;
  __device__ __forceinline__ void init() {
    s0 = s1 = s2 = s3 = s4 = -1.0f;
    c0 = c1 = c2 = c3 = c4 = 0u;
    f0 = f1 = f2 = f3 = f4 = -1;
    count = 0;
  }
  __device__ __forceinline__ void insert(float s, uint32_t c, int32_t f) {
    count += 1;
    if (s > s4) {
      s4 = s; c4 = c; f4 = f;
      if (s4 > s3) {
        float ts = s3; s3 = s4; s4 = ts;
        uint32_t tc = c3; c3 = c4; c4 = tc;
        int32_t tf = f3; f3 = f4; f4 = tf;
        if (s3 > s2) {
          ts = s2; s2 = s3; s3 = ts;
          tc = c2; c2 = c3; c3 = tc;
          tf = f2; f2 = f3; f3 = tf;
          if (s2 > s1) {
            ts = s1; s1 = s2; s2 = ts;
            tc = c1; c1 = c2; c2 = tc;
            tf = f1; f1 = f2; f2 = tf;
            if (s1 > s0) {
              ts = s0; s0 = s1; s1 = ts;
              tc = c0; c0 = c1; c1 = tc;
              tf = f0; f0 = f1; f1 = tf;
            }
          }
        }
      }
    }
  }
  __device__ __forceinline__ uint32_t finalise() const {
    float total = 0.0f, r = 0.0f, g = 0.0f, b = 0.0f;
    const float ss[5] = {s0, s1, s2, s3, s4};
    const uint32_t cc[5] = {c0, c1, c2, c3, c4};
    const int32_t ff[5] = {f0, f1, f2, f3, f4};
#pragma unroll
    for (int k = 0; k < 5; ++k) {
      if (ff[k] >= 0) {
        const float s = ss[k];
        r += static_cast<float>((cc[k] >> 16) & 0xffu) * s;
        g += static_cast<float>((cc[k] >> 8) & 0xffu) * s;
        b += static_cast<float>(cc[k] & 0xffu) * s;
        total += s;
      }
    }
    if (f0 < 0) return 0u;
    const uint32_t ri = static_cast<uint32_t>(r / total) & 0xffu;
    const uint32_t gi = static_cast<uint32_t>(g / total) & 0xffu;
    const uint32_t bi = static_cast<uint32_t>(b / total) & 0xffu;
    const uint32_t has = (ri | gi | bi) ? 1u : 0u;
    return ri | (gi << 8) | (bi << 16) | (has << 24);
  }
  __device__ __forceinline__ uint32_t labels(uint32_t &bad) const {
    const float ss[5] = {s0, s1, s2, s3, s4};
    const uint32_t cc[5] = {c0, c1, c2, c3, c4};
    const int32_t ff[5] = {f0, f1, f2, f3, f4};
    uint64_t num = 0;
    uint32_t den = 0u, hits = 0u, views = 0u;
#pragma unroll
    for (int k = 0; k < 5; ++k) {
      if (ff[k] >= 0) {
        const float s = ss[k];
        if (!(s >= 0x1p-3f && s < 2.0f)) bad = 1u;
        const uint32_t S = static_cast<uint32_t>(s * 0x1p26f);
        const uint32_t m = cc[k] >> 24;
        num += static_cast<uint64_t>(m) * S;
        den += S;
        hits += m == 255u ? 1u : 0u;
        views += 1u;
      }
    }
    if (views == 0u) return 0u;
    uint32_t q = 0u;
#pragma unroll
    for (uint32_t bit = 128u; bit != 0u; bit >>= 1) {
      const uint32_t t = q | bit;
      if (static_cast<uint64_t>(t) * den <= num) q = t;
    }
    return q | (hits << 8) | (views << 16);
  }
};

}
```

### pointcloudprocessor_amd/csrc/pcp_internal.hpp

```cpp
#pragma once

#include <hip/hip_runtime.h>

#include <cstdarg>
#include <cstdint>
#include <chrono>
#include <cstdio>
#include <cstring>
#include <string>
#include <vector>

#include "pcp_hip.h"

namespace pcp {

struct DevCamera {
  double fx, fy, cx, cy;
  double k1, k2, p1, p2, k3;
  double slack;
  float ds_f;
  double img_wd, img_hd;
  float cull_wf, cull_hf;
  float ds_rcp;
  int32_t ds_fast;
  int32_t ds;
  int32_t img_w, img_h;
  int32_t cull_w, cull_h;
  int32_t mw, mh;
  int32_t enable_zbuf;
  int32_t cull_mode;
  int32_t match_mode;
  double cull_wd, cull_hd;
  float match_r2;
  int32_t pretest;
  int32_t frames_bounded;
  float qfx, qfy, qcx, qcy;
  float qk1, qk2, qk3, qp1, qp2;
  float u_lo, u_hi, v_lo, v_hi;
};

struct DevFrame {
  float w2c[12];
  float c2w[12];
  double px, py, pz;
  double norm_bound;
  float c2w_inv[12];
  float pad_[4];
};
static_assert(sizeof(DevFrame) == 192, "DevFrame layout");

constexpr int kTopM = 5;

struct TimingSlot {
  double total_ms = 0.0;
  int64_t launches = 0;
};

struct PendingEvent {
  hipEvent_t start, stop;
  int32_t kernel;
};

struct AllocTally {
  double seconds = 0.0, bytes = 0.0;
};
inline AllocTally &alloc_tally() {
  static AllocTally t;
  return t;
}
struct AllocClock {
  std::chrono::steady_clock::time_point t0 = std::chrono::steady_clock::now();
  ~AllocClock() { alloc_tally().seconds += std::chrono::duration<double>(std::chrono::steady_clock::now() - t0).count(); }
};

template <typename T>
struct DevBuf {
  T *p = nullptr;
  size_t count = 0;
  hipError_t ensure(size_t n) {
    if (n <= count && p) return hipSuccess;
    AllocClock clk;
    if (p) (void)hipFree(p);
    p = nullptr;
    count = 0;
    if (n == 0) return hipSuccess;
    hipError_t e = hipMalloc(reinterpret_cast<void **>(&p), n * sizeof(T));
    if (e == hipSuccess) {
      count = n;
      alloc_tally().bytes += static_cast<double>(n) * sizeof(T);
    }
    return e;
  }
  void release() {
    if (!p) return;
    AllocClock clk;
    (void)hipFree(p);
    p = nullptr;
    count = 0;
  }
};

struct AsciiParseSlot {
  void *stage = nullptr, *res_h = nullptr;
  size_t stage_bytes = 0;
  DevBuf<uint8_t> text;
  DevBuf<int32_t> end, tiles;
  DevBuf<uint32_t> out;
  DevBuf<unsigned long long> res;
  hipEvent_t staged = nullptr, parsed = nullptr, drained = nullptr;
  bool staged_live = false, parsed_live = false, drained_live = false;
};

struct HprLane {
  hipStream_t own_stream = nullptr;
  hipStream_t stream = nullptr;
  unsigned long long seq = 0;
  DevBuf<int32_t> index, i32, tiles;
  DevBuf<double> f64, cells_d, cont;
  DevBuf<uint8_t> state;
  DevBuf<unsigned long long> stats;
  void *readback = nullptr;
  bool busy = false;
  int32_t frame = -1;
  uint8_t *d_flags = nullptr;
  uint32_t *hull_plane = nullptr;
  uint32_t bit = 0;
  void release() {
    index.release();
    i32.release();
    tiles.release();
    f64.release();
    cells_d.release();
    cont.release();
    state.release();
    stats.release();
    if (readback) (void)hipHostFree(readback);
    readback = nullptr;
    if (own_stream) (void)hipStreamDestroy(own_stream);
    own_stream = nullptr;
  }
};

}

struct pcp_context {
  int32_t device = 0;
  hipStream_t own_stream = nullptr;
  hipStream_t stream = nullptr;
  void *readback = nullptr;
  static constexpr size_t kReadbackBytes = 65536;
  mutable std::string error;

  bool have_camera = false;
  pcp_camera camera{};
  pcp_cull_params cull{};
  pcp::DevCamera dcam{};

  int64_t n = 0;
  int64_t nonfinite_points = 0;
  pcp::DevBuf<float> xyz;
  pcp::DevBuf<float> sxyz;
  pcp::DevBuf<int32_t> perm;
  pcp::DevBuf<int32_t> inv_perm;
  std::vector<float> host_min = {0, 0, 0}, host_max = {0, 0, 0};

  int32_t n_frames = 0;
  std::vector<pcp_pose> poses;
  std::vector<pcp::DevFrame> hframes;
  pcp::DevBuf<pcp::DevFrame> frames;
  pcp::DevBuf<uint32_t> images;
  std::vector<uint8_t> image_set, mask_set;
  static constexpr int kUploadLanes = 2;
  hipStream_t upload_stream[kUploadLanes] = {nullptr, nullptr};
  pcp::DevBuf<uint8_t> upload_stage[kUploadLanes];
  pcp::DevBuf<uint8_t> jpeg_planes[kUploadLanes];
  std::vector<hipEvent_t> image_event;
  std::vector<uint8_t> image_pending;
  std::vector<uint8_t> image_lane;
  std::vector<uint64_t> image_seq;
  bool lane_must_wait[kUploadLanes] = {false, false};
  uint64_t upload_seq = 0;
  uint64_t upload_turn = 0;
  hipEvent_t texels_idle = nullptr;
  bool texels_touched = false;
  bool adjust_images = false;
  float saturation_scale = 1.0f, brightness_scale = 1.0f;
  pcp::DevBuf<int32_t> hsv_tables;

  pcp::DevBuf<uint32_t> depth;
  pcp::DevBuf<unsigned long long> depth_sq;
  std::vector<uint8_t> depth_valid;
  bool depth_from_batch = false;
  pcp::DevBuf<uint32_t> depth_accum;
  bool depth_accum_live = false;

  int64_t n_tiles = 0;
  pcp::DevBuf<float> tile_sphere;
  pcp::DevBuf<uint32_t> tile_mask, group_mask;
  pcp::DevBuf<uint32_t> tile_inside;
  int32_t mask_words = 0;
  pcp::DevBuf<int32_t> tile_work, tile_order, work_hist;
  bool tile_order_live = false;

  pcp::DevBuf<float> top_score;
  pcp::DevBuf<uint32_t> top_rgb;
  pcp::DevBuf<int32_t> top_frame;
  pcp::DevBuf<int32_t> view_count;
  pcp::DevBuf<uint32_t> rgba2[2];
  int32_t rgba_cur = 0;
  hipStream_t copy_stream = nullptr;
  hipEvent_t result_ready[2] = {nullptr, nullptr}, copy_done[2] = {nullptr, nullptr};
  bool copy_pending[2] = {false, false};
  bool colour_state_live = false;
  bool colour_result_live = false;
  bool label_fusion = false;
  bool labels_live = false;
  pcp::DevBuf<uint32_t> labels;

  bool match_live = false;
  double match_e = 0.0, match_rc = 0.0;
  float match_e2 = 0.0f;
  int64_t match_a = 0;
  int64_t match_entries = 0;
  pcp::DevBuf<uint8_t> match_in_a;
  pcp::DevBuf<int32_t> match_list;
  pcp::DevBuf<int64_t> match_off;
  pcp::DevBuf<int32_t> match_cols;
  pcp::DevBuf<unsigned long long> match_moved;

  pcp::DevBuf<int32_t> s_cell, s_pixel;
  pcp::DevBuf<float> s_range, s_cam;
  pcp::DevBuf<uint8_t> s_keep;
  pcp::DevBuf<uint32_t> s_u32;
  pcp::DevBuf<unsigned long long> s_counter;
  pcp::DevBuf<int32_t> s_tiles;

  static constexpr int kHprMaxLanes = 8;
  pcp::HprLane hpr_lane[kHprMaxLanes];
  int32_t hpr_last_lane = 0;
  hipEvent_t hpr_fork = nullptr, hpr_join[kHprMaxLanes] = {};
  pcp::DevBuf<uint32_t> hull_bits;
  std::vector<uint8_t> hull_valid;
  int64_t hpr_stats[10] = {0, 0, 0, 0, 0, 0, 0, 0, 0, 0};
  bool hpr_stats_pending = false;

  pcp::DevBuf<int32_t> g_cell, g_rank, g_start, g_order;
  pcp::DevBuf<unsigned long long> g_occ;
  pcp::DevBuf<int32_t> g_occ_rank;
  pcp::DevBuf<float> g_xyz;
  pcp::DevBuf<float> m_tmp;
  pcp::DevBuf<float> s_dist;
  pcp::DevBuf<double> m_state;
  double slp_radius = 0.05, slp_step = 0.01;
  pcp::DevBuf<float> slp_table;
  double slp_table_of[2] = {0.0, 0.0};
  pcp::DevBuf<int32_t> c_perm;
  pcp::DevBuf<uint8_t> m_flag;
  pcp::DevBuf<double> m_sums;
  pcp::DevBuf<int32_t> c_index;
  int32_t sor_partial_slab = -1, sor_partial_slabs = -1;
  bool sor_distances_live = false;
  pcp::DevBuf<uint8_t> c_mark;
  pcp::DevBuf<int32_t> c_where;
  pcp::DevBuf<float> c_xyz, c_xyz2;
  pcp::DevBuf<uint32_t> v_bitmap;
  pcp::DevBuf<int32_t> v_offsets;
  pcp::DevBuf<uint32_t> v_occ;
  pcp::DevBuf<int32_t> v_rank;
  pcp::DevBuf<unsigned long long> v_plane;
  pcp::DevBuf<int64_t> v_vox;
  pcp::DevBuf<float> mls_xyz, mls_normal, mls_curv;
  pcp::DevBuf<int32_t> mls_index;
  pcp::DevBuf<float> mls_alt_xyz, mls_alt_normal, mls_alt_curv;
  pcp::DevBuf<int32_t> mls_alt_index;
  int64_t mls_count = 0;
  bool mls_result_live = false;
  hipEvent_t handoff = nullptr;
  pcp::DevBuf<uint8_t> cc_out;
  pcp::DevBuf<uint8_t> ascii_in, ascii_len, ascii_text;
  pcp::DevBuf<unsigned long long> ascii_tiles;
  pcp::AsciiParseSlot parse_slot[2];
  hipStream_t parse_up = nullptr, parse_down = nullptr;
  std::vector<uint8_t> vgd_blob;
  std::vector<int64_t> vgd_chunks;
  int64_t vgd_next = -1;
  std::vector<uint8_t> css_blob;
  std::vector<int64_t> css_chunks;
  int64_t css_next = -1;
  pcp::DevBuf<float> css_dist;
  pcp::DevBuf<float> s_kth;
  pcp::DevBuf<uint32_t> css_words;
  bool css_building = false;
  double css_ball = 0.0;
  double sor_redo_fraction = 0.0;

  pcp::DevBuf<float> intensity;
  bool have_intensity = false;
  pcp::DevBuf<float> nid_pts;
  pcp::DevBuf<int32_t> nid_chunk_kf;
  pcp::DevBuf<double> nid_hist;
  int64_t nid_chunks = 0, nid_points = 0;
  int32_t nid_frames = 0;
  int32_t nid_hist_bins = 0;

  bool timing = false;
  pcp::TimingSlot slots[PCP_K_COUNT];
// ... 106 lines not shown
```

### pointcloudprocessor_amd/host_build.py

```python
from __future__ import annotations

import os
import subprocess

from . import _build

HOST = os.path.join(os.path.dirname(os.path.abspath(__file__)), "host")
BIN = os.path.join(HOST, "bin")
ROCM = os.environ.get("ROCM_PATH", "/opt/rocm")

TARGETS = {
    "pcp_shim_selftest": ["shim_selftest.cpp"],
    "PointCloudProcessor": ["main.cpp"],
    "image_dump": ["image_dump.cpp"],
    "format_selftest": ["format_selftest.cpp"],
    "parse_selftest": ["parse_selftest.cpp"],
}


def build(force: bool = False) -> dict:
    os.makedirs(BIN, exist_ok=True)
    out = {}
    for name, srcs in TARGETS.items():
        exe = os.path.join(BIN, name)
        deps = [os.path.join(HOST, s) for s in srcs] + [os.path.join(HOST, "pcp_shim.hpp"), os.path.join(HOST, "pcp_multi.hpp"), os.path.join(HOST, "pcd_io.hpp"), os.path.join(HOST, "image_io.hpp"), os.path.join(HOST, "pcd_device_reader.hpp"),
                                                       os.path.join(_build.CSRC, "pcp_ascii_parse.hpp"), os.path.join(_build.CSRC, "pcp_ascii.hpp"),
                                                       os.path.join(_build.INCLUDE, "pcp_hip.h")]
        deps = [d for d in deps if os.path.exists(d)]
        stale = force or not os.path.exists(exe) or any(os.path.getmtime(d) > os.path.getmtime(exe) for d in deps)
        if stale:
            extra = os.environ.get("PCP_HOST_CXXFLAGS", "").split()
            multi = ["-D__HIP_PLATFORM_AMD__", "-isystem", os.path.join(ROCM, "include")] if name == "PointCloudProcessor" else []
            multi_libs = ["-L", os.path.join(ROCM, "lib"), "-lrccl", "-lamdhip64", "-Wl,-rpath," + os.path.join(ROCM, "lib")] \
                if name == "PointCloudProcessor" else []
            cmd = ["g++", "-std=c++17", "-O2", "-pthread", "-Wall", "-Wextra"] + extra + multi + ["-I", _build.INCLUDE, "-I", HOST] + [
                os.path.join(HOST, s) for s in srcs] + ["-L", _build.LIB_DIR, "-lpcp_hip"] + multi_libs + [
                                                        "-lz", "-Wl,-rpath,$ORIGIN/../../lib", "-o", exe]
            proc = subprocess.run(cmd, capture_output=True, text=True)
            if proc.returncode != 0:
                raise RuntimeError(f"g++ failed for {name}:\n{proc.stderr[-3000:]}")
        out[name] = exe
    return out
```

Measured before the change: 1.875 million.

## Add bit-exact short projection path for tame distortion in depth and colour passes

```diff
diff --git a/include/pcp_hip.h b/include/pcp_hip.h
--- a/include/pcp_hip.h
+++ b/include/pcp_hip.h
@@ -246,6 +246,8 @@
 int pcp_sor_distances(pcp_context *ctx, int64_t capacity, float *out_distance);
 int pcp_selftest_arithmetic(pcp_context *ctx, int64_t samples, uint64_t seed, int64_t *mismatches_fp64,
                             int64_t *mismatches_fp32);
+int pcp_selftest_visit_forms(pcp_context *ctx, int64_t samples, uint64_t seed, int64_t *mismatches_uv, int64_t *mismatches_cell,
+                             int64_t *mismatches_sqrt, int32_t *short_distortion);
 
 #ifdef __cplusplus
 }
diff --git a/pointcloudprocessor_amd/_build.py b/pointcloudprocessor_amd/_build.py
--- a/pointcloudprocessor_amd/_build.py
+++ b/pointcloudprocessor_amd/_build.py
@@ -12,7 +12,7 @@
 
 SOURCES = ["pcp_context.hip", "pcp_colour.hip", "pcp_mls.hip", "pcp_nid.hip", "pcp_hpr.hip", "pcp_colour_smooth.hip", "pcp_match.hip", "pcp_jpeg.hip",
            "pcp_stream_colour.hip", "pcp_ascii.hip", "pcp_ascii_parse.hip"]
-HEADERS = ["pcp_internal.hpp", "pcp_device.hpp", "pcp_scan.hpp", "pcp_hsv.hpp", "pcp_exact.hpp", "pcp_ascii.hpp", "pcp_ascii_parse.hpp"]
+HEADERS = ["pcp_internal.hpp", "pcp_device.hpp", "pcp_scan.hpp", "pcp_hsv.hpp", "pcp_exact.hpp", "pcp_ascii.hpp", "pcp_ascii_parse.hpp", "pcp_visit_forms.hpp"]
 
 HIPCC_FLAGS = [
     "--offload-arch=gfx950",
diff --git a/pointcloudprocessor_amd/capi.py b/pointcloudprocessor_amd/capi.py
--- a/pointcloudprocessor_amd/capi.py
+++ b/pointcloudprocessor_amd/capi.py
@@ -811,6 +811,12 @@
         self._check(self.lib.pcp_selftest_arithmetic(self.h, C.c_int64(samples), C.c_uint64(seed), C.byref(a), C.byref(b)))
         return a.value, b.value
 
+    def selftest_visit_forms(self, samples: int = 1 << 24, seed: int = 1):
+        a, b, c, f = C.c_int64(), C.c_int64(), C.c_int64(), C.c_int32()
+        self._check(self.lib.pcp_selftest_visit_forms(self.h, C.c_int64(samples), C.c_uint64(seed), C.byref(a), C.byref(b), C.byref(c),
+                                                      C.byref(f)))
+        return a.value, b.value, c.value, bool(f.value)
+
     def tile_masks(self) -> np.ndarray:
         t, w = C.c_int64(), C.c_int32()
         self._check(self.lib.pcp_tile_masks(self.h, C.byref(t), C.byref(w), None))
diff --git a/pointcloudprocessor_amd/csrc/pcp_colour.hip b/pointcloudprocessor_amd/csrc/pcp_colour.hip
--- a/pointcloudprocessor_amd/csrc/pcp_colour.hip
+++ b/pointcloudprocessor_amd/csrc/pcp_colour.hip
@@ -22,8 +22,9 @@
   }
   return c;
 }
-inline bool is_common_camera(const DevCamera &c) {
-  return c.cull_mode == PCP_CULL_ZBUFFER && c.enable_zbuf == 1 && c.pretest == 1 && c.ds_fast == 1;
+inline bool is_common_camera(const pcp_context *ctx) {
+  const DevCamera &c = ctx->dcam;
+  return c.cull_mode == PCP_CULL_ZBUFFER && c.enable_zbuf == 1 && c.pretest == 1 && c.ds_fast == 1 && ctx->uv_tame;
 }
 
 struct ProjectOut {
@@ -384,12 +385,18 @@
       const int32_t f = (w << 5) + b;
       todo &= todo - 1u;
       const DevFrame &fr = frames[f];
-      const Projected p = project_point(cam, fr.w2c, px, py, pz, ((inside >> b) & 1u) == 0u, finite_sure);
-      const bool in_map = live && p.cell >= 0;
-      const bool cand = live && p.pixel >= 0 && (cam.enable_zbuf ? p.cell >= 0 : p.cell != -1);
-      if (__ballot(cand)) seen |= 1u << b;
+      const auto p = project_visit<true, kCommon>(cam, fr.w2c, px, py, pz, ((inside >> b) & 1u) == 0u, finite_sure);
+      bool in_map, cand;
+      if constexpr (kCommon) {
+        in_map = live && p.map_ok;
+        cand = in_map && p.image_ok;
+      } else {
+        in_map = live && p.cell >= 0;
+        cand = live && p.pixel >= 0 && (cam.enable_zbuf ? p.cell >= 0 : p.cell != -1);
+      }
+      if (__builtin_amdgcn_ballot_w64(cand)) seen |= 1u << b;
       settle_held();
-      if (cam.enable_zbuf && __ballot(in_map)) {
+      if (cam.enable_zbuf && __builtin_amdgcn_ballot_w64(in_map)) {
         unsigned long long *map = depth + static_cast<uint64_t>(static_cast<uint32_t>(f - depth_first_frame)) * static_cast<uint32_t>(cells);
         unsigned long long key = ~0ull, sbits = 0ull;
         if (in_map) {
@@ -469,6 +476,7 @@
                                                         uint32_t *__restrict__ rgba, int32_t flags_in,
                                                         const uint32_t *__restrict__ hull_bits_in, MatchArgs mb,
                                                         [[maybe_unused]] LabelOut lab) {
+  constexpr bool kShort = kCommon && kOneShot && kMatch == 2;
   DevCamera cam = common_camera<kCommon>(cam_in);
   if constexpr (kMatch == 1) cam.match_mode = PCP_MATCH_IDENTITY;
   if constexpr (kMatch == 2 || kMatch == 3) cam.match_mode = PCP_MATCH_ROUNDTRIP;
@@ -503,9 +511,12 @@
       const int32_t f = (w << 5) + __builtin_ctz(todo);
       todo &= todo - 1u;
       const DevFrame &fr = frames[f];
-      const Projected p = project_point<false>(cam, fr.w2c, px, py, pz, true, finite_sure);
-      const bool cand = live && p.pixel >= 0 && (cam.enable_zbuf ? p.cell >= 0 : p.cell != -1) &&
-                        ((hull_word >> (f & 31)) & 1u);
+      const auto p = project_visit<false, kShort>(cam, fr.w2c, px, py, pz, true, finite_sure);
+      bool cand;
+      if constexpr (kShort)
+        cand = live && p.image_ok && p.map_ok && ((hull_word >> (f & 31)) & 1u);
+      else
+        cand = live && p.pixel >= 0 && (cam.enable_zbuf ? p.cell >= 0 : p.cell != -1) && ((hull_word >> (f & 31)) & 1u);
       if (cand) {
         const uint32_t dbits = cam.enable_zbuf ? depth[static_cast<uint64_t>(static_cast<uint32_t>(f)) * static_cast<uint32_t>(cells) + static_cast<uint32_t>(p.cell)] : 0u;
         bool keep = true;
@@ -518,7 +529,7 @@
         }
         if (keep) {
           const uint32_t texel = images[static_cast<uint64_t>(static_cast<uint32_t>(f)) * static_cast<uint32_t>(image_px) + static_cast<uint32_t>(p.pixel)];
-          t.insert(final_score(sx, sy, sz, fr.px, fr.py, fr.pz), kLabel ? texel : texel & 0xffffffu, f);
+          t.insert(final_score<kShort>(sx, sy, sz, fr.px, fr.py, fr.pz), kLabel ? texel : texel & 0xffffffu, f);
         }
       }
     }
@@ -711,6 +722,54 @@
   if (wrong) atomicAdd(bad, static_cast<unsigned long long>(wrong));
 }
 
+__device__ __forceinline__ bool same_bits_f64(double a, double b) {
+  return (a != a && b != b) || __double_as_longlong(a) == __double_as_longlong(b);
+}
+__global__ __launch_bounds__(kBlock) void k_selftest_uv(DevCamera cam, int32_t tame, int64_t samples, uint64_t seed,
+                                                        unsigned long long *__restrict__ bad) {
+  const int64_t i = static_cast<int64_t>(blockIdx.x) * kBlock + threadIdx.x;
+  if (i >= samples) return;
+  const uint64_t a = mix64(seed ^ static_cast<uint64_t>(i) * 3u), b = mix64(a);
+  uint32_t bx = static_cast<uint32_t>(a), by = static_cast<uint32_t>(a >> 32), bz = static_cast<uint32_t>(b);
+  const uint32_t mode = static_cast<uint32_t>(b >> 32) & 3u;
+  if (mode != 0u) {
+    const uint32_t span = mode == 1u ? 12u : 40u;
+    bx = (bx & 0x807fffffu) | ((127u - span / 2u + (bx >> 23) % span) << 23);
+    by = (by & 0x807fffffu) | ((127u - span / 2u + (by >> 23) % span) << 23);
+    bz = (bz & 0x807fffffu) | ((127u - span / 2u + (bz >> 23) % span) << 23);
+  }
+  const float xc = __uint_as_float(bx), yc = __uint_as_float(by), zc = fabsf(__uint_as_float(bz));
+  if (!(zc > 0.0f)) return;
+  double u0, v0, u1, v1;
+  if (tame)
+    project_uv<true, true>(cam, xc, yc, zc, u0, v0);
+  else
+    project_uv<true, false>(cam, xc, yc, zc, u0, v0);
+  project_uv<true, false>(cam, xc, yc, zc, u1, v1);
+  if (!same_bits_f64(u0, u1) || !same_bits_f64(v0, v1)) atomicAdd(bad, 1ull);
+}
+
+__global__ __launch_bounds__(kBlock) void k_selftest_cell_sqrt(DevCamera cam, unsigned long long *__restrict__ bad_cell,
+                                                               unsigned long long *__restrict__ bad_sqrt) {
+  const uint32_t lane = blockIdx.x * kBlock + threadIdx.x;
+  uint32_t wrong_cell = 0u, wrong_sqrt = 0u;
+  for (uint32_t k = 0; k < 256u; ++k) {
+    const float q = __uint_as_float((k << 24) | lane);
+    const float qx[3] = {q, 0.5f, q}, qy[3] = {0.5f, q, q};
+#pragma unroll
+    for (int t = 0; t < 3; ++t) {
+      const int32_t old_cell = vf::map_cell_written(qx[t], qy[t], cam.cull_wf, cam.cull_hf, cam.mw, cam.mh);
+      int32_t cell;
+      const bool ok = vf::map_cell_short(qx[t], qy[t], vf::map_bound(cam.mw), vf::map_bound(cam.mh), cam.mw, cell);
+      if ((ok ? cell : -1) != old_cell) ++wrong_cell;
+    }
+    const float r0 = sqrt_rn(q), r1 = sqrtf(q);
+    if (!((r0 != r0 && r1 != r1) || __float_as_uint(r0) == __float_as_uint(r1))) ++wrong_sqrt;
+  }
+  if (wrong_cell) atomicAdd(bad_cell, static_cast<unsigned long long>(wrong_cell));
+  if (wrong_sqrt) atomicAdd(bad_sqrt, static_cast<unsigned long long>(wrong_sqrt));
+}
+
 __global__ __launch_bounds__(kBlock) void k_unpack_result(const uint32_t *__restrict__ packed, int64_t n,
                                                          uint8_t *__restrict__ rgb, uint8_t *__restrict__ has) {
   const int64_t i = static_cast<int64_t>(blockIdx.x) * kBlock + threadIdx.x;
@@ -1472,7 +1531,7 @@
   o.zc = out_xyz_cam ? ctx->s_cam.p + 2 * plane : nullptr;
   {
     LaunchTimer t(ctx, PCP_K_PROJECT);
-    hipLaunchKernelGGL(is_common_camera(ctx->dcam) ? k_project_frame<true> : k_project_frame<false>, dim3(blocks_for(div_up(n, 4))), dim3(kBlock), 0, ctx->stream, ctx->sxyz.p,
+    hipLaunchKernelGGL(is_common_camera(ctx) ? k_project_frame<true> : k_project_frame<false>, dim3(blocks_for(div_up(n, 4))), dim3(kBlock), 0, ctx->stream, ctx->sxyz.p,
                        ctx->sxyz.p + plane, ctx->sxyz.p + 2 * plane, n, ctx->dcam,
                        ctx->hframes[static_cast<size_t>(frame)], o);
     PCP_HIP_TRY(ctx, hipGetLastError());
@@ -1646,7 +1705,7 @@
     }
     {
       LaunchTimer t(ctx, PCP_K_DEPTH);
-      hipLaunchKernelGGL(is_common_camera(ctx->dcam) ? k_depth_pass<true> : k_depth_pass<false>,
+      hipLaunchKernelGGL(is_common_camera(ctx) ? k_depth_pass<true> : k_depth_pass<false>,
                          dim3(static_cast<uint32_t>(ctx->n_tiles)), dim3(64), 0, ctx->stream, ctx->sxyz.p,
                          ctx->sxyz.p + plane, ctx->sxyz.p + 2 * plane, ctx->n, ctx->dcam, ctx->frames.p, frame_begin,
                          frame_end, ctx->depth_sq.p, cells, frame_begin, ctx->tile_mask.p, ctx->tile_inside.p,
@@ -1809,7 +1868,7 @@
   const uint32_t *hull = ctx->cull.cull_mode == PCP_CULL_HPR ? ctx->hull_bits.p : static_cast<const uint32_t *>(nullptr);
   {
     LaunchTimer t(ctx, PCP_K_COLOUR);
-    const bool common = is_common_camera(ctx->dcam) && ctx->cull.cull_mode != PCP_CULL_HPR;
+    const bool common = is_common_camera(ctx) && ctx->cull.cull_mode != PCP_CULL_HPR;
     const bool label = ctx->label_fusion;
     const LabelOut lab{label ? ctx->labels.p : nullptr};
     auto kernel = label ? colour_pass_kernel<true>(common, ctx->dcam.match_mode, flags)
@@ -2097,4 +2156,27 @@
   return PCP_OK;
 }
 
-}
+int pcp_selftest_visit_forms(pcp_context *ctx, int64_t samples, uint64_t seed, int64_t *mismatches_uv, int64_t *mismatches_cell,
+                             int64_t *mismatches_sqrt, int32_t *short_distortion) {
+  if (!ctx) return PCP_ERR_INVALID;
+  if (!ctx->have_camera) return set_error(ctx, PCP_ERR_STATE, "pcp_selftest_visit_forms: pcp_set_camera has not been called");
+  PCP_HIP_TRY(ctx, hipSetDevice(ctx->device));
+  if (samples < 0) return set_error(ctx, PCP_ERR_INVALID, "pcp_selftest_visit_forms: negative sample count");
+  PCP_HIP_TRY(ctx, ctx->s_counter.ensure(4));
+  unsigned long long *bad = ctx->s_counter.p;
+  PCP_HIP_TRY(ctx, hipMemsetAsync(bad, 0, 32, ctx->stream));
+  if (samples > 0)
+    hipLaunchKernelGGL(k_selftest_uv, dim3(blocks_for(samples)), dim3(kBlock), 0, ctx->stream, ctx->dcam, ctx->uv_tame ? 1 : 0, samples, seed, bad);
+  hipLaunchKernelGGL(k_selftest_cell_sqrt, dim3((1u << 24) / kBlock), dim3(kBlock), 0, ctx->stream, ctx->dcam, bad + 1, bad + 2);
+  PCP_HIP_TRY(ctx, hipGetLastError());
+  unsigned long long h[3] = {0, 0, 0};
+  PCP_HIP_TRY(ctx, hipMemcpyAsync(h, bad, 24, hipMemcpyDeviceToHost, ctx->stream));
+  PCP_HIP_TRY(ctx, hipStreamSynchronize(ctx->stream));
+  if (mismatches_uv) *mismatches_uv = static_cast<int64_t>(h[0]);
+  if (mismatches_cell) *mismatches_cell = static_cast<int64_t>(h[1]);
+  if (mismatches_sqrt) *mismatches_sqrt = static_cast<int64_t>(h[2]);
+  if (short_distortion) *short_distortion = ctx->uv_tame ? 1 : 0;
+  return PCP_OK;
+}
+
+}
diff --git a/pointcloudprocessor_amd/csrc/pcp_context.hip b/pointcloudprocessor_amd/csrc/pcp_context.hip
--- a/pointcloudprocessor_amd/csrc/pcp_context.hip
+++ b/pointcloudprocessor_amd/csrc/pcp_context.hip
@@ -6,6 +6,7 @@
 #include <vector>
 
 #include "pcp_internal.hpp"
+#include "pcp_visit_forms.hpp"
 #include "pcp_scan.hpp"
 
 namespace pcp {
@@ -823,6 +824,8 @@
   d.cull_hf = static_cast<float>(cam->cull_height);
   d.mw = cam->cull_width / cp.downsample_factor;
   d.mh = cam->cull_height / cp.downsample_factor;
+  ctx->uv_tame = vf::distortion_is_tame(cam->p1, cam->p2);
+  if (const char *e = std::getenv("PCP_DISABLE_FAST_EXACT")) ctx->uv_tame = (e[0] == '1') ? false : ctx->uv_tame;
   d.cull_mode = cp.cull_mode == PCP_CULL_HPR ? PCP_CULL_HPR_CANDIDATES : cp.cull_mode;
   d.match_mode = cp.match_mode;
   d.cull_wd = static_cast<double>(cam->cull_width);
diff --git a/pointcloudprocessor_amd/csrc/pcp_device.hpp b/pointcloudprocessor_amd/csrc/pcp_device.hpp
--- a/pointcloudprocessor_amd/csrc/pcp_device.hpp
+++ b/pointcloudprocessor_amd/csrc/pcp_device.hpp
@@ -6,6 +6,7 @@
 #include <cstdint>
 
 #include "pcp_internal.hpp"
+#include "pcp_visit_forms.hpp"
 
 namespace pcp {
 
@@ -34,7 +35,7 @@
   }
 }
 
-template <bool kShortDiv = true>
+template <bool kShortDiv = true, bool kShortUV = false>
 __device__ __forceinline__ void project_uv(const DevCamera &c, float xc, float yc, float zc, double &u, double &v,
                                            bool finite_sure = false) {
   double xn, yn;
@@ -47,17 +48,22 @@
     xn = static_cast<double>(xc) / static_cast<double>(zc);
     yn = static_cast<double>(yc) / static_cast<double>(zc);
   }
-  const double x2 = xn * xn;
-  const double y2 = yn * yn;
-  const double r2 = x2 + y2;
-  const double r4 = r2 * r2;
-  const double r6 = r2 * r4;
-  const double rc = ((1.0 + c.k1 * r2) + c.k2 * r4) + c.k3 * r6;
-  const double t1 = (2.0 * xn) * yn;
-  const double t2 = r2 + 2.0 * x2;
-  const double t3 = r2 + 2.0 * y2;
-  const double xd = (rc * xn + c.p1 * t1) + c.p2 * t2;
-  const double yd = (rc * yn + c.p1 * t3) + c.p2 * t1;
+  double xd, yd;
+  if constexpr (kShortUV) {
+    vf::distort_short(vf::Distortion{c.k1, c.k2, c.k3, c.p1, c.p2}, xn, yn, xd, yd);
+  } else {
+    const double x2 = xn * xn;
+    const double y2 = yn * yn;
+    const double r2 = x2 + y2;
+    const double r4 = r2 * r2;
+    const double r6 = r2 * r4;
+    const double rc = ((1.0 + c.k1 * r2) + c.k2 * r4) + c.k3 * r6;
+    const double t1 = (2.0 * xn) * yn;
+    const double t2 = r2 + 2.0 * x2;
+    const double t3 = r2 + 2.0 * y2;
+    xd = (rc * xn + c.p1 * t1) + c.p2 * t2;
+    yd = (rc * yn + c.p1 * t3) + c.p2 * t1;
+  }
   u = c.fx * xd + c.cx;
   v = c.fy * yd + c.cy;
 }
@@ -142,6 +148,40 @@
   return p;
 }
 
+struct ShortVisit {
+  float xc, yc, zc;
+  int32_t cell, pixel;
+  bool map_ok, image_ok;
+};
+template <bool kPretest>
+__device__ __forceinline__ ShortVisit project_point_short(const DevCamera &c, const float *__restrict__ m, float x, float y, float z,
+                                                          bool pretest_here = true, bool finite_sure = false) {
+  ShortVisit p;
+  xform(m, x, y, z, p.xc, p.yc, p.zc);
+  p.cell = 0;
+  p.pixel = 0;
+  p.map_ok = p.image_ok = false;
+  const bool go = p.zc > 0.0f && !(kPretest && pretest_here && c.pretest && surely_rejected(c, p.xc, p.yc, p.zc));
+  if (!kPretest || __builtin_amdgcn_ballot_w64(go)) {
+    double u, v;
+    project_uv<true, true>(c, p.xc, p.yc, p.zc, u, v, finite_sure);
+    const bool cell_ok = vf::map_cell_short(div_by_ds(c, static_cast<float>(u)), div_by_ds(c, static_cast<float>(v)), vf::map_bound(c.mw),
+                                            vf::map_bound(c.mh), c.mw, p.cell);
+    p.map_ok = go & cell_ok;
+    p.image_ok = go & (u > -1.0) & (u < c.img_wd) & (v > -1.0) & (v < c.img_hd);
+    p.pixel = p.image_ok ? static_cast<int32_t>(v) * c.img_w + static_cast<int32_t>(u) : 0;
+  }
+  return p;
+}
+template <bool kPretest, bool kShort>
+__device__ __forceinline__ auto project_visit(const DevCamera &c, const float *__restrict__ m, float x, float y, float z,
+                                              bool pretest_here = true, bool finite_sure = false) {
+  if constexpr (kShort)
+    return project_point_short<kPretest>(c, m, x, y, z, pretest_here, finite_sure);
+  else
+    return project_point<kPretest>(c, m, x, y, z, pretest_here, finite_sure);
+}
+
 __device__ __forceinline__ bool keep_rule(const DevCamera &c, const Projected &p, const uint32_t *__restrict__ depth) {
   if (!c.enable_zbuf) return p.cell != -1;
   if (p.cell < 0) return false;
@@ -183,6 +223,12 @@
   return true;
 }
 
+__device__ __forceinline__ float sqrt_rn(float x) {
+  if (vf::sqrt_in_window(x)) return vf::sqrt_from_estimate(x, __builtin_amdgcn_sqrtf(x));
+  return sqrtf(x);
+}
+
+template <bool kShortSqrt = false>
 __device__ __forceinline__ float final_score(float xc, float yc, float zc, double px, double py, double pz) {
   const double dx = static_cast<double>(xc) - px;
   const double dy = static_cast<double>(yc) - py;
@@ -200,7 +246,8 @@
     o = static_cast<float>((cosA + 1.0) / 2.0);
   }
   o = 0.2f + 0.8f * o;
-  const float dist = sqrtf((xc * xc + yc * yc) + zc * zc);
+  const float d2 = (xc * xc + yc * yc) + zc * zc;
+  const float dist = kShortSqrt ? sqrt_rn(d2) : sqrtf(d2);
   const float diff = fabsf(dist - 2.0f);
   float nd = diff / 2.0f;
   nd = nd < 1.0f ? nd : 1.0f;
diff --git a/pointcloudprocessor_amd/csrc/pcp_internal.hpp b/pointcloudprocessor_amd/csrc/pcp_internal.hpp
--- a/pointcloudprocessor_amd/csrc/pcp_internal.hpp
+++ b/pointcloudprocessor_amd/csrc/pcp_internal.hpp
@@ -152,6 +152,7 @@
   mutable std::string error;
 
   bool have_camera = false;
+  bool uv_tame = false;
   pcp_camera camera{};
   pcp_cull_params cull{};
   pcp::DevCamera dcam{};
diff --git a/pointcloudprocessor_amd/csrc/pcp_visit_forms.hpp b/pointcloudprocessor_amd/csrc/pcp_visit_forms.hpp
--- /dev/null
+++ b/pointcloudprocessor_amd/csrc/pcp_visit_forms.hpp
@@ -0,0 +1,105 @@
+#pragma once
+
+#include <stdint.h>
+
+#if defined(__HIPCC__)
+#include <hip/hip_runtime.h>
+#define PCP_VF_HD __host__ __device__ __forceinline__
+#define PCP_VF_FMA(a, b, c) __builtin_fma((a), (b), (c))
+#define PCP_VF_FMAF(a, b, c) __builtin_fmaf((a), (b), (c))
+#define PCP_VF_FMINF(a, b) __builtin_fminf((a), (b))
+#else
+#include <cmath>
+#define PCP_VF_HD inline
+#define PCP_VF_FMA(a, b, c) std::fma((a), (b), (c))
+#define PCP_VF_FMAF(a, b, c) std::fma((a), (b), (c))
+#define PCP_VF_FMINF(a, b) std::fmin((a), (b))
+#endif
+
+namespace pcp {
+namespace vf {
+
+struct Distortion {
+  double k1, k2, k3, p1, p2;
+};
+
+PCP_VF_HD void distort_written(const Distortion &c, double xn, double yn, double &xd, double &yd) {
+  const double x2 = xn * xn;
+  const double y2 = yn * yn;
+  const double r2 = x2 + y2;
+  const double r4 = r2 * r2;
+  const double r6 = r2 * r4;
+  const double rc = ((1.0 + c.k1 * r2) + c.k2 * r4) + c.k3 * r6;
+  const double t1 = (2.0 * xn) * yn;
+  const double t2 = r2 + 2.0 * x2;
+  const double t3 = r2 + 2.0 * y2;
+  xd = (rc * xn + c.p1 * t1) + c.p2 * t2;
+  yd = (rc * yn + c.p1 * t3) + c.p2 * t1;
+}
+
+PCP_VF_HD void distort_short(const Distortion &c, double xn, double yn, double &xd, double &yd) {
+  const double x2 = xn * xn;
+  const double y2 = yn * yn;
+  const double r2 = x2 + y2;
+  const double r4 = r2 * r2;
+  const double r6 = r2 * r4;
+  const double rc = ((1.0 + c.k1 * r2) + c.k2 * r4) + c.k3 * r6;
+  const double w = xn * yn;
+  const double a = c.p1 * w, b = c.p2 * w;
+  const double t2 = PCP_VF_FMA(2.0, x2, r2);
+  const double t3 = PCP_VF_FMA(2.0, y2, r2);
+  xd = PCP_VF_FMA(2.0, a, rc * xn) + c.p2 * t2;
+  yd = PCP_VF_FMA(2.0, b, rc * yn + c.p1 * t3);
+}
+
+PCP_VF_HD bool tame_coefficient(double p) {
+  const double m = p < 0.0 ? -p : p;
+  return p == 0.0 || (m >= 0x1p-400 && m <= 0x1p400);
+}
+PCP_VF_HD bool distortion_is_tame(double p1, double p2) { return tame_coefficient(p1) && tame_coefficient(p2); }
+
+PCP_VF_HD int32_t map_cell_written(float qx, float qy, float cull_wf, float cull_hf, int32_t mw, int32_t mh) {
+  const int32_t cx = ((qx > -1.0f) & (qx < cull_wf)) ? static_cast<int32_t>(qx) : -1;
+  const int32_t cy = ((qy > -1.0f) & (qy < cull_hf)) ? static_cast<int32_t>(qy) : -1;
+  if ((cx < 0) | (cy < 0)) return -1;
+  return ((cx < mw) & (cy < mh)) ? cy * mw + cx : -1;
+}
+
+PCP_VF_HD float map_bound(int32_t cells_along_axis) { return cells_along_axis > 0 ? static_cast<float>(cells_along_axis) : -1.0f; }
+
+PCP_VF_HD bool map_cell_short(float qx, float qy, float mwf, float mhf, int32_t mw, int32_t &cell) {
+  const float lo = PCP_VF_FMINF(qx, qy);
+  const bool ok = (lo > -1.0f) & (qx < mwf) & (qy < mhf);
+  cell = ok ? static_cast<int32_t>(qy) * mw + static_cast<int32_t>(qx) : 0;
+  return ok;
+}
+
+PCP_VF_HD bool sqrt_in_window(float x) {
+  union {
+    float f;
+    uint32_t u;
+  } b;
+  b.f = x;
+  return b.u - 0x0f800000u < 0x7f800000u - 0x0f800000u;
+}
+
+PCP_VF_HD float sqrt_from_estimate(float x, float s) {
+  union {
+    float f;
+    uint32_t u;
+  } b;
+  b.f = s;
+  const uint32_t sb = b.u;
+  b.u = sb - 1u;
+  const float dn = b.f;
+  b.u = sb + 1u;
+  const float up = b.f;
+  const float vp = PCP_VF_FMAF(-dn, s, x);
+  const float vs = PCP_VF_FMAF(-up, s, x);
+  float r = vp <= 0.0f ? dn : s;
+  r = vs > 0.0f ? up : r;
+  return r;
+}
+
+}
+}
diff --git a/pointcloudprocessor_amd/host/visit_forms_selftest.cpp b/pointcloudprocessor_amd/host/visit_forms_selftest.cpp
--- /dev/null
+++ b/pointcloudprocessor_amd/host/visit_forms_selftest.cpp
@@ -0,0 +1,189 @@
+#include <cfloat>
+#include <cmath>
+#include <cstdint>
+#include <cstdio>
+#include <cstdlib>
+#include <cstring>
+#include <vector>
+
+#include "../csrc/pcp_visit_forms.hpp"
+
+namespace vf = pcp::vf;
+
+static uint64_t mix(uint64_t v) {
+  v += 0x9e3779b97f4a7c15ull;
+  v = (v ^ (v >> 30)) * 0xbf58476d1ce4e5b9ull;
+  v = (v ^ (v >> 27)) * 0x94d049bb133111ebull;
+  return v ^ (v >> 31);
+}
+static float f32_of(uint32_t b) {
+  float f;
+  std::memcpy(&f, &b, 4);
+  return f;
+}
+static uint32_t bits_of(float f) {
+  uint32_t b;
+  std::memcpy(&b, &f, 4);
+  return b;
+}
+static uint64_t bits_of(double d) {
+  uint64_t b;
+  std::memcpy(&b, &d, 8);
+  return b;
+}
+static bool same(double a, double b) { return (a != a && b != b) || bits_of(a) == bits_of(b); }
+static bool same(float a, float b) { return (a != a && b != b) || bits_of(a) == bits_of(b); }
+
+static long check_distortion(long samples) {
+  const double inf = INFINITY, nan = NAN;
+  const vf::Distortion sets[] = {
+      {0.003043514741045163, 0.06634739187544138, 0.0, -0.000217681797407554, -0.0006654964142658197},
+      {0.0, 0.0, 0.0, 0.0, 0.0},
+      {0.1, -0.02, 0.003, 0.0, 0.0},
+      {-0.2, 0.05, -0.001, -0.01, -0.02},
+      {0.1, 0.2, 0.3, 0x1p-400, -0x1p400},
+      {1e10, -1e20, 1e30, 1e100, -0.0},
+  };
+  std::vector<double> edge = {0.0, -0.0, inf, -inf, nan, 1.0, -1.0, 0.5, 0x1p-277, -0x1p-277, 0x1p277, -0x1p277,
+                              0x1p-149 / 3.0, 3.0e38 / 0x1p-149, 1.0 / 3.0, -2.0 / 3.0, 0x1p128, 0x1p-128};
+  long bad = 0, done = 0;
+  for (const vf::Distortion &c : sets) {
+    if (!vf::distortion_is_tame(c.p1, c.p2)) {
+      std::printf("distortion: a coefficient set of the test is not tame\n");
+      return 1;
+    }
+    auto one = [&](double xn, double yn) {
+      double xa, ya, xb, yb;
+      vf::distort_written(c, xn, yn, xa, ya);
+      vf::distort_short(c, xn, yn, xb, yb);
+      ++done;
+      if (!same(xa, xb) || !same(ya, yb)) {
+        if (bad < 10) std::printf("distortion: xn %a yn %a: written (%a, %a) short (%a, %a)\n", xn, yn, xa, ya, xb, yb);
+        ++bad;
+      }
+    };
+    for (double a : edge)
+      for (double b : edge) one(a, b);
+    for (long i = 0; i < samples; ++i) {
+      const uint64_t r = mix(static_cast<uint64_t>(i) * 3u + 17u), s = mix(r);
+      uint32_t bx = static_cast<uint32_t>(r), by = static_cast<uint32_t>(r >> 32), bz = static_cast<uint32_t>(s);
+      if ((s >> 32) & 3u) {
+        bx = (bx & 0x807fffffu) | ((121u + (bx >> 23) % 12u) << 23);
+        by = (by & 0x807fffffu) | ((121u + (by >> 23) % 12u) << 23);
+        bz = (bz & 0x807fffffu) | ((121u + (bz >> 23) % 12u) << 23);
+      }
+      const float x = f32_of(bx), y = f32_of(by), z = std::fabs(f32_of(bz));
+      if (!(z > 0.0f)) continue;
+      one(static_cast<double>(x) / static_cast<double>(z), static_cast<double>(y) / static_cast<double>(z));
+    }
+  }
+  const double wild[] = {0x1p-401, -0x1p-401, 0x1p401, 4.9e-324, 1e-200, inf, -inf, nan};
+  for (double p : wild)
+    if (vf::distortion_is_tame(p, 0.0) || vf::distortion_is_tame(0.0, p) || vf::distortion_is_tame(p, p)) {
+      std::printf("distortion: %a passes as tame\n", p);
+      ++bad;
+    }
+  std::printf("distortion: %ld pairs, %ld mismatches\n", done, bad);
+  return bad;
+}
+
+static long check_cells(long samples) {
+  struct Geometry {
+    int32_t cull_w, cull_h, ds;
+  };
+  const Geometry sets[] = {{703, 405, 14}, {703, 405, 1}, {703, 405, 7}, {703, 405, 20}, {4096, 3000, 14}, {13, 405, 14},
+                           {703, 5, 7}, {1 << 24, 100, 1}, {100, 1 << 24, 1}, {(1 << 24) - 1, 3, 2}};
+  long bad = 0, done = 0;
+  for (const Geometry &g : sets) {
+    const int32_t mw = g.cull_w / g.ds, mh = g.cull_h / g.ds;
+    const float cwf = static_cast<float>(g.cull_w), chf = static_cast<float>(g.cull_h);
+    const float mwf = vf::map_bound(mw), mhf = vf::map_bound(mh);
+    std::vector<float> edge = {0.0f, -0.0f, -1.0f, std::nextafter(-1.0f, 0.0f), std::nextafter(-1.0f, -2.0f), -0.5f, 0.5f,
+                               1.0f, INFINITY, -INFINITY, NAN, FLT_MAX, -FLT_MAX, FLT_MIN, -FLT_MIN, 1e-45f, -1e-45f,
+                               2147483648.0f, -2147483648.0f, 4294967296.0f, 16777216.0f};
+    for (float m : {static_cast<float>(mw), static_cast<float>(mh), cwf, chf, cwf / static_cast<float>(g.ds), chf / static_cast<float>(g.ds)})
+      for (float e : {m, std::nextafter(m, 0.0f), std::nextafter(m, INFINITY), m - 1.0f, m - 0.5f, m + 0.5f}) edge.push_back(e);
+    auto one = [&](float qx, float qy) {
+      const int32_t a = vf::map_cell_written(qx, qy, cwf, chf, mw, mh);
+      int32_t cell = 0;
+      const int32_t b = vf::map_cell_short(qx, qy, mwf, mhf, mw, cell) ? cell : -1;
+      ++done;
+      if (a != b) {
+        if (bad < 10) std::printf("cell: %d x %d / %d, q (%a, %a): written %d short %d\n", g.cull_w, g.cull_h, g.ds, qx, qy, a, b);
+        ++bad;
+      }
+    };
+    for (float a : edge)
+      for (float b : edge) one(a, b);
+    for (long i = 0; i < samples; ++i) {
+      const uint64_t r = mix(static_cast<uint64_t>(i) * 5u + 3u);
+      float qx = f32_of(static_cast<uint32_t>(r)), qy = f32_of(static_cast<uint32_t>(r >> 32));
+      if (i & 1) {
+        qx = (static_cast<float>(static_cast<uint32_t>(r) >> 8) * 0x1p-24f) * (1.25f * cwf + 2.0f) - 2.0f;
+        qy = (static_cast<float>(static_cast<uint32_t>(r >> 32) >> 8) * 0x1p-24f) * (1.25f * chf + 2.0f) - 2.0f;
+      }
+      one(qx, qy);
+    }
+  }
+  std::printf("cell: %ld pairs, %ld mismatches\n", done, bad);
+  return bad;
+}
+
+static long check_sqrt(long samples) {
+  long bad = 0, done = 0;
+  auto one = [&](float x) {
+    if (!vf::sqrt_in_window(x)) {
+      if (x >= 0x1p-96f && x <= FLT_MAX) {
+        std::printf("sqrt: %a is in the window but not recognised\n", x);
+        ++bad;
+      }
+      return;
+    }
+    const float want = std::sqrt(x);
+    const double root = std::sqrt(static_cast<double>(x));
+    float lo = static_cast<float>(root);
+    if (static_cast<double>(lo) > root) lo = std::nextafter(lo, 0.0f);
+    float cand[3];
+    int n = 0;
+    if (static_cast<double>(lo) == root) {
+      cand[n++] = std::nextafter(lo, 0.0f);
+      cand[n++] = lo;
+      cand[n++] = std::nextafter(lo, INFINITY);
+    } else {
+      cand[n++] = lo;
+      cand[n++] = std::nextafter(lo, INFINITY);
+    }
+    for (int k = 0; k < n; ++k) {
+      const float got = vf::sqrt_from_estimate(x, cand[k]);
+      ++done;
+      if (!same(got, want)) {
+        if (bad < 10) std::printf("sqrt: x %a estimate %a: %a, sqrtf %a\n", x, cand[k], got, want);
+        ++bad;
+      }
+    }
+  };
+  const float edge[] = {0.0f, -0.0f, -1.0f, INFINITY, -INFINITY, NAN, 1e-45f, FLT_MIN, std::nextafter(0x1p-96f, 0.0f), 0x1p-96f,
+                        std::nextafter(0x1p-96f, 1.0f), 0x1p-95f, FLT_MAX, std::nextafter(FLT_MAX, 0.0f), 1.0f, 2.0f, 4.0f,
+                        std::nextafter(1.0f, 0.0f), std::nextafter(1.0f, 2.0f), std::nextafter(4.0f, 0.0f), 0x1p127f, 0x1p126f};
+  for (float x : edge) one(x);
+  for (int e = -96; e <= 127; ++e) {
+    const float p = std::ldexp(1.0f, e);
+    for (float x : {p, std::nextafter(p, INFINITY), std::nextafter(p, 0.0f), p * 1.5f, p * 1.5625f}) one(x);
+  }
+  for (uint32_t k = 1; k < 4096; ++k) {
+    const float s = static_cast<float>(k) * static_cast<float>(k);
+    one(s);
+    one(std::nextafter(s, 0.0f));
+    one(std::nextafter(s, INFINITY));
+  }
+  for (long i = 0; i < samples; ++i) one(f32_of(static_cast<uint32_t>(mix(static_cast<uint64_t>(i) * 7u + 1u))));
+  std::printf("sqrt: %ld estimates, %ld mismatches\n", done, bad);
+  return bad;
+}
+
+int main(int argc, char **argv) {
+  const long samples = argc > 1 ? std::atol(argv[1]) : 1000000;
+  const long bad = check_distortion(samples) + check_cells(samples) + check_sqrt(samples);
+  std::printf("visit_forms_selftest: %ld mismatches\n", bad);
+  return bad == 0 ? 0 : 1;
+}
diff --git a/pointcloudprocessor_amd/host_build.py b/pointcloudprocessor_amd/host_build.py
--- a/pointcloudprocessor_amd/host_build.py
+++ b/pointcloudprocessor_amd/host_build.py
@@ -15,6 +15,7 @@
     "image_dump": ["image_dump.cpp"],
     "format_selftest": ["format_selftest.cpp"],
     "parse_selftest": ["parse_selftest.cpp"],
+    "visit_forms_selftest": ["visit_forms_selftest.cpp"],
 }
 
 
@@ -24,7 +25,7 @@
     for name, srcs in TARGETS.items():
         exe = os.path.join(BIN, name)
         deps = [os.path.join(HOST, s) for s in srcs] + [os.path.join(HOST, "pcp_shim.hpp"), os.path.join(HOST, "pcp_multi.hpp"), os.path.join(HOST, "pcd_io.hpp"), os.path.join(HOST, "image_io.hpp"), os.path.join(HOST, "pcd_device_reader.hpp"),
-                                                       os.path.join(_build.CSRC, "pcp_ascii_parse.hpp"), os.path.join(_build.CSRC, "pcp_ascii.hpp"),
+                                                       os.path.join(_build.CSRC, "pcp_ascii_parse.hpp"), os.path.join(_build.CSRC, "pcp_ascii.hpp"), os.path.join(_build.CSRC, "pcp_visit_forms.hpp"),
                                                        os.path.join(_build.INCLUDE, "pcp_hip.h")]
         deps = [d for d in deps if os.path.exists(d)]
         stale = force or not os.path.exists(exe) or any(os.path.getmtime(d) > os.path.getmtime(exe) for d in deps)
@@ -33,7 +34,7 @@
             multi = ["-D__HIP_PLATFORM_AMD__", "-isystem", os.path.join(ROCM, "include")] if name == "PointCloudProcessor" else []
             multi_libs = ["-L", os.path.join(ROCM, "lib"), "-lrccl", "-lamdhip64", "-Wl,-rpath," + os.path.join(ROCM, "lib")] \
                 if name == "PointCloudProcessor" else []
-            cmd = ["g++", "-std=c++17", "-O2", "-pthread", "-Wall", "-Wextra"] + extra + multi + ["-I", _build.INCLUDE, "-I", HOST] + [
+            cmd = ["g++", "-std=c++17", "-O2", "-ffp-contract=off", "-pthread", "-Wall", "-Wextra"] + extra + multi + ["-I", _build.INCLUDE, "-I", HOST] + [
                 os.path.join(HOST, s) for s in srcs] + ["-L", _build.LIB_DIR, "-lpcp_hip"] + multi_libs + [
                                                         "-lz", "-Wl,-rpath,$ORIGIN/../../lib", "-o", exe]
             proc = subprocess.run(cmd, capture_output=True, text=True)
```

Result: faster. 1.959 million (median of 6 runs) (+4.5%).
